# Mamba413/bess

Hardware: AMD Instinct MI355X
Metric: candidate subsets solved/sec (n=50k,p=10k,k<=200 LM) (higher is better)
Workload: dtype f64; 1 GPU; configs[1]: LM sequential path, Gaussian X n=50000 p=10000, s.list=1..200, GIC, warm start, max_iter=20, is_normal; score_pass=covariance updates (cached Gram columns), collective=none, ranks_with_work=1

## Files before the change

bess_amd/capi.py:

```python
import ctypes
import os
import sys

import numpy as np

_HERE = os.path.dirname(os.path.abspath(__file__))
LIB_PATH = os.environ.get("BESSX_LIB_PATH") or os.path.join(_HERE, "libbessx.so")

_D = ctypes.POINTER(ctypes.c_double)
_I = ctypes.POINTER(ctypes.c_int)
_i = ctypes.c_int
_d = ctypes.c_double
_ll = ctypes.c_longlong
_vp = ctypes.c_void_p

SYMBOLS = [
    "bessx_last_error", "bessx_device_info", "bessx_pywrap_bess", "bessx_bessCpp", "bessx_session_create",
    "bessx_session_destroy", "bessx_session_set_cv", "bessx_session_get_cv_folds", "bessx_session_sequential_path", "bessx_session_gs_path",
    "bessx_session_pgs_path", "bessx_session_get_screening", "bessx_session_get_screening_groups", "bessx_session_get_screening_scores", "bessx_session_score_mode", "bessx_session_counter",
    "bessx_session_trace_enable", "bessx_session_trace_size", "bessx_session_trace_copy_int",
    "bessx_session_trace_copy_double", "bessx_session_get_normalization", "bessx_session_score_pass_stats",
    "bessx_session_enable_kernel_timing", "bessx_session_submodel_steps", "bessx_session_fit", "bessx_session_fit_width", "bessx_session_reset_caches",
    "bessx_session_sequential_path_chain", "bessx_session_cv_eval", "bessx_session_debug_block_stream",
    "bessx_session_set_fill_hook", "bessx_session_set_kpath_chains",
# ... 537 lines not shown
    y, weight, state, lambda_seq = _f64(y).reshape(-1), _f64(weight), _f64(state), _f64(lambda_seq)
    sequence, g_index, always_select = _i32(sequence), _i32(g_index), _i32(always_select)
    cap = sequence.size * lambda_seq.size if path_type == 1 else 2 * (s_max - s_min + 1) + 128
    beta = np.zeros(p)
    beta_all = np.zeros((p, cap), order="F")
    coef0_all, loss_all, ic_all = np.zeros(cap), np.zeros(cap), np.zeros(cap)
    scr = np.zeros(max(screening_size, 1), dtype=np.int32)
    r = RResult()
    r.beta, r.all_capacity = _dp(beta), cap
    r.beta_all, r.coef0_all, r.train_loss_all, r.ic_all, r.screening_A = (_dp(beta_all), _dp(coef0_all), _dp(loss_all),
                                                                         _dp(ic_all), _ip(scr))
    _check(lib().bessx_bessCpp(_dp(x), n, p, _dp(y), data_type, _dp(weight), int(is_normal), algorithm_type, model_type,
                               max_iter, exchange_num, path_type, int(is_warm_start), ic_type, int(is_cv), K, _dp(state),
                               state.size, _ip(sequence), sequence.size, _dp(lambda_seq), lambda_seq.size, s_min, s_max,
                               K_max, epsilon, lambda_min, lambda_max, nlambda, int(is_screening), screening_size,
                               powell_path, _ip(g_index), g_index.size, _ip(always_select), always_select.size, tao,
                               ctypes.byref(r)))
    k = min(r.n_all, cap)
    out = {"beta": beta, "coef0": r.coef0, "train_loss": r.train_loss, "ic": r.ic, "lambda": r.lambda_,
           "beta_all": np.array(beta_all[:, :k]), "coef0_all": coef0_all[:k], "train_loss_all": loss_all[:k],
           "ic_all": ic_all[:k]}
    if path_type == 1:
        ns, nl = sequence.size, lambda_seq.size
        out["beta_all"] = [np.array(beta_all[:, j * ns:(j + 1) * ns]) for j in range(nl)]
        out["coef0_all"] = [coef0_all[j * ns:(j + 1) * ns] for j in range(nl)]
        out["train_loss_all"] = [loss_all[j * ns:(j + 1) * ns] for j in range(nl)]
        out["ic_all"] = ic_all[:ns * nl].reshape(nl, ns).T
    if is_screening:
        out["screening_A"] = scr[:screening_size].copy()
    return out


class Session:

    def __init__(self, x, y, weight=None, data_type=1, is_normal=True, model_type=1, algorithm_type=1, max_iter=20,
                 is_warm_start=True, always_select=(), x_col_major=False, device=-1, g_index=None,
                 is_screening=False, screening_size=0, score_mode=0, max_sparsity=0, stream=0, row_order=None):
        din = None
        if is_device_array(x):
            din, self.n, self.p, _keep = _device_input(x, y, weight, row_order, stream)
            x = y = w = None
        else:
            x = np.asfortranarray(x, dtype=np.float64) if x_col_major else _f64(x)
            self.n, self.p = x.shape
            y = _f64(y).reshape(-1)
            if y.size != self.n:
                raise ValueError("X.shape(0) should be equal to y.size")
            w = None if weight is None else _f64(weight)
        al = _i32(always_select)
        gi = None if g_index is None else _i32(g_index)
        self._gsize_max = 1
        if gi is not None and gi.size:
            self._gsize_max = int(np.max(np.diff(np.append(gi, self.p))))
        pb = Problem(self.n, self.p, _dp(x), int(x_col_major), _dp(y), _dp(w), data_type, int(is_normal), model_type,
                     algorithm_type, max_iter, int(is_warm_start), _ip(al), al.size, device, _ip(gi),
                     0 if gi is None else gi.size, int(is_screening), int(screening_size), int(score_mode),
                     int(max_sparsity))
        h = _vp()
        if din is not None:
            _check_device_route(lib().bessx_session_create_device(ctypes.byref(h), ctypes.byref(pb), ctypes.byref(din)))
        else:
            _check(lib().bessx_session_create(ctypes.byref(h), ctypes.byref(pb)))
        self._h = h
        self.K = 0
        self.is_warm_start = bool(is_warm_start)
        self.p_kept = lib().bessx_session_get_screening(h, None, 0)

    def score_mode(self):
        return int(lib().bessx_session_score_mode(self._h))

    def counters(self):
        names = {0: "chained_fits", 1: "cg_fallbacks", 2: "passes_over_X", 3: "chained_queued", 7: "cv_side_by_side_rounds",
                 8: "cv_union_fills", 9: "tie_rescues", 10: "cache_restarts", 11: "cv_contexts_dropped",
                 12: "cv_fold_contexts", 13: "shared_wide_fills", 14: "kpath_chunked_paths", 15: "kpath_stitch_refits",
                 16: "kpath_chunk_fills", 17: "kpath_chains_last_path",
                 18: "kpath_stitch_giveups", 19: "group_XTX_ns",
                 22: "kpath_coarse_us",
                 23: "kpath_chunks_us", 24: "kpath_stitch_us", 25: "panel_launches_one_group",
                 26: "panel_ns_one_group", 27: "panel_launches_two_groups", 28: "panel_ns_two_groups",
                 29: "shared_pass_launches", 30: "shared_pass_chain_slots", 31: "shared_pass_partial_batches",
                 32: "own_queue_streams_created_by_the_process", 33: "multi_responses_batched",
                 34: "multi_responses_host", 35: "multi_union_fills", 36: "x_bytes_uploaded_from_host",
                 37: "x_bytes_ingested_on_device", 38: "live_device_bytes_of_the_process",
                 39: "live_pinned_bytes_of_the_process", 40: "allocation_requests_of_the_process"}
        return {n: int(lib().bessx_session_counter(self._h, i)) for i, n in names.items()}

    def screening(self):
        a = np.zeros(self.p_kept, dtype=np.int32)
        lib().bessx_session_get_screening(self._h, _ip(a), a.size)
        return a

    def screening_groups(self):
        n = lib().bessx_session_get_screening_groups(self._h, None, 0)
        a = np.zeros(max(n, 1), dtype=np.int32)
        lib().bessx_session_get_screening_groups(self._h, _ip(a), n)
        return a[:n]

    def screening_scores(self):
        n = lib().bessx_session_get_screening_scores(self._h, None, 0)
        a = np.zeros(max(n, 1))
        lib().bessx_session_get_screening_scores(self._h, _dp(a), n)
        return a[:n]

    def close(self):
        if getattr(self, "_h", None):
            lib().bessx_session_destroy(self._h)
            self._h = None

    def __del__(self):
        try:
            self.close()
        except Exception:
            pass

    def __enter__(self):
        return self

    def __exit__(self, *a):
        self.close()

    def set_cv(self, K, fold_id=None, seed=123):
        f = None if fold_id is None else _i32(fold_id)
        _check(lib().bessx_session_set_cv(self._h, K, _ip(f), seed))
        self.K = K

    def cv_folds(self):
        f = np.zeros(self.n, dtype=np.int32)
        _check(lib().bessx_session_get_cv_folds(self._h, _ip(f)))
        return f

    def trace_enable(self, on=True):
        _check(lib().bessx_session_trace_enable(self._h, int(on)))

    def enable_kernel_timing(self, on=True):
        _check(lib().bessx_session_enable_kernel_timing(self._h, int(on)))

    def score_pass_stats(self, reset=False):
        sec, nb, cnt = _d(0), _d(0), _ll(0)
        _check(lib().bessx_session_score_pass_stats(self._h, int(reset), ctypes.byref(sec), ctypes.byref(cnt),
                                                    ctypes.byref(nb)))
        return {"seconds": sec.value, "launches": cnt.value, "algorithmic_bytes": nb.value}

    def submodel_steps(self, reset=False):
        cnt = _ll(0)
        _check(lib().bessx_session_submodel_steps(self._h, int(reset), ctypes.byref(cnt)))
        return cnt.value

    def normalization(self):
        xm, xn, ym = np.zeros(self.p_kept), np.zeros(self.p_kept), _d(0)
        _check(lib().bessx_session_get_normalization(self._h, _dp(xm), _dp(xn), ctypes.byref(ym)))
        return xm, xn, ym.value

    def _result(self, res, capacity, max_T0):
        beta = np.zeros(self.p)
        arr = {
            "cand_T0": np.zeros(capacity, dtype=np.int32), "cand_lambda": np.zeros(capacity),
            "cand_iters": np.zeros(capacity, dtype=np.int32), "cand_train_loss": np.zeros(capacity),
            "cand_ic": np.zeros(capacity), "cand_coef0": np.zeros(capacity),
            "cand_support": np.full((capacity, max_T0), -1, dtype=np.int32), "cand_beta": np.zeros((capacity, max_T0)),
        }
        res.beta = _dp(beta)
        res.capacity = capacity
        res.max_T0 = max_T0
        for k, v in arr.items():
            setattr(res, k, _ip(v) if v.dtype == np.int32 else _dp(v))
        return beta, arr

# ... 2316 lines not shown
```

bess_amd/csrc/bessx_dev.h:

```cpp
#ifndef BESSX_DEV_H
#define BESSX_DEV_H

#include <hip/hip_runtime.h>

namespace bessx {

struct FitCtrl {
  int done;
  int l;
  int T0;
  int k_cur;
  int irls_done;
  int irls_steps;
  int info;
  int same_prev;
  double coef0;
  double ll0;
  int d_fresh;
  int irls_last;
  int fast_same;
  int ls_m;
  double ll1;
  int gram_full;
  int cov_nfill;
  int cov_stall;
  int cov_groups;
  int cov_miss;
  int cov_nmiss;
  int serial;
  int sse_valid;
  double sse_dot;
  double sse_nrm;
  unsigned long long snap_seq;
};
static_assert(sizeof(FitCtrl) <= 128, "the published control block is 128 bytes");

constexpr int GRAM_JC = 8;
struct GramTask {
  int I, J0, nJ, pad_;
};

hipError_t launch_transpose_in(const double *src, int rows, int p, double *X, long ld, long r0, hipStream_t st);
hipError_t launch_ingest(const void *src, int f32, long long rs, long long cs, const int *order, long long n,
                         long long p, double *X, long long ld, unsigned *nan_flag, hipStream_t st);
enum { PREDICT_IDENTITY = 0, PREDICT_LOGISTIC = 1, PREDICT_POISSON = 2 };
hipError_t launch_predict(const void *src, int f32, long long rs, long long cs, long long n, const int *cols, int m,
                          const double *B, const double *c, int R, int link, double *out, long long ors, long long ocs,
                          double *out2, hipStream_t st);
struct EvalData {
  const void *y;
  int y_f32;
  long long yrs, ycs;
  const void *w;
  int w_f32;
  long long ws;
};
long long eval_workspace(int f32, long long rs, long long cs, long long n, int m, int R, int link, int weighted);
hipError_t launch_eval(const void *src, int f32, long long rs, long long cs, long long n, const int *cols, int m,
                       const double *B, const double *c, int R, int link, const EvalData &d, double *work, double *res,
                       hipStream_t st);
hipError_t launch_eval_finish(const double *part, long long nb, int RS, double *out, hipStream_t st);
long long cox_eval_workspace(long long n, int R);
hipError_t launch_cox_eval_eta(const void *src, int f32, long long rs, long long cs, long long n, const int *cols, int m,
                               const double *B, const double *zero, int R, const int *pos, double *eta, double *ex,
                               hipStream_t st);
bool cox_eval_eta_by_rows(long long rs, long long cs, int m);
hipError_t launch_cox_eval_eta_rows(const void *src, int f32, long long rs, long long cs, long long n, const int *cols,
                                    int m, const double *B, const double *zero, const int *pos, double *eta, double *ex,
                                    hipStream_t st);
hipError_t launch_cox_eval_scan_tot(const double *e, long long n, int R, double *scr, hipStream_t st);
hipError_t launch_cox_eval_suffix(double *ex, long long n, int R, double *scr, hipStream_t st);
hipError_t launch_cox_eval_loglik(const double *eta, double *ex, const double *wd, const int *first, long long n, int R,
                                  double *work, double *res, hipStream_t st);
hipError_t launch_cox_eval_pairs(const double *eta, const int *kg, const int *first, long long n, int R,
                                 unsigned long long *cnt, hipStream_t st);
long long cox_surv_workspace(long long n);
hipError_t launch_cox_baseline(const double *S, const double *wd, const int *first, long long n, const int *ends, int J,
                               double *h, double *scr, double *hout, hipStream_t st);
hipError_t launch_cox_surv_ex(const void *src, int f32, long long rs, long long cs, long long n, const int *cols, int m,
                              const double *B, const double *zero, double *ex, hipStream_t st);
hipError_t launch_cox_surv_curves(const double *ex, const double *hg, long long n, int T, int kind, double *out,
                                  long long ors, long long ocs, hipStream_t st);
constexpr int COX_BRIER_T_MAX = 1 << 20;
void cox_brier_split(long long n, long long *rows_per_slab, long long *slabs);
int cox_brier_row_groups(int T);
long long cox_brier_workspace(long long n, int T, int R);
hipError_t launch_cox_brier_ex(const void *src, int f32, long long rs, long long cs, long long n, const int *cols, int m,
                               const double *B, const double *zero, int R, double *ex, hipStream_t st);
hipError_t launch_cox_brier(const double *e, const double *time, const double *w, const double *wa, const double *hg,
                            const double *tg, const double *b, long long n, int T, int R, double W, double *part,
                            double *bs, int only, hipStream_t st);
constexpr int PAIRAUC_TILE = 1024, PAIRAUC_T_MAX = 1024;
long long pairauc_tiles_max(long long n, int T);
long long pairauc_workspace(long long n, int T, int R);
hipError_t launch_pairauc_eta(const void *src, int f32, long long rs, long long cs, long long n, const int *cols, int m,
                              const double *B, const double *zero, int R, const int *pos, double *eta, hipStream_t st);
hipError_t launch_pairauc(const double *eta, const double *cw, const double *lw, const int *kg, const int *first,
                          const int *tstart, const int *tseg, const int *tnext, long long n, int NT, int S, int R, int uno,
                          const int *last, const int *from, int Q, double *part, double *og, double *oe, int only,
                          hipStream_t st);
constexpr int INFO_M_MAX = 1024;
void info_split(long long n, int m, long long *rows_per_slab, int *slabs);
long long info_gram_workspace(long long n, int m);
long long info_workspace(int f32, long long rs, long long cs, long long n, int m, int link, int weighted);
hipError_t launch_info_gram(const void *src, int f32, long long rs, long long cs, long long n, const int *cols, int m,
                            const double *vw, const double *gw, double *part, double *info, long long ld, double *score,
                            hipStream_t st);
hipError_t launch_info(const void *src, int f32, long long rs, long long cs, long long n, const int *cols, int m,
                       const double *B, const double *c, int link, const EvalData &d, double *work, double *res,
                       double *info, long long ld, double *score, hipStream_t st);
bool info_eta_by_rows(long long rs, long long cs, int m);
hipError_t launch_info_vg(const void *src, int f32, long long rs, long long cs, long long n, const int *cols, int m,
                          const double *B, const double *c, int link, const EvalData &d, double *v, double *g,
                          hipStream_t st);
enum { SANDWICH_HC0 = 0, SANDWICH_HC1 = 1, SANDWICH_HC2 = 2, SANDWICH_HC3 = 3 };
int sandwich_run_rows();
int sandwich_sum_depth(long long rows);
int sandwich_sq_depth(long long G);
// ... 65 lines not shown
hipError_t launch_cox_addscore_cc(const double *wd, const double *S0, const int *first, const int *lastk, long long n,
                                  double *scr, double *Cc, hipStream_t st);
hipError_t launch_cox_addscore_quad(const void *src, int f32, long long rs, long long cs, long long n, const int *cand,
                                    int q, int block, const int *rowof, const double *e, const double *Cc, double *part,
                                    double *t, int only, hipStream_t st);
int groupscore_band(int dmax);
void groupscore_rows(long long n, long long *rows_per_slab, int *slabs);
int groupscore_cut(const int *d, int nt, int block, int *first);
long long groupscore_doubles(long long n, int m, int qmax, int band);
hipError_t launch_groupscore_gram(const void *src, int f32, long long rs, long long cs, long long n, const int *cand,
                                  int qb, int band, const double *vw, double *work, int only, hipStream_t st);
hipError_t launch_groupscore_sband(const double *Cb, int m, int qb, int band, const double *pk, double *Tb, double *bandS,
                                   double *a, hipStream_t st);
hipError_t launch_groupscore_extract(const double *bandT, int band, const int *lpos, const long long *offs, int g0, int ng,
                                     double *out, hipStream_t st);
void cox_groupscore_rows(long long n, long long *rows_per_slab, int *slabs, int *t_depth);
long long cox_groupscore_doubles(long long n, int qmax, int band);
hipError_t launch_cox_groupscore_cc(const double *wd, const double *S0, const int *first, const int *lastk, long long n,
                                    double *cc, hipStream_t st);
hipError_t launch_cox_groupscore_tband(const void *src, int f32, long long rs, long long cs, long long n, const int *cand,
                                       int qb, int band, const int *rowof, const double *e, const double *cc, double *work,
                                       int only, double **bandT, hipStream_t st);
hipError_t launch_y_prepare_multi(double *Y, int n, long ld, int R, const double *w, int data_type, int is_normal,
                                  int add_weight, double *y_mean, double *yy, hipStream_t st);
hipError_t launch_normalize(double *X, long ld, int n, int p, double *y, const double *w, int data_type,
                            int is_normal, int add_weight, double *x_mean, double *x_norm, double *y_mean,
                            hipStream_t st);
hipError_t launch_xtv(const double *X, long ld, int p, int U, const double *v, const double *v2, double *part,
                      double *part2, const FitCtrl *ctrl, int slot, hipStream_t st);
hipError_t launch_xtv_variant(int variant, const double *X, long ld, int p, const double *v, double *part,
                              hipStream_t st);
constexpr int XTV_MC_MAX = 8;
struct XtvMc {
  const double *v[XTV_MC_MAX], *v2[XTV_MC_MAX];
  double *part[XTV_MC_MAX], *part2[XTV_MC_MAX];
  const FitCtrl *ctrl[XTV_MC_MAX];
  int slot[XTV_MC_MAX];
  int nc;
  int *ran;
};
hipError_t launch_xtv_mc(const double *X, long ld, int p, int U, const XtvMc &a, bool two, hipStream_t st);
hipError_t launch_score(const double *part, const double *part2, int nrb, int p, const double *beta_dense,
                        const double *xtx, double n_t, double lambda, int glm, const unsigned char *always,
                        double *bd, const FitCtrl *ctrl, int slot, hipStream_t st);
struct PubArgs {
  const unsigned char *dev;
  unsigned char *host;
  int ctrl_bytes;
  size_t off_sse;
  int n_sse;
  size_t off_b, off_a;
  int kcopy;
  unsigned long long *seq_host;
  unsigned long long seq;
  const int *count_ptr;
  int on;
  unsigned char *snap;
  size_t snap_count_off;
};
struct TopkNeed {
  const double *bd;
  double *bd2;
  int p;
  int C;
  int *slot_of, *meta, *fcols;
  FitCtrl *ctrl;
  const int *A_cur;
  const double *bmm;
  int nbmm;
  const unsigned char *inA;
  int inc1;
  int bmm_fresh;
  PubArgs pub;
  PubArgs snap;
  int cont_on, cont_serial, cont_parent;
  int commit_on;
  int no_restart;
  int *cm_A_cur;
  double *cm_b_cur, *cm_beta_dense;
  int *cm_hist;
  double *cm_hist_beta, *cm_hist_coef0;
  int cm_hist_stride;
  unsigned char *cm_inA;
};
bool topk_can_fuse_need(int len);
struct TopkTie {
  int *flag;
  int *work;
};
hipError_t launch_topk(const double *score, int len, int k, int *out, int *cand, const FitCtrl *ctrl, int slot,
                       hipStream_t st, const int *run_flag = nullptr, const TopkNeed *need = nullptr,
                       const TopkTie *tie = nullptr);
bool topk_supported(int len, int k);
void topk_set_variant(int v);
void gram_set_variant(int v);
bool gram_lds_applies(int ntiles, int tile_base);
hipError_t gram_lds_prepare();
bool irls_gram_applies(int mt);
int irls_gram_slab_rows(int mt, long ld);
int irls_gram_chunks(int mt);
hipError_t launch_irls_gram(int fam, const double *X, const double *aux, long ld, int n, const int *cols,
                            const double *y, const double *w, const double *mask, int nslab, int mt, double *part,
                            int ntiles, const FitCtrl *ctrl, int slot, int t, int T0, const double *bcur,
                            double *llpart, hipStream_t st, int wfloor = 1, int rows_override = 0);
hipError_t launch_gram_reduce(const double *part, int nslab, int ntiles, double *Gt, const FitCtrl *ctrl, int slot,
                              int gate_mode, hipStream_t st);
hipError_t launch_gram(const double *X, const double *aux, long ld, const int *cols, const double *w,
                       int rows_per_slab, const GramTask *tasks, int ntask, int nslab, double *part, int ntiles,
                       double *Gt, const FitCtrl *ctrl, int slot, int gate_mode, hipStream_t st, int tile_base = 0);
hipError_t launch_gram_lm_cached(const double *X, const double *aux, long ld, int *cols, const double *w,
                                 const int *A_new, int T0, int mt, const GramTask *tasks_full, int ntask_full,
                                 int rps_full, int nslab_full, const GramTask *tasks_inc, int ntask_inc, int rps_inc,
                                 int nslab_inc, double *part, double *Gt, double *Rt, int *src, double *gbuf0,
                                 double *gbuf1, int *Ac, int *meta, FitCtrl *ctrl, int slot, hipStream_t st);
struct CholFuse {
  const double *G;
  const int *slot_of;
  int p;
  int T0;
  FitCtrl *ctrl;
  int *A_cur;
  double *b_cur, *beta_dense;
  int *hist;
  double *hist_beta, *hist_coef0;
  int hist_stride;
  unsigned char *inA;
  double yy;
  const double *d;
  const double *GS;
  int CS;
  const double *zero;
  PubArgs pub;
  double *fb_work;
  const int *dep;
};
constexpr size_t CHOL_FB_DOUBLES = 256 * 256 + 1024;
struct IrlsChk {
  int on;
  FitCtrl *ctrl;
  int t, fam;
  const double *llpart;
  int nblk, m;
  double *bcur, *bprev;
};
hipError_t launch_chol(const double *Gt, int m, int mt, double ridge, int ridge_skip0, const double *rhs,
                       const int *rhs_gather, double *sol, int *info, const FitCtrl *ctrl, int slot, int gate_mode,
                       hipStream_t st, const CholFuse *fuse = nullptr, const IrlsChk *chk = nullptr);
hipError_t launch_sym_fallback(const double *Gt, int m, int mt, double ridge, int ridge_skip0, const double *rhs,
                               const int *rhs_gather, double *sol, int *info, const FitCtrl *ctrl, int slot,
                               hipStream_t st, const CholFuse *fuse);
hipError_t launch_cg(int m, int mt, double ridge, const double *rhs, const int *A_new, double *sol, const FitCtrl *ctrl,
                     int slot, const CholFuse *fuse, int maxit, hipStream_t st, double tol = 1e-13, bool by_rows = true);
bool sel_cgr_applies(int len, int m);
hipError_t launch_sel_cgr(const double *score, int len, int k, int *A_new, const FitCtrl *ctrl, int slot,
                          const TopkNeed *need, double ridge, const double *rhs, double *sol, const CholFuse *fuse,
                          int maxit, hipStream_t st, double tol);
struct McState {
  int cand;
  int ncand;
  int need_d;
  int finished;
  int parked;
  int resume;
  int prev_fresh;
  int prev_T0;
  int solves;
// ... 116 lines not shown
bool screen_logit_group_supported(int gmax);
size_t screen_logit_group_state_doubles(int N);
hipError_t launch_screen_logit_group(const double *X, long ld, int n, int N, const int *gidx, const int *gsz,
                                     const double *y, const double *w, double *state, int *done,
                                     const unsigned char *always, double *score, hipStream_t st);
bool screen_cox_group_supported(int gmax);
hipError_t launch_screen_cox_group(const double *X, long ld, int n, int N, const int *gidx, const int *gsz,
                                   const double *st_, const double *w, const unsigned char *always, double *score,
                                   hipStream_t st);
hipError_t launch_cox_group_moments(const double *X, long ld, int n, int p, CoxBufs cb, const int *allcols, int mcols,
                                    int smax, int N, const int *gidx_h, const int *gsz_h, const int *gidx,
                                    const int *gsz, const int *goff, long mblk_len, double *mblk, double *mblk2,
                                    double *dcol, hipStream_t st);
hipError_t launch_group_score(int N, const int *gidx, const int *gsz, const int *goff, const double *mblk,
                              const double *dcol, const double *part, int nrb, int p, int lm, double n_t,
                              double lambda, const double *beta_dense, const unsigned char *always, double *bd,
                              hipStream_t st, int smax = 1, double *work = nullptr, double *zwork = nullptr,
                              const FitCtrl *ctrl = nullptr, int slot = 0, int eig_mode = 0, double *eig_v = nullptr,
                              double *eig_l = nullptr);
constexpr int GRP_EIG_MAX = 16;
hipError_t launch_group_expand(const int *G_sel, int T0, int gs, const int *gidx, int *cols, const FitCtrl *ctrl,
                               int slot, hipStream_t st);
hipError_t launch_commit_group(FitCtrl *ctrl, int slot, int T0, const int *G_new, int K, const int *cols,
                               const double *sol, int has_intercept, int wait_chain, int *A_cur, double *b_cur,
                               double *beta_dense, int *hist, double *hist_beta, double *hist_coef0, int hist_stride,
                               hipStream_t st);
hipError_t launch_screen_score_lm(const double *sxy, const double *sxx, int p, const unsigned char *always,
                                  double *score, hipStream_t st);
hipError_t launch_screen_logit(const double *X, long ld, int n, int p, const double *y, const double *w,
                               double *state, int *done, const unsigned char *always, double *score, hipStream_t st);
hipError_t launch_screen_cox(const double *X, long ld, int n, int p, const double *st_, const double *w,
                             const unsigned char *always, double *score, hipStream_t st);
hipError_t launch_gather_cols(const double *X, long ld, const int *A, int pnew, double *X2, hipStream_t st);
hipError_t launch_cov_need(const int *list, int len, const double *bd, double *bd2, int p, int *slot_of, int *meta,
                           int C, int *fcols, FitCtrl *ctrl, int slot, const int *A_cur, hipStream_t st,
                           int no_restart = 0);
hipError_t launch_cov_publish_slots(const int *fcols, const int *slot_w, int *slot_of, const FitCtrl *ctrl, hipStream_t st);
hipError_t launch_cov_fill_list(int *fcols, const int *extras, const double *bd2, int *slot_of, int *meta,
                                FitCtrl *ctrl, int parked, hipStream_t st, int spec_max, int spec, int spec_min = 0);
hipError_t launch_cov_resume(FitCtrl *ctrl, hipStream_t st);
struct CovRowSets {
  int nr;
  double *G[9], *GS[9];
  const double *xtx[9];
  int ex_lo[9], ex_hi[9];
};
hipError_t launch_cov_reduce_compact_sets(const double *part, int p, const int *fcols, const int *slot_of, int *meta,
                                          const CovRowSets &rs, int g0, int ngroups, int nslab, int CS,
                                          const FitCtrl *ctrl, int parked, hipStream_t st);
constexpr int CGB_MAX_K = 4096;
struct CgbState {
  double rr[2];
  double qq;
  int done_step;
  int steps;
};
struct CgbWork {
  double *x, *q, *r[2], *p[2], *ap[2], *part_pq[2], *part_qq;
  CgbState *st;
};
size_t cgb_work_doubles(int kcap);
hipError_t launch_cg_big(const double *G, int p, const int *slot_of, const int *meta, const int *A_new, int k,
                         double ridge, const double *xty, const double *beta_dense, double *work, int kcap, double *sol,
                         FitCtrl *ctrl, int slot, int nsteps, double tol, double yy, hipStream_t st);
struct CovUnion {
  int nf;
  const int *list[8];
  int len[8];
  int on_restart[8];
  int dn;
  const int *const *dlist;
  const int *dlen;
};
hipError_t launch_cov_fill_union(const CovUnion &u, int restart, const int *extras, const double *bd2, int spec_max,
                                 int spec_min, int *slot_of, int *meta, int p, int *fcols, FitCtrl *fill_ctrl,
                                 hipStream_t st, int C = 0);
int cov_streamed_tiles_per_wave();
hipError_t launch_cov_panel(const double *X, const double *aux, long ld, int p, const double *mask, const int *fcols,
                            int g0, int ngroups, int rows_per_slab, int nslab, double *part, const FitCtrl *ctrl,
                            int parked, hipStream_t st);
hipError_t cov_panel_prepare();
hipError_t launch_cov_reduce(const double *part, int p, const int *fcols, const int *slot_of, double *G, int g0,
                             int ngroups, int nslab, const FitCtrl *ctrl, int parked, hipStream_t st,
                             int ex_lo = 0, int ex_hi = 0);
hipError_t launch_rows_permute(const double *X, long ld, int p, const int *perm, long ldp, double *Xp, hipStream_t st);
hipError_t launch_cov_compact(const double *G, int p, const int *slot_of, const int *fcols, int g0, int ngroups,
                              double *GS, int CS, const FitCtrl *ctrl, int parked, hipStream_t st,
                              const double *xtx = nullptr, int *meta = nullptr);
hipError_t launch_cov_d(const double *G, int p, const int *slot_of, const double *xty, const int *A_cur,
                        const double *b_cur, double *d_out, const double *beta_dense, const double *xtx, double n_t,
                        double lambda, const unsigned char *always, double *bd, const unsigned char *inA, double *bmm,
                        const FitCtrl *ctrl, int slot, hipStream_t st);
hipError_t launch_cov_gram(const double *G, int p, const int *slot_of, const int *A_new, int T0, int mt, double *Gt,
                           int *meta, const FitCtrl *ctrl, int slot, hipStream_t st);
hipError_t launch_publish(const unsigned char *dev, unsigned char *host, int ctrl_bytes, size_t off_sse, int n_sse,
                          size_t off_b, size_t off_a, int kcopy, unsigned long long *seq_host, unsigned long long seq,
                          hipStream_t st, const int *count_ptr = nullptr);
hipError_t launch_vec_mul(const double *a, const double *b, long n, double *out, hipStream_t st);
hipError_t launch_part_sum(const double *part, int nrb, int p, double *out, hipStream_t st);
hipError_t launch_fill(double *a, long n, double v, hipStream_t st);
hipError_t launch_gram_cols(const int *A_new, int T0, int mp, int intercept, int rhs_col, int *cols, FitCtrl *ctrl,
                            int slot, const int *A_cur, int allow_skip, hipStream_t st);
hipError_t launch_copy(const double *src, double *dst, long n, hipStream_t st);

}
#endif
```

bess_amd/csrc/bessx_fit.cpp:

```cpp
#include "bessx_host.h"

namespace bessx {

static int score_pass(bessx_session *s, int kind, int rs, int slot, std::vector<std::pair<size_t, bool>> &k1_pairs) {
  if (rs == 0 && shared_pass_applies(s)) {
    if (s->timing) k1_pairs.push_back({(size_t)-1, false});
    if (kind == 2 && s->cox.one_pass)
      return shared_pass_submit(s, nullptr, nullptr, s->part_rs[rs], nullptr, &s->cox, s->ctrl, slot);
    if (kind != 2)
      return shared_pass_submit(s, s->r_rs[rs], kind == 1 ? s->h_rs[rs] : nullptr, s->part_rs[rs],
                                kind == 1 ? s->part2_rs[rs] : nullptr, nullptr, s->ctrl, slot);
  }
  hipEvent_t ea = nullptr, eb = nullptr;
  if (int rc = k1_begin(s, &ea, &eb)) return rc;
  hipError_t e;
  if (kind == 2)
    e = launch_cox_score_pass(s->X, s->ld, s->p, s->U, s->nrb, s->cox, s->part_rs[rs], s->part2_rs[rs], s->ctrl, slot, s->st);
  else
    e = launch_xtv(s->X, s->ld, s->p, s->U, s->r_rs[rs], kind == 1 ? s->h_rs[rs] : nullptr, s->part_rs[rs],
                   kind == 1 ? s->part2_rs[rs] : nullptr, s->ctrl, slot, s->st);
  if (s->timing && e == hipSuccess) {
    e = hipEventRecord(eb, s->st);
    k1_pairs.push_back({s->ev_used - 2, false});
  }
// ... 31 lines not shown
    return 0;
  }
  if (e == hipSuccess && mt > 16) {
    e = launch_gram(s->X, s->aux, s->ld, s->gcols, s->mask[rs], rps, tasks_full, ntask, nslab, s->gpart, ntiles, s->Gt,
                    s->ctrl, slot, 0, s->st, 0);
    if (e == hipSuccess)
      e = launch_chol_big(s->Gt, T0, mt, lambda, 0, s->xty[rs], s->A_new, s->sol, &s->ctrl->info, s->rdiag, s->zbig,
                          s->ctrl, slot, 0, s->st);
  } else if (e == hipSuccess) {
    int rps_i, nslab_i;
    const int ntask_i = s->gtask_inc_cnt[mt];
    gram_geometry(s, ntask_i * 3, &rps_i, &nslab_i);
    bessx_session::GramCache &gc = s->gcache[rs];
    e = launch_gram_lm_cached(s->X, s->aux, s->ld, s->gcols, s->mask[rs], s->A_new, T0, mt,
                              tasks_full, ntask, rps, nslab, s->gtasks + s->gtask_inc_off[mt],
                              ntask_i, rps_i, nslab_i, s->gpart, s->Gt, s->Rt, s->gsrc, gc.g0, gc.g1, gc.A, gc.meta,
                              s->ctrl, slot, s->st);
    const CholFuse fbz = chol_fallback_only(s);
    if (e == hipSuccess)
      e = launch_chol(s->Gt, T0, mt, lambda, 0, s->xty[rs], s->A_new, s->sol, &s->ctrl->info, s->ctrl, slot, 0, s->st,
                      &fbz);
    if (e == hipSuccess)
      e = launch_sym_fallback(s->Gt, T0, mt, lambda, 0, s->xty[rs], s->A_new, s->sol, &s->ctrl->info, s->ctrl, slot, s->st,
                              &fbz);
  }
  if (e == hipSuccess)
    e = launch_commit(s->ctrl, slot, T0, s->A_new, s->sol, 0, 0, s->A_cur, s->b_cur, s->beta_dense, s->hist,
                      s->hist_beta, s->hist_coef0, s->hist_stride, s->st, s->inA);
  if (e == hipSuccess)
    e = launch_resid_lm(s->X, s->ld, s->n, s->y, s->mask[rs], s->ctrl, slot, s->A_cur, s->b_cur, s->r_rs[rs],
                        s->sse, s->st);
  if (e != hipSuccess) return fail(BESSX_ERR_HIP, std::string("enqueue_lm_slot: ") + hipGetErrorString(e));
  return 0;
}


int enqueue_cov_fill(bessx_session *s, int rs, int ngroups, int parked, const FitCtrl *gate,
                            int gfirst, bool compact, const int *slot_map) {
  bessx_session::CovCache &cv = s->cov[rs];
  const FitCtrl *gc = gate ? gate : s->ctrl;
  const int *smap = slot_map ? slot_map : cv.slot_of;
  for (int g0 = gfirst; g0 < gfirst + ngroups; g0 += COV_SLOT_GROUPS) {
    const int ng = std::min(COV_SLOT_GROUPS, gfirst + ngroups - g0);
    hipEvent_t ea = nullptr, eb = nullptr;
    if (int rc = k1_begin(s, &ea, &eb)) return rc;
    hipError_t e = hipSuccess;
    if (s->cv_shared) {
      const int nsl_all = s->K * s->cvp_nsl;
      e = launch_cov_panel(s->Xp, s->zp, s->ldp, s->p, nullptr, s->cov_fcols, g0, ng, s->cvp_rps, nsl_all, s->cvp_part,
                           gc, parked, s->st);
      if (s->timing && e == hipSuccess) {
        e = hipEventRecord(eb, s->st);
        s->cov_timed.push_back({s->ev_used - 2, g0});
      }
      if (s->K + 1 <= 9 && e == hipSuccess) {
        CovRowSets rsets = {};
        rsets.nr = s->K + 1;
        for (int r = 0; r <= s->K; r++) {
          rsets.G[r] = s->cov[r].G;
          rsets.GS[r] = s->cov[r].GS;
          rsets.xtx[r] = s->xtx[r];
          rsets.ex_lo[r] = r == 0 ? 0 : (r - 1) * s->cvp_nsl;
          rsets.ex_hi[r] = r == 0 ? 0 : r * s->cvp_nsl;
        }
        e = launch_cov_reduce_compact_sets(s->cvp_part, s->p, s->cov_fcols, s->cov[0].slot_of, s->cov[0].meta, rsets, g0, ng,
                                           nsl_all, s->cov_cs, gc, parked, s->st);
      }
      for (int r = 0; r <= s->K && e == hipSuccess && s->K + 1 > 9; r++) {
        bessx_session::CovCache &cr = s->cov[r];
        const int lo = r == 0 ? 0 : (r - 1) * s->cvp_nsl, hi = r == 0 ? 0 : r * s->cvp_nsl;
        e = launch_cov_reduce(s->cvp_part, s->p, s->cov_fcols, cr.slot_of, cr.G, g0, ng, nsl_all, gc, parked, s->st,
                              lo, hi);
        if (e == hipSuccess)
          e = launch_cov_compact(cr.G, s->p, cr.slot_of, s->cov_fcols, g0, ng, cr.GS, s->cov_cs, gc, parked, s->st,
                                 s->xtx[r], cr.meta);
      }
      if (e != hipSuccess) return fail(BESSX_ERR_HIP, std::string("cov panel (shared): ") + hipGetErrorString(e));
      continue;
    }
    e = launch_cov_panel(s->X, s->aux, s->ld, s->p, s->mask[rs], s->cov_fcols, g0, ng, s->cov_rps,
                         s->cov_nslab, s->cov_part, gc, parked, s->st);
    if (s->timing && e == hipSuccess) {
      e = hipEventRecord(eb, s->st);
      s->cov_timed.push_back({s->ev_used - 2, g0});
    }
    if (e == hipSuccess)
      e = launch_cov_reduce(s->cov_part, s->p, s->cov_fcols, smap, cv.G, g0, ng, s->cov_nslab, gc, parked,
                            s->st);
    if (e == hipSuccess && compact)
      e = launch_cov_compact(cv.G, s->p, smap, s->cov_fcols, g0, ng, cv.GS, s->cov_cs, gc, parked, s->st, s->xtx[rs],
                             cv.meta);
    if (e != hipSuccess) return fail(BESSX_ERR_HIP, std::string("cov panel: ") + hipGetErrorString(e));
  }
  return 0;
}

int cov_C_dev(const bessx_session *s) { return s->cov_C - (s->cov_spec - COV_R); }

struct SlotFuse {
  const PubArgs *pub = nullptr;
  bool pub_fused = false;
  bool pub_snapshot = false;
  const PubArgs *attach = nullptr;
  bool attached = false;
  int cont_serial = 0, cont_parent = 0;
  bool cont = false, cont_fused = false;
};

CholFuse cov_fuse_args(bessx_session *s, int rs, int T0, bool force_chol, SlotFuse *sf) {
  bessx_session::CovCache &cv = s->cov[rs];
  CholFuse fz = {cv.G,          cv.slot_of, s->p,         T0,           s->ctrl,        s->A_cur, s->b_cur,
                 s->beta_dense, s->hist,    s->hist_beta, s->hist_coef0, s->hist_stride, s->inA,   s->yy_h[rs],
                 s->part_rs[rs], cv.GS, s->cov_cs,
                 cv.zero, PubArgs{}, s->fb_work, cv.meta + 4};
  if (sf && sf->pub && s->fuse && s->cov_cg && !force_chol && rs == 0) {
    fz.pub = *sf->pub;
    if (sf->pub_snapshot) fz.pub.on = 2;
    sf->pub_fused = true;
  }
  return fz;
}

int cgb_reserve(bessx_session *s) {
  bessx_session *owner = s->parent ? s->parent : s;
  if (!owner->cgb_work) {
    const int kcap = std::min(owner->cap, CGB_MAX_K);
    if (owner->own.alloc(&owner->cgb_work, cgb_work_doubles(kcap)) != hipSuccess) {
      (void)hipGetLastError();
      return 1;
    }
    owner->cgb_cap = kcap;
  }
  s->cgb_work = owner->cgb_work;
  s->cgb_cap = owner->cgb_cap;
  return 0;
}

int enqueue_cov_tail(bessx_session *s, int slot, int T0, double lambda, int rs, bool force_chol,
                            SlotFuse *sf) {
  const int mt = (T0 + 1 + 15) / 16;
  bessx_session::CovCache &cv = s->cov[rs];
  hipError_t e = hipSuccess;
  bool used_cgb = false;
  if (mt > 16 && s->cov_cg && !force_chol && T0 <= CGB_MAX_K && cgb_reserve(s) == 0) {
    e = launch_cg_big(cv.G, s->p, cv.slot_of, cv.meta, s->A_new, T0, lambda, s->xty[rs], s->beta_dense, s->cgb_work,
                      s->cgb_cap, s->sol, s->ctrl, slot, s->cgb_guess, s->cg_tol, s->yy_h[rs], s->st);
    used_cgb = e == hipSuccess;
    if (e == hipSuccess)
      e = launch_commit(s->ctrl, slot, T0, s->A_new, s->sol, 0, 0, s->A_cur, s->b_cur, s->beta_dense, s->hist,
                        s->hist_beta, s->hist_coef0, s->hist_stride, s->st, s->inA);
  } else if (mt > 16) {
    e = launch_cov_gram(cv.G, s->p, cv.slot_of, s->A_new, T0, mt, s->Gt, cv.meta, s->ctrl, slot, s->st);
    if (e == hipSuccess)
      e = launch_chol_big(s->Gt, T0, mt, lambda, 0, s->xty[rs], s->A_new, s->sol, &s->ctrl->info, s->rdiag, s->zbig,
                          s->ctrl, slot, 0, s->st);
    if (e == hipSuccess)
      e = launch_commit(s->ctrl, slot, T0, s->A_new, s->sol, 0, 0, s->A_cur, s->b_cur, s->beta_dense, s->hist,
                        s->hist_beta, s->hist_coef0, s->hist_stride, s->st, s->inA);
  } else {
    CholFuse fz = cov_fuse_args(s, rs, T0, force_chol, sf);
    if (s->cov_cg && !force_chol)
      e = launch_cg(T0, (T0 + 15) / 16, lambda, s->xty[rs], s->A_new, s->sol, s->ctrl, slot, &fz, 64, s->st, s->cg_tol,
                    s->cg_by_rows);
    else {
      e = launch_chol(s->Gt, T0, mt, lambda, 0, s->xty[rs], s->A_new, s->sol, &s->ctrl->info, s->ctrl, slot, 0, s->st,
                      &fz);
      if (e == hipSuccess)
        e = launch_sym_fallback(s->Gt, T0, mt, lambda, 0, s->xty[rs], s->A_new, s->sol, &s->ctrl->info, s->ctrl, slot,
                                s->st, &fz);
    }
  }
  if (e == hipSuccess && (rs != 0 || (mt > 16 && !used_cgb) || !s->cov_cg))
    e = launch_resid_lm(s->X, s->ld, s->n, s->y, s->mask[rs], s->ctrl, slot, s->A_cur, s->b_cur, s->r_rs[rs],
                        s->sse, s->st, 1);
  if (e != hipSuccess) return fail(BESSX_ERR_HIP, std::string("enqueue_cov_tail: ") + hipGetErrorString(e));
  return 0;
}

bool cov_speculates(const bessx_session *s) { return topk_supported(s->p, s->cov_spec) && s->p >= 2 * s->cov_spec; }

int enqueue_lm_slot_cov(bessx_session *s, int slot, int T0, double lambda, int rs, bool skip_d,
                               bool scores_ok, bool grow1, SlotFuse *sf) {
  bessx_session::CovCache &cv = s->cov[rs];
  hipError_t e = hipSuccess;
  if (skip_d && scores_ok) {
  } else if (!skip_d)
  {
    e = launch_cov_d(cv.G, s->p, cv.slot_of, s->xty[rs], s->A_cur, s->b_cur, s->part_rs[rs], s->beta_dense, s->xtx[rs],
                     (double)s->n_train[rs], lambda, s->always, s->bd, s->inA, s->cov_bmm, s->ctrl, slot, s->st);
    s->bmm_owner = rs;
  }
  else {
    e = launch_score(s->part_rs[rs], nullptr, 1, s->p, s->beta_dense, s->xtx[rs], (double)s->n_train[rs], lambda, 0,
                     s->always, s->bd, s->ctrl, slot, s->st);
    s->bmm_owner = -1;
  }
  if (e == hipSuccess && topk_can_fuse_need(s->p)) {
    TopkNeed nd = {cov_speculates(s) ? s->bd : nullptr, s->bd2, s->p, cov_C_dev(s), cv.slot_of, cv.meta, s->cov_fcols,
                   s->ctrl, s->A_cur, s->cov_bmm, (s->p + 31) / 32, s->inA, (slot == 1 && grow1) ? 1 : 0,
                   (slot == 1 && grow1 && s->bmm_owner == rs) ? 1 : 0};
    nd.cm_A_cur = s->A_cur;
    nd.cm_b_cur = s->b_cur;
    nd.cm_beta_dense = s->beta_dense;
    nd.cm_hist = s->hist;
    nd.cm_hist_beta = s->hist_beta;
    nd.cm_hist_coef0 = s->hist_coef0;
    nd.cm_hist_stride = s->hist_stride;
    nd.cm_inA = s->inA;
    nd.commit_on = (s->fuse && (T0 + 1 + 15) / 16 <= 16) ? 1 : 0;
    nd.no_restart = s->cov_no_restart ? 1 : 0;
    if (sf && sf->cont && s->fuse && slot == 1 && skip_d && scores_ok) {
      nd.cont_on = 1;
      nd.cont_serial = sf->cont_serial;
      nd.cont_parent = sf->cont_parent;
      sf->cont_fused = true;
      if (sf->attach) {
        nd.pub = *sf->attach;
        sf->attached = true;
      }
    }
    if (sf && sf->pub && sf->pub_snapshot && s->fuse && nd.commit_on && s->cov_cg && rs == 0) {
      nd.snap = *sf->pub;
      nd.snap.on = 2;
    }
    if (s->fuse_sel && s->fuse && s->cov_cg && s->cg_by_rows && sel_cgr_applies(s->p, T0)) {
      CholFuse fz = cov_fuse_args(s, rs, T0, false, sf);
      e = launch_sel_cgr(s->bd, s->p, T0, s->A_new, s->ctrl, slot, &nd, lambda, s->xty[rs], s->sol, &fz, 64, s->st,
                         s->cg_tol);
      if (e == hipSuccess && rs != 0)
        e = launch_resid_lm(s->X, s->ld, s->n, s->y, s->mask[rs], s->ctrl, slot, s->A_cur, s->b_cur, s->r_rs[rs],
                            s->sse, s->st, 1);
      if (e != hipSuccess) return fail(BESSX_ERR_HIP, std::string("enqueue_lm_slot_cov (fused): ") + hipGetErrorString(e));
      return 0;
    }
    e = launch_topk(s->bd, s->p, T0, s->A_new, s->cand, s->ctrl, slot, s->st, nullptr, &nd);
  } else if (e == hipSuccess) {
    e = launch_topk(s->bd, s->p, T0, s->A_new, s->cand, s->ctrl, slot, s->st, nullptr, nullptr, &s->tie);
    if (e == hipSuccess)
      e = launch_cov_need(s->A_new, T0, cov_speculates(s) ? s->bd : nullptr, s->bd2, s->p, cv.slot_of, cv.meta, cov_C_dev(s),
                          s->cov_fcols, s->ctrl, slot, s->A_cur, s->st, s->cov_no_restart ? 1 : 0);
  }
  if (e != hipSuccess) return fail(BESSX_ERR_HIP, std::string("enqueue_lm_slot_cov: ") + hipGetErrorString(e));
  return enqueue_cov_tail(s, slot, T0, lambda, rs, false, sf);
}

int cov_unpark(bessx_session *s, const FitCtrl *hc, int T0, double lambda, int rs, int *next_slot) {
  bessx_session::CovCache &cv = s->cov[rs];
  const int stalled = -1 - hc->l + 1, nm = hc->cov_nmiss;
  if (hc->cov_stall == 2) {
    s->cov_cg_fallbacks++;
    if ((T0 + 1 + 15) / 16 > 16) s->cgb_guess = 64;
    HIPX(launch_cov_resume(s->ctrl, s->st));
    if (int rc = enqueue_cov_tail(s, stalled, T0, lambda, rs, true)) return rc;
    *next_slot = stalled + 1;
    return 0;
  }
  if (hc->cov_stall == 3) {
    s->cov_tie_rescues++;
    HIPX(launch_cov_resume(s->ctrl, s->st));
    hipError_t e = launch_topk(s->bd, s->p, T0, s->A_new, s->cand, s->ctrl, stalled, s->st, nullptr, nullptr, &s->tie);
    if (e == hipSuccess)
      e = launch_cov_need(s->A_new, T0, cov_speculates(s) ? s->bd : nullptr, s->bd2, s->p, cv.slot_of, cv.meta,
                          cov_C_dev(s), s->cov_fcols, s->ctrl, stalled, s->A_cur, s->st, s->cov_no_restart ? 1 : 0);
    if (e != hipSuccess) return fail(BESSX_ERR_HIP, std::string("cov_unpark (tie): ") + hipGetErrorString(e));
    if (int rc = enqueue_cov_tail(s, stalled, T0, lambda, rs)) return rc;
    *next_slot = stalled + 1;
    return 0;
  }
  const bool spec = cov_speculates(s);
  hipError_t e = hipSuccess;
  struct FillGuard {
    bessx_session *c = nullptr;
    bool filled = false;
    ~FillGuard() {
      if (c) kchains_fill_end(c, filled);
    }
  } guard;
  const bool staged = s->kch_owner && kchains_staged(s) && cv.slot_w != nullptr;
  int *smap = staged ? cv.slot_w : cv.slot_of;
  if (s->kch_owner) {
    kchains_log(s, "parked: asks for the cache", T0, nm);
    const int waited = kchains_fill_begin(s);
    if (waited < 0) return fail(BESSX_ERR_HIP, "chunk chains: the fill rendezvous was abandoned");
    guard.c = s;
    kchains_log(s, waited ? "has the cache: looks again" : "has the cache: fills", T0, nm);
    if (waited > 0) {
      HIPX(launch_cov_resume(s->ctrl, s->st));
      e = launch_cov_need(s->A_new, T0, spec ? s->bd : nullptr, s->bd2, s->p, cv.slot_of, cv.meta, cov_C_dev(s),
                          s->cov_fcols, s->ctrl, stalled, s->A_cur, s->st, 1);
      if (e != hipSuccess) return fail(BESSX_ERR_HIP, std::string("cov_unpark (chunk chain): ") + hipGetErrorString(e));
      if (int rc = enqueue_cov_tail(s, stalled, T0, lambda, rs)) return rc;
      *next_slot = stalled + 1;
      return 0;
    }
  }
  if (s->fill_hook && rs == 0 && !s->parent && spec) {
    const int p = s->p;
    std::vector<int> miss((size_t)nm), slot_h((size_t)p);
    std::vector<double> sc((size_t)p);
    HIPX(hipMemcpyAsync(miss.data(), s->cov_fcols, (size_t)nm * sizeof(int), hipMemcpyDeviceToHost, s->st));
    HIPX(hipMemcpyAsync(sc.data(), s->bd2, (size_t)p * sizeof(double), hipMemcpyDeviceToHost, s->st));
    HIPX(hipMemcpyAsync(slot_h.data(), cv.slot_of, (size_t)p * sizeof(int), hipMemcpyDeviceToHost, s->st));
    HIPX(hipStreamSynchronize(s->st));
    std::vector<int> order;
    order.reserve((size_t)p);
    for (int j = 0; j < p; j++)
      if (slot_h[j] < 0 && sc[j] >= 0.0) order.push_back(j);
    int total = std::max(s->fill_hook_width, (nm + COV_R - 1) / COV_R * COV_R);
    if (nm + (int)order.size() < total) total = (nm + (int)order.size()) / COV_R * COV_R;
    if (total >= nm && total >= COV_R && total <= s->capA) {
      const int extra = total - nm;
      std::partial_sort(order.begin(), order.begin() + extra, order.end(), [&](int a, int b) {
        return sc[a] > sc[b] || (sc[a] == sc[b] && a < b);
      });
      std::vector<int> list(miss);
      list.insert(list.end(), order.begin(), order.begin() + extra);
      if (int rc = prefill_begin(s, list.data(), total, 2)) return rc;
      if (s->fill_hook(s->fill_hook_user, total / COV_R) != 0)
        return fail(BESSX_ERR_ARG, "the fill hook reported a failure");
      if (s->prefill_cols != 0) return fail(BESSX_ERR_ARG, "the fill hook returned without bessx_session_cov_prefill_end");
      s->shared_wide_fills++;
      HIPX(launch_cov_resume(s->ctrl, s->st));
      if (int rc = enqueue_cov_tail(s, stalled, T0, lambda, rs)) return rc;
      *next_slot = stalled + 1;
      return 0;
    }
  }
  const bool wide = spec && s->cov_C >= (s->p + 31) / 32 * 32 + COV_R && topk_supported(s->p, 2 * COV_R) && s->p >= 4 * COV_R;
  const int pool = wide ? 2 * COV_R : s->cov_spec;
  if (spec) e = launch_topk(s->bd2, s->p, pool, s->cov_extras, s->cand, nullptr, 0, s->st);
  if (e == hipSuccess)
    e = launch_cov_fill_list(s->cov_fcols, s->cov_extras, s->bd2, smap, cv.meta, s->ctrl, 1, s->st, s->cov_spec,
                             spec ? (wide ? 2 : 1) : 0, s->cov_spec_min);
  if (e != hipSuccess) return fail(BESSX_ERR_HIP, std::string("cov_unpark: ") + hipGetErrorString(e));
  const int room = spec ? std::min(((nm + s->cov_spec_min + s->cov_spec - 1) / s->cov_spec) * s->cov_spec - nm, pool) : 0;
  const int ngroups = (nm + room + COV_R - 1) / COV_R;
  if (test_hook("panel_log")) std::fprintf(stderr, "[bessx] fill: level %d, %d missing, list of up to %d -> %d group(s)%s\n", T0, nm, nm + room, ngroups, s->kch_owner ? " (chunk chain)" : "");
  hipStream_t own_st = s->st;
  hipStream_t fill_st = staged ? s->kch_owner->kch_fill_st : nullptr;
  if (fill_st && !s->kch_ev && s->own.event(&s->kch_ev, hipEventDisableTiming) != hipSuccess) {
    (void)hipGetLastError();
    fill_st = nullptr;
  }
  if (fill_st) {
    HIPX(hipEventRecord(s->kch_ev, own_st));
    HIPX(hipStreamWaitEvent(fill_st, s->kch_ev, 0));
    s->st = fill_st;
  }
  int frc = enqueue_cov_fill(s, rs, ngroups, 1, nullptr, 0, true, smap);
  hipError_t fe = hipSuccess;
  if (frc == 0 && staged) fe = launch_cov_publish_slots(s->cov_fcols, cv.slot_w, cv.slot_of, s->ctrl, s->st);
  s->st = own_st;
  if (frc) return frc;
  HIPX(fe);
  if (s->kch_owner) {
    HIPX(hipStreamSynchronize(fill_st ? fill_st : s->st));
    s->kch_owner->kch_chunk_fills++;
    guard.filled = true;
    kchains_log(s, "fill done", ngroups, nm);
  }
  HIPX(launch_cov_resume(s->ctrl, s->st));
  if (int rc = enqueue_cov_tail(s, stalled, T0, lambda, rs)) return rc;
  *next_slot = stalled + 1;
  return 0;
}

int glm_geometry(bessx_session *s, int T0, int *mt, int *mp, int *ntask, int *ntiles, int *rps, int *nslab) {
  *mt = (T0 + 2 + 15) / 16;
  *mp = *mt * 16;
  const GramTask *tk = nullptr;
  if (int rc = gram_tasks_for(s, *mt, &tk, ntask)) return rc;
  *ntiles = *mt * (*mt + 1) / 2;
  gram_geometry(s, *ntask, rps, nslab, *ntiles);
  if ((size_t)*nslab * *ntiles * 256 > s->gpart_elems) return fail(BESSX_ERR_ARG, "gram workspace too small");
  return 0;
}

int enqueue_glm_head(bessx_session *s, int slot, int T0, double lambda, int rs, bool skip_k1,
                            std::vector<std::pair<size_t, bool>> &k1_pairs) {
  const int fam = s->model_type;
  int mt, mp, ntask, ntiles, rps, nslab;
  if (int rc = glm_geometry(s, T0, &mt, &mp, &ntask, &ntiles, &rps, &nslab)) return rc;
  hipError_t e = hipSuccess;
  if (!skip_k1) {
    if (int rc = score_pass(s, 1, rs, slot, k1_pairs)) return rc;
  } else if (s->timing) {
    k1_pairs.push_back({(size_t)-1, false});
  }
  if (e == hipSuccess)
    e = launch_score(s->part_rs[rs], s->part2_rs[rs], s->nrb, s->p, s->beta_dense, nullptr, (double)s->n_train[rs],
                     lambda, 1, s->always, s->bd, s->ctrl, slot, s->st);
  if (e == hipSuccess) e = launch_topk(s->bd, s->p, T0, s->A_new, s->cand, s->ctrl, slot, s->st, nullptr, nullptr, &s->tie);
  if (e == hipSuccess)
    e = launch_gram_cols(s->A_new, T0, mp, 1, 1, s->gcols, s->ctrl, slot, s->A_cur, fam == 2 ? 1 : 0, s->st);
  if (e == hipSuccess) e = launch_glm_irls_begin(s->ctrl, slot, fam, T0 + 1, s->bcur, s->bprev, s->st);
  if (e != hipSuccess) return fail(BESSX_ERR_HIP, std::string("enqueue_glm_head: ") + hipGetErrorString(e));
  return 0;
}

int enqueue_glm_irls_step(bessx_session *s, int slot, int t, int T0, double lambda, int rs) {
  const int fam = s->model_type;
  int mt, mp, ntask, ntiles, rps, nslab;
  if (int rc = glm_geometry(s, T0, &mt, &mp, &ntask, &ntiles, &rps, &nslab)) return rc;
  double *z = s->aux + 2 * s->ld;
  if (s->irls_fuse && irls_gram_applies(mt)) {
    const int rows = irls_gram_slab_rows(mt, s->ld);
    const int ns = (int)((s->ld + rows - 1) / rows);
    if ((size_t)ns * ntiles * 256 <= s->gpart_elems && (size_t)ns <= s->llpart_cap) {
      hipError_t e = launch_irls_gram(fam, s->X, s->aux, s->ld, s->n, s->gcols, s->y, s->w, s->mask[rs], ns, mt,
                                      s->gpart, ntiles, s->ctrl, slot, t, T0, s->bcur, s->llpart, s->st, s->irls_wfloor);
      if (e == hipSuccess) e = launch_gram_reduce(s->gpart, ns, ntiles, s->Gt, s->ctrl, slot, 1, s->st);
      const IrlsChk ck = {1, s->ctrl, t, fam, s->llpart, ns, T0 + 1, s->bcur, s->bprev};
      const CholFuse fbz = chol_fallback_only(s);
      if (e == hipSuccess)
        e = launch_chol(s->Gt, T0 + 1, mt, 2.0 * lambda, 1, nullptr, nullptr, s->bcur, &s->ctrl->info, s->ctrl, slot, 1,
                        s->st, &fbz, &ck);
      if (e == hipSuccess && s->glm_fallback)
        e = launch_sym_fallback(s->Gt, T0 + 1, mt, 2.0 * lambda, 1, nullptr, nullptr, s->bcur, &s->ctrl->info, s->ctrl, slot,
                                s->st, &fbz);
      if (e != hipSuccess) return fail(BESSX_ERR_HIP, std::string("enqueue_glm_irls_step: ") + hipGetErrorString(e));
      return 0;
    }
  }
  hipError_t e = launch_glm_irls_prep(fam, s->X, s->ld, s->n, s->y, s->w, s->mask[rs], s->ctrl, slot, t, s->A_new, T0,
                                      s->bcur, s->Wv, z, s->llpart, s->st, s->irls_wfloor);
  if (e == hipSuccess)
    e = launch_glm_irls_check(s->ctrl, slot, t, fam, s->llpart, s->n_sse_blk, T0 + 1, s->bcur, s->bprev, s->st);
  const GramTask *tk = nullptr;
  int ntk = 0;
  if (int rc = gram_tasks_for(s, mt, &tk, &ntk)) return rc;
  if (e == hipSuccess)
    e = launch_gram(s->X, s->aux, s->ld, s->gcols, s->Wv, rps, tk, ntask, nslab, s->gpart, ntiles, s->Gt, s->ctrl,
// ... 578 lines not shown
    s->glm_fallback = true;
    HIPX(hipStreamSynchronize(s->st));
    HIPX(hipMemsetAsync(&s->ctrl->info, 0, sizeof(int), s->st));
    s->cache[rs].valid = s->cache[rs].model_only = false;
    s->dev_state_rs = -1;
    return algorithm_fit_grouped(s);
  }
  if (hc->info) return fail(BESSX_ERR_NUMERIC, "non-finite value in the k x k solve (singular Gram matrix?)");
  const int K = hc->k_cur;
  const double *sse_h = reinterpret_cast<const double *>(s->res_h + ((unsigned char *)s->sse - s->resblk));
  const double *b_h = reinterpret_cast<const double *>(s->res_h + ((unsigned char *)s->b_cur - s->resblk));
  const int *a_h = reinterpret_cast<const int *>(s->res_h + ((unsigned char *)s->A_cur - s->resblk));
  s->beta.idx.assign(a_h, a_h + K);
  s->beta.val.assign(b_h, b_h + K);
  s->coef0 = hc->coef0;
  s->l = hc->done ? hc->l : s->max_iter + 1;
  double tr = 0.0, te = 0.0;
  for (int b = 0; b < s->n_sse_blk; b++) {
    tr += sse_h[2 * b];
    te += sse_h[2 * b + 1];
  }
  s->sse_train = tr;
  s->sse_test = te;
  s->n_fits += 1;
  s->n_iters += hc->l;
  if (gcov && hc->done) {
    cc.valid = true;
    cc.cov_layout = true;
    cc.lambda = lambda;
    cc.T0 = T0;
    cc.beta = s->beta;
    cc.coef0 = s->coef0;
    s->dev_state_rs = rs;
  }
  if (s->trace.on) {
    const int L = hc->l;
    std::vector<double> hb((size_t)(L + 1) * s->hist_stride), hc0(L + 1);
    HIPX(hipMemcpy(hb.data(), s->hist_beta, hb.size() * sizeof(double), hipMemcpyDeviceToHost));
    HIPX(hipMemcpy(hc0.data(), s->hist_coef0, hc0.size() * sizeof(double), hipMemcpyDeviceToHost));
    for (int it = 1; it <= L; it++) {
      const std::vector<int> &cc = cols_hist[it - 1];
      s->trace.meta.push_back(it);
      s->trace.meta.push_back(T0);
      s->trace.meta.push_back(s->n_train[rs]);
      s->trace.meta.push_back((int)s->trace.a_flat.size());
      for (size_t i = 0; i < cc.size(); i++) {
        s->trace.a_flat.push_back(cc[i]);
        s->trace.beta_flat.push_back(hb[(size_t)it * s->hist_stride + i]);
      }
      s->trace.coef0_calls.push_back(hc0[it]);
    }
  }
  return 0;
}

int enqueue_chained(bessx_session *s, const bessx_session::Hint &hint, int rs, int parent, int buf, int batch,
                           double parent_lambda, int parent_T0) {
  const int Tn = hint.T0;
  if (!(hint.on && s->chain && s->publish && s->warm_start && !s->trace.on && rs == 0 && s->cov_mode && Tn >= 1 &&
        Tn <= s->cap && Tn + COV_R + s->cov_spec <= s->cov_C && topk_supported(s->p, Tn)))
    return 0;
  bessx_session::Ahead &ah = s->ahead;
  s->chain_queued++;
  ah.armed = true;
  ah.T0 = Tn;
  ah.lambda = hint.lambda;
  ah.rs = rs;
  ah.serial = ++s->fit_serial;
  ah.buf = buf;
  const bool cont_fusable = s->fuse && hint.lambda == parent_lambda && topk_can_fuse_need(s->p);
  PubArgs parent_pub = {};
  const bool have_parent_pub = s->pend_on && cont_fusable && s->defer_pub;
  if (have_parent_pub) {
    parent_pub = s->pend;
    s->pend_on = false;
  } else if (int rc = publish_flush(s)) {
    return rc;
  }
  if (!cont_fusable) HIPX(launch_fit_continue(s->ctrl, Tn, s->hist, s->st, ah.serial, 1, parent));
  const PubArgs pa = publish_args(s, Tn, buf, &ah.seq);
  bool published = false, snapshotted = false;
  for (int b = 0, sl = 1; b < batch && sl <= s->max_iter; b++, sl++) {
    SlotFuse sf;
    const bool last = b + 1 == batch || sl == s->max_iter;
    if (last) {
      sf.pub = &pa;
      sf.pub_snapshot = s->defer_pub;
    }
    if (sl == 1 && cont_fusable) {
      sf.cont = true;
      sf.cont_serial = ah.serial;
      sf.cont_parent = parent;
      if (have_parent_pub) sf.attach = &parent_pub;
    }
    if (int rc = enqueue_lm_slot_cov(s, sl, Tn, hint.lambda, rs, sl == 1, hint.lambda == parent_lambda,
                                     hint.lambda == parent_lambda && Tn == parent_T0 + 1, &sf))
      return rc;
    if (sl == 1 && cont_fusable && !sf.cont_fused) return fail(BESSX_ERR_HIP, "internal: chained fit was not opened");
    if (sl == 1 && have_parent_pub && !sf.attached) return fail(BESSX_ERR_HIP, "internal: deferred publication lost");
    published = published || sf.pub_fused;
    snapshotted = snapshotted || (sf.pub_fused && sf.pub_snapshot);
  }
  if (snapshotted) {
    s->pend = publish_from_snapshot(pa);
    s->pend_on = true;
    return 0;
  }
  return published ? 0 : publish_launch(s, pa);
}


int algorithm_fit(bessx_session *s) {
  if (s->grouped) return algorithm_fit_grouped(s);
  const int T0 = s->sparsity_level, rs = s->cur_rows;
  const double lambda = s->lambda_level;
  if (rs != 0 && !s->fold_ctx.empty()) fold_contexts_invalidate(s);
  if (T0 < 1 || T0 > s->cap)
    return fail(BESSX_ERR_ARG, "sparsity level " + std::to_string(T0) + " outside [1, " + std::to_string(s->cap) +
                                   "]: a session holds work space for min(p, max(2046, bessx_problem.max_sparsity))"
                                   " active columns, max_sparsity <= " + std::to_string(T0_HARD));
  if (s->model_type == 4)
    if (int rc = cox_reserve(s, T0)) return rc;
  if (!topk_supported(s->p, T0)) return fail(BESSX_ERR_UNSUPPORTED, "top-k selection: p too large for this sparsity level");
  const bool glm = s->model_type != 1;
  const bool cox = s->model_type == 4;
  const int k_init = (int)s->beta_init.idx.size();
  if (k_init > s->cap) return fail(BESSX_ERR_ARG, "initial support too large");
  bessx_session::RsCache &cc = s->cache[rs];
  const bool cov = s->cov_mode && !glm && T0 + COV_R + s->cov_spec <= s->cov_C && k_init + COV_R + s->cov_spec <= s->cov_C;
  bool use_cache = cc.valid && cc.coef0 == s->coef0_init && cc.beta.idx == s->beta_init.idx &&
                   cc.beta.val == s->beta_init.val && (!cox || s->cox_state_rs == rs) && (glm || cc.cov_layout == cov);
  if (cox) s->cox_state_rs = rs;
  bool model_kept = cov && !use_cache && cc.model_only && cc.cov_layout && s->dev_state_rs == rs &&
                          cc.coef0 == s->coef0_init && cc.beta.idx == s->beta_init.idx && cc.beta.val == s->beta_init.val &&
                          !s->trace.on && test_hook("model_kept") == nullptr;
  cc.valid = cc.model_only = false;
  const bessx_session::Hint hint = s->hint;
  s->hint.on = false;
  bool ahead_hit = false;
  int my_buf = 0, ahead_serial = 0;
  if (s->ahead.armed) {
    s->ahead.armed = false;
    const bessx_session::Ahead mine = s->ahead;
    if (cov && use_cache && s->dev_state_rs == rs && mine.T0 == T0 && mine.lambda == lambda && mine.rs == rs &&
        !s->trace.on) {
      if (int rc = enqueue_chained(s, hint, rs, mine.serial, mine.buf ^ 1, 2, lambda, T0)) return rc;
      if (!s->ahead.armed)
        if (int rc = publish_flush(s)) return rc;
      if (int rc = publish_wait(s, mine.buf, mine.seq)) return rc;
      ahead_hit = reinterpret_cast<const FitCtrl *>(s->res_h)->serial == mine.serial;
      if (!ahead_hit) {
        s->ahead.armed = false;
        s->pend_on = false;
      }
      (ahead_hit ? s->chain_hits : s->chain_dead)++;
      my_buf = mine.buf;
      ahead_serial = mine.serial;
    } else {
      HIPX(hipStreamSynchronize(s->st));
      s->pend_on = false;
      s->dev_state_rs = -1;
      use_cache = false;
      model_kept = false;
      s->chain_mismatch++;
    }
  }
// ... 269 lines not shown
```

bess_amd/csrc/bessx_host.h:

```cpp
#ifndef BESSX_HOST_H
#define BESSX_HOST_H
#include <hip/hip_runtime.h>

#include <algorithm>
#include <atomic>
#include <chrono>
#include <cfloat>
#include <cmath>
#include <cstdio>
#include <condition_variable>
#include <cstring>
#include <functional>
#include <mutex>
#include <numeric>
#include <random>
#include <string>
#include <thread>
#include <vector>

#include "../../include/bessx.h"
#include "bessx_dev.h"
#include "bessx_sync.h"

namespace bessx {
// ... 210 lines not shown
  double *Wv = nullptr, *llpart = nullptr, *bcur = nullptr, *bprev = nullptr;
  int irls_guess = 8;
  bool grouped = false;
  int N = 0, gmax = 1;
  int g_uniform = 0;
  std::vector<int> gidx_h, gsz_h, goff_h;
  int *gidx = nullptr, *gsz = nullptr, *goff = nullptr, *gcols_new = nullptr;
  double *mblk = nullptr, *dcol = nullptr;
  double *mblk2 = nullptr;
  double *mwork = nullptr, *zwork = nullptr;
  int *allcols = nullptr;
  std::vector<double *> gxtx_rs;
  std::vector<double *> geig_v_rs, geig_l_rs;
  std::vector<double> geig_lambda;
  std::vector<char> geig_valid;
  bool geig_on = true;
  int cox_state_rs = -1;
  int dev_state_rs = -1;
  CoxBufs cox = {};
  int *idcols = nullptr;
  struct RsCache {
    bool valid = false;
    bool model_only = false;
    bool cov_layout = false;
    double lambda = 0.0;
    int T0 = 0;
    SparseVec beta;
    double coef0 = 0.0;
  };
  std::vector<RsCache> cache;
  std::vector<int> n_train;
  std::vector<double> yy_h;
  int K = 0;
  double *part2 = nullptr, *bd = nullptr, *beta_dense = nullptr, *sol = nullptr;
  double *tmpv = nullptr;
  int *A_new = nullptr, *cand = nullptr, *hist = nullptr, *gcols = nullptr, *info = nullptr;
  double *fb_work = nullptr;
  int *tie_buf = nullptr;
  TopkTie tie = {nullptr, nullptr};
  double *hist_beta = nullptr, *hist_coef0 = nullptr;
  int cap = 0;
  int capA = 0;
  int hist_stride = 0;
  double *rdiag = nullptr, *zbig = nullptr;
  std::vector<std::pair<int, GramTask *>> big_tasks;
  std::vector<int> big_task_cnt;
  size_t cox_M_cols = 0;
  GramTask *gtasks = nullptr;
  std::vector<int> gtask_off, gtask_cnt;
  std::vector<int> gtask_inc_off, gtask_inc_cnt;
  struct GramCache {
    double *g0 = nullptr, *g1 = nullptr;
    int *A = nullptr, *meta = nullptr;
  };
  std::vector<GramCache> gcache;
  struct CovCache {
    double *G = nullptr;
    int *slot_of = nullptr, *meta = nullptr;
    int *slot_w = nullptr;
    double *GS = nullptr;
    double *zero = nullptr;
    bool shares_map = false;
  };
  std::vector<CovCache> cov;
  long long dbg_waits = 0, dbg_waits_ready = 0;
  double dbg_enq_s = 0.0;
  bool cov_mode = false;
  int cov_cs = 512;
  double cg_tol = 1e-13;
  int cov_spec = 32;
  int cov_spec_min = 8;
  bool fuse_sel = true;
  bool cg_by_rows = true;
  bool irls_fuse = true;
  bool glm_fallback = false;
  int irls_wfloor = 1;
  size_t llpart_cap = 0;
  long long n_submodel_steps = 0;
  bool defer_pub = true;
  bool fuse = true;
  bool cov_cg = true;
  long long cov_cg_fallbacks = 0;
  long long cov_tie_rescues = 0;
  int cov_C = 0;
  int cov_rps = 0, cov_nslab = 0;
  bool cv_shared = false;
  double *Xp = nullptr, *zp = nullptr, *cvp_part = nullptr;
  long ldp = 0;
  int cvp_rps = 0, cvp_nsl = 0;
  bessx_session *parent = nullptr;
  std::vector<bessx_session *> fold_ctx;
  bool cv_side_by_side = true;
  bool cov_no_restart = false;
  FitCtrl *fill_ctrl = nullptr;
  FitCtrl *fill_ctrl_h = nullptr;
  hipEvent_t ev_fill = nullptr, ev_ctx = nullptr;
  long long cv_union_fills = 0, cv_rounds = 0;
  long long cv_ctx_dropped = 0;
  int fill_groups_seen = 0;
  FoldPool *fold_pool = nullptr;
  double wait_deadline_s = 30.0;
  double sbs_t[6] = {0, 0, 0, 0, 0, 0};
  double *cov_part = nullptr, *bd2 = nullptr;
  unsigned char *inA = nullptr;
  double *cov_bmm = nullptr;
  int bmm_owner = -1;
  int *cov_fcols = nullptr, *cov_extras = nullptr;
  long long cov_panel_groups = 0;
  bessx::KChains *kch = nullptr;
  bessx_session *kch_owner = nullptr;
  int kpath_chains = 0;
  int kch_index = -1;
  unsigned long long kch_gen_seen = 0;
  bool light_confirm = true;
  bool kch_fill_tried = false;
  bool kch_sp_member = false;
  long long sp_launches = 0, sp_chain_slots = 0, sp_partial = 0;
  int *kch_slot_w = nullptr;
  hipStream_t kch_fill_st = nullptr;
  hipEvent_t kch_ev = nullptr;
  int resp_R = 0;
  double *resp_y = nullptr, *resp_xty = nullptr, *resp_part = nullptr, *own_xty = nullptr;
  std::vector<double> resp_mean, resp_yy, resp_null;
  double *own_y = nullptr;
  double own_yy = 0.0, own_mean = 0.0, own_null = 0.0;
  long long multi_batched = 0, multi_host = 0, multi_fills = 0;
  long long x_host_bytes = 0, x_dev_bytes = 0;
  bool fcols_wide = false;
  long long kch_paths = 0, kch_refits = 0, kch_chunk_fills = 0;
  int kch_last_chains = 0;
  bool kch_auto_off = false;
  int cov_panel_blocks = 0;
  bool own_hw_queue = false;
  long long group_xtx_ns = 0;
  hipEvent_t xtx_ev[2] = {nullptr, nullptr};
  bool xtx_ev_pending = false;
  bool path_group_xtx = true;
  long long kch_giveups = 0;
  double kch_t[3] = {0, 0, 0};
  bessx_fill_hook fill_hook = nullptr;
  void *fill_hook_user = nullptr;
  int fill_hook_width = 0;
  long long shared_wide_fills = 0;
  int prefill_cols = 0;
  int prefill_base = 0;
  double *cgb_work = nullptr;
  int cgb_cap = 0, cgb_guess = 40;
  std::vector<std::pair<size_t, int>> cov_timed;
  double *Rt = nullptr;
  int *gsrc = nullptr;
  double *gpart = nullptr, *Gt = nullptr;
  size_t gpart_elems = 0;
  int *init_idx_d = nullptr;
  double *init_val_d = nullptr;
  unsigned char *resblk = nullptr;
  size_t res_bytes = 0;
  FitCtrl *ctrl = nullptr;
  double *sse = nullptr, *b_cur = nullptr;
  int *A_cur = nullptr;
  int n_sse_blk = 0;
  unsigned char *res_h = nullptr;
  bool publish = true;
  unsigned long long *pub_flag = nullptr, pub_seq = 0;
  unsigned char *res_buf[2] = {nullptr, nullptr};
  unsigned char *snap[2] = {nullptr, nullptr};
  bool pend_on = false;
// ... 205 lines not shown
```

bess_amd/csrc/bessx_k_cov.hip:

```cpp
#include "bessx_kdev.hpp"

namespace bessx {

constexpr int COV_NJ = 4;

#ifdef BESSX_PANEL_CLOCK
#define PCLK_BEGIN()                                                  \
  const unsigned long long pclk_t0_ = __builtin_amdgcn_s_memtime();   \
  const unsigned long long pclk_r0_ = __builtin_amdgcn_s_memrealtime()
#define PCLK_END(tag)                                                                                           \
  do {                                                                                                          \
    asm volatile("s_waitcnt vmcnt(0) lgkmcnt(0)" ::: "memory");                                                 \
    if (blockIdx.x == 7 && threadIdx.x == 0) {                                                                  \
      const unsigned long long dt_ = __builtin_amdgcn_s_memtime() - pclk_t0_;                                   \
      const unsigned long long dr_ = __builtin_amdgcn_s_memrealtime() - pclk_r0_;                               \
      printf("PCLK %s cycles %llu ticks100MHz %llu MHz %.0f\n", tag, dt_, dr_, dr_ ? 100.0 * (double)dt_ / (double)dr_ : 0.0); \
    }                                                                                                           \
  } while (0)
#else
#define PCLK_BEGIN()
#define PCLK_END(tag)
#endif

__device__ __forceinline__ bool cov_gate(const FitCtrl *ctrl, int slot) {
  if (ctrl->done) return false;
  if (slot == 0) return ctrl->l == 0;
  return ctrl->l == slot - 1 && !ctrl->same_prev;
}


__global__ void __launch_bounds__(256) k_cov_need(const int *__restrict__ list, int len,
                                                  const double *__restrict__ bd, double *__restrict__ bd2, int p,
                                                  int *__restrict__ slot_of, int *__restrict__ meta, int C,
                                                  int *__restrict__ fcols, FitCtrl *__restrict__ ctrl, int slot,
                                                  const int *__restrict__ A_cur, int no_restart) {
  KT(12);
  if (ctrl->done || (slot == 0 ? ctrl->l != 0 : ctrl->l != slot - 1)) return;
  cov_need_body<256>(list, len, bd, bd2, p, slot_of, meta, C, fcols, ctrl, slot, A_cur, false, no_restart != 0);
}

__global__ void __launch_bounds__(256) k_cov_fill_list(int *__restrict__ fcols, const int *__restrict__ extras,
                                                       const double *__restrict__ bd2, int *__restrict__ slot_of,
                                                       int *__restrict__ meta, FitCtrl *__restrict__ ctrl,
                                                       int parked, int spec_max, int spec, int spec_min) {
  KT(10);
  if (parked ? !ctrl->cov_stall : (ctrl->done || ctrl->l != 0)) return;
  const int nm = ctrl->cov_nmiss;
  const int tid = threadIdx.x;
  if (nm == 0) {
    if (tid == 0) ctrl->cov_nfill = 0;
    return;
  }
  const int count = meta[0];
  const int pool = spec == 2 ? 2 * COV_R : spec_max;
  const int room = spec ? min(((nm + spec_min + spec_max - 1) / spec_max) * spec_max - nm, pool) : 0;
  __shared__ int s_ne;
  if (tid < 64) {
    const int col = (spec && tid < pool) ? extras[tid] : -1;
    const double sc = col >= 0 ? bd2[col] : -1.0;
    const bool valid = col >= 0 && sc >= 0.0 && slot_of[col] < 0;
    const unsigned long long bal = __ballot(valid);
    int rank = 0;
    if (pool > spec_max) {
      for (int u = 0; u < 64; u++) {
        const double su = __shfl(sc, u);
        const int cu = __shfl(col, u);
        const bool vu = (bal >> u) & 1ull;
        if (vu && (su > sc || (su == sc && cu < col))) rank++;
      }
    } else {
      rank = __popcll(bal & ((1ull << tid) - 1ull));
    }
    if (valid && rank < room) fcols[nm + rank] = col;
    if (tid == 0) s_ne = min((int)__popcll(bal), room);
  }
  __syncthreads();
  const int tot = nm + s_ne, padded = (tot + COV_R - 1) / COV_R * COV_R;
  for (int i = tot + tid; i < padded; i += 256) fcols[i] = -1;
  for (int i = tid; i < tot; i += 256) slot_of[fcols[i]] = count + i;
  if (tid == 0) {
    meta[0] = count + tot;
    ctrl->cov_nfill = padded;
    ctrl->cov_groups += padded / COV_R;
  }
}

__global__ void __launch_bounds__(256) k_cov_publish_slots(const int *__restrict__ fcols, const int *__restrict__ slot_w,
                                                           int *__restrict__ slot_of, const FitCtrl *__restrict__ ctrl) {
  if (!ctrl->cov_stall) return;
  const int nf = ctrl->cov_nfill;
  for (int i = threadIdx.x; i < nf; i += 256) {
    const int col = fcols[i];
    if (col >= 0) slot_of[col] = slot_w[col];
  }
}

__global__ void k_cov_resume(FitCtrl *__restrict__ ctrl) {
  KT(11);
  if (ctrl->cov_stall) {
    ctrl->cov_stall = 0;
    ctrl->l = -1 - ctrl->l;
  }
}

__global__ void __launch_bounds__(256) k_cov_fill_union(const CovUnion u, int restart, const int *__restrict__ extras,
                                                        const double *__restrict__ bd2, int spec_max, int spec_min,
                                                        int *__restrict__ slot_of, int *__restrict__ meta, int p,
                                                        int *__restrict__ fcols, FitCtrl *__restrict__ fill_ctrl, int C) {
  __shared__ int wsum[4];
  __shared__ int s_ne;
  const int tid = threadIdx.x, lane = tid & 63, wave = tid >> 6;
  const int nsets = u.nf + u.dn;
  if (restart == 2) {
    int ub = 0;
    for (int f = 0; f < nsets; f++) {
      if (f < u.nf && u.on_restart[f]) continue;
      const int *__restrict__ list = f < u.nf ? u.list[f] : u.dlist[f - u.nf];
      const int len = f < u.nf ? u.len[f] : u.dlen[f - u.nf];
      for (int base = 0; base < len; base += 256) {
        const int i = base + tid;
        const int col = i < len ? list[i] : -1;
        ub += __syncthreads_count(col >= 0 && slot_of[col] < 0);
      }
    }
    restart = (meta[0] + ub + COV_R > C) ? 1 : 0;
    __syncthreads();
  }
  if (restart) {
    for (int j = tid; j < p; j += 256) slot_of[j] = -1;
    __syncthreads();
  }
  const int count = restart ? 0 : meta[0];
  int nm = 0;
  for (int f = 0; f < nsets; f++) {
    if (f < u.nf && u.on_restart[f] && !restart) continue;
    const int *__restrict__ list = f < u.nf ? u.list[f] : u.dlist[f - u.nf];
    const int len = f < u.nf ? u.len[f] : u.dlen[f - u.nf];
    for (int base = 0; base < len; base += 256) {
      const int i = base + tid;
      const int col = i < len ? list[i] : -1;
      const int miss = (col >= 0 && slot_of[col] < 0) ? 1 : 0;
      const unsigned long long bal = __ballot(miss);
      const int rank = __popcll(bal & ((1ull << lane) - 1ull));
      if (lane == 0) wsum[wave] = __popcll(bal);
      __syncthreads();
      int off = 0, tot = 0;
#pragma unroll
      for (int w = 0; w < 4; w++) {
        off += (w < wave) ? wsum[w] : 0;
        tot += wsum[w];
      }
      if (miss) {
        fcols[nm + off + rank] = col;
        slot_of[col] = count + nm + off + rank;
      }
      nm += tot;
      __syncthreads();
    }
  }
  const int room = (extras != nullptr && nm > 0) ? min(((nm + spec_min + spec_max - 1) / spec_max) * spec_max - nm, spec_max) : 0;
  if (tid == 0) s_ne = 0;
  __syncthreads();
  if (tid < 64 && room > 0) {
    const int col = tid < spec_max ? extras[tid] : -1;
    const bool valid = col >= 0 && bd2[col] >= 0.0 && slot_of[col] < 0;
    const unsigned long long bal = __ballot(valid);
    const int rank = __popcll(bal & ((1ull << tid) - 1ull));
// ... 112 lines not shown
      __builtin_amdgcn_sched_barrier(0);                                                                        \
    }                                                                                                           \
  } while (0)
#define DP_CHUNK(cur, nxt, st, ms, rload)                                                                       \
  do {                                                                                                          \
    read_ops((cur) + 16, ob);                                                                                   \
    __builtin_amdgcn_sched_barrier(0);                                                                          \
    DP_STEP(oa, 0, nxt, st, ms, rload);                                                                         \
    __syncthreads();                                                                                            \
    read_ops(nxt, oa);                                                                                          \
    __builtin_amdgcn_sched_barrier(0);                                                                          \
    DP_STEP(ob, 1, nxt, st, ms, rload);                                                                         \
  } while (0)
  double *buf0 = smem, *buf1 = smem + BUF;
  const long r_last = r_begin + (long)(nchunk - 1) * DP_RB;
#pragma unroll
  for (int i = 0; i < NL; i++) DP_LOAD1(stA, mA, r_begin, i);
#pragma unroll
  for (int i = 0; i < NL; i++) DP_STORE1(buf0, stA, mA, i);
  {
    const long r1 = min(r_begin + DP_RB, r_last), r2 = min(r_begin + 2 * DP_RB, r_last);
#pragma unroll
    for (int i = 0; i < NL; i++) DP_LOAD1(stB, mB, r1, i);
#pragma unroll
    for (int i = 0; i < NL; i++) DP_LOAD1(stA, mA, r2, i);
  }
  __syncthreads();
  Ops oa, ob;
  read_ops(buf0, oa);
  for (int k = 0; k < nchunk; k += 2) {
    {
      const long rl = min(r_begin + (long)(k + 3) * DP_RB, r_last);
      DP_CHUNK(buf0, buf1, stB, mB, rl);
    }
    if (k + 1 >= nchunk) break;
    {
      const long rl = min(r_begin + (long)(k + 4) * DP_RB, r_last);
      DP_CHUNK(buf1, buf0, stA, mA, rl);
    }
  }
#undef DP_STEP
#undef DP_CHUNK
#undef DP_MFMA
#undef DP_LOAD1
#undef DP_STORE1
  const size_t tiles_per_slab = (size_t)njg * COV_NJ * 2;
#pragma unroll
  for (int a = 0; a < NA; a++) {
    const int jg = 2 * jb + ((ta + a) >> 2);
    if (jg < njg) {
#pragma unroll
      for (int t = 0; t < NB; t++) {
        double *out = part + (((size_t)((tb + t) >> 1) * nslab + slab) * tiles_per_slab + (size_t)(jg * COV_NJ + ((ta + a) & 3)) * 2 + ((tb + t) & 1)) * 256;
        *reinterpret_cast<d4 *>(out + lane * 4) = acc[a * NB + t];
      }
    }
  }
}

template <bool MASKED>
__global__ void __launch_bounds__(512, 1) k_cov_panel_dp(const double *__restrict__ X, const double *__restrict__ aux,
                                                         long ld, int p, const double *__restrict__ mask,
                                                         const int *__restrict__ fcols, int g0, int ngroups,
                                                         int rows_per_slab, int nslab, int njg,
                                                         double *__restrict__ part, const FitCtrl *__restrict__ ctrl,
                                                         int big) {
  KT(5);
  if (big ? !ctrl->cov_stall : (ctrl->done || ctrl->l != 0)) return;
  const int nfill = ctrl->cov_nfill;
  if (g0 * COV_R >= nfill) return;
  extern __shared__ double smem[];
  PCLK_BEGIN();
  if (ngroups >= 2 && (g0 + 1) * COV_R < nfill)
    cov_dp_body<MASKED, 4>(X, aux, ld, p, mask, fcols, g0, rows_per_slab, nslab, njg, part, smem);
  else
    cov_dp_body<MASKED, 2>(X, aux, ld, p, mask, fcols, g0, rows_per_slab, nslab, njg, part, smem);
  PCLK_END("dp");
}

__device__ __forceinline__ void cov_reduce_body(const double *__restrict__ part, int g0, int ngroups, int nslab,
                                                int njg, int p, const int *__restrict__ fcols,
                                                const int *__restrict__ slot_of, double *__restrict__ G,
                                                const FitCtrl *__restrict__ ctrl, int big,
                                                int ex_lo, int ex_hi) {
  if (big ? !ctrl->cov_stall : (ctrl->done || ctrl->l != 0)) return;
  const int gl = blockIdx.y;
  if (gl >= ngroups || (g0 + gl) * COV_R >= ctrl->cov_nfill) return;
  const size_t tiles_per_slab = (size_t)njg * COV_NJ * 2;
  const int tile = blockIdx.x, e = threadIdx.x;
  double s = 0.0;
  for (int sl = 0; sl < nslab; sl++)
    if (sl < ex_lo || sl >= ex_hi) s += part[(((size_t)gl * nslab + sl) * tiles_per_slab + tile) * 256 + e];
  const int jt = tile >> 1, ni = tile & 1, lane = e >> 2, reg = e & 3;
  const int j = jt * 16 + (lane >> 4) + 4 * reg;
  const int ci = (g0 + gl) * COV_R + ni * 16 + (lane & 15);
  const int col = fcols[ci];
  if (j < p && col >= 0) G[(size_t)slot_of[col] * p + j] = s;
}

__global__ void __launch_bounds__(256) k_cov_reduce(const double *__restrict__ part, int g0, int ngroups, int nslab,
                                                    int njg, int p, const int *__restrict__ fcols,
                                                    const int *__restrict__ slot_of, double *__restrict__ G,
                                                    const FitCtrl *__restrict__ ctrl, int slot, int big,
                                                    int ex_lo, int ex_hi) {
  KT(6);
  cov_reduce_body(part, g0, ngroups, nslab, njg, p, fcols, slot_of, G, ctrl, big, ex_lo, ex_hi);
}

__global__ void __launch_bounds__(256) k_cov_reduce_sets(const double *__restrict__ part, int g0, int ngroups, int nslab,
                                                         int njg, int p, const int *__restrict__ fcols,
                                                         const int *__restrict__ slot_of, const CovRowSets rs,
                                                         const FitCtrl *__restrict__ ctrl, int big) {
  KT(6);
  const int r = blockIdx.z;
  cov_reduce_body(part, g0, ngroups, nslab, njg, p, fcols, slot_of, rs.G[r], ctrl, big, rs.ex_lo[r], rs.ex_hi[r]);
}

__device__ __forceinline__ void cov_compact_body(const double *__restrict__ G, int p,
                                                 const int *__restrict__ slot_of,
                                                 const int *__restrict__ fcols, int g0, double *__restrict__ GS,
                                                 int CS, const FitCtrl *__restrict__ ctrl, int big,
                                                 const double *__restrict__ xtx, int *__restrict__ meta) {
  if (big ? !ctrl->cov_stall : (ctrl->done || ctrl->l != 0)) return;
  const int gl = blockIdx.y;
  if ((g0 + gl) * COV_R >= ctrl->cov_nfill) return;
  const int j = blockIdx.x * 256 + threadIdx.x;
  const int t = j < p ? slot_of[j] : -1;
  if (t < 0) return;
  const double dj = xtx != nullptr ? xtx[j] : 0.0;
  for (int c = 0; c < COV_R; c++) {
    const int col = fcols[(g0 + gl) * COV_R + c];
    if (col < 0) continue;
    const int sc = slot_of[col];
    if (sc < 0) continue;
    const double v = G[(size_t)sc * p + j];
    if (xtx != nullptr && j != col && v * v >= (1.0 - 2e-11) * dj * xtx[col] && dj > 0.0) meta[4] = 1;
    if (sc < CS && t < CS) {
      GS[(size_t)sc * CS + t] = v;
      GS[(size_t)t * CS + sc] = v;
    }
  }
}

__global__ void __launch_bounds__(256) k_cov_compact(const double *__restrict__ G, int p,
                                                     const int *__restrict__ slot_of,
                                                     const int *__restrict__ fcols, int g0, double *__restrict__ GS,
                                                     int CS, const FitCtrl *__restrict__ ctrl, int big,
                                                     const double *__restrict__ xtx, int *__restrict__ meta) {
  KT(7);
  cov_compact_body(G, p, slot_of, fcols, g0, GS, CS, ctrl, big, xtx, meta);
}

__global__ void __launch_bounds__(256) k_cov_compact_sets(const CovRowSets rs, int p, const int *__restrict__ slot_of,
                                                          const int *__restrict__ fcols, int g0, int CS,
                                                          const FitCtrl *__restrict__ ctrl, int big,
                                                          int *__restrict__ meta) {
  KT(7);
  const int r = blockIdx.z;
  cov_compact_body(rs.G[r], p, slot_of, fcols, g0, rs.GS[r], CS, ctrl, big, rs.xtx[r], meta);
}


__device__ __forceinline__ void cov_d_body(const double *__restrict__ G, int p, const int *__restrict__ slot_of,
                                           const double *__restrict__ xty, const int *__restrict__ A_cur,
                                           const double *__restrict__ b_cur, double *__restrict__ d_out,
                                           const double *__restrict__ beta_dense, const double *__restrict__ xtx,
                                           double n_t, double lambda, const unsigned char *__restrict__ always,
                                           double *__restrict__ bd, const unsigned char *__restrict__ inA,
                                           double *__restrict__ bmm, const FitCtrl *__restrict__ ctrl, int slot,
                                           int jb ) {
  const int jj = threadIdx.x & 31, g = threadIdx.x >> 5;
  const int j = jb * 32 + jj;
  const bool epi = g == 0 && j < p;
  const double e_xty = epi ? xty[j] : 0.0, e_b = epi ? beta_dense[j] : 0.0, e_xtx = epi ? xtx[j] : 1.0;
  const unsigned char e_in = epi ? inA[j] : (unsigned char)0;
  const unsigned char e_al = (epi && always != nullptr) ? always[j] : (unsigned char)0;
  if (slot >= 0 && (ctrl->done || ctrl->l != slot - 1)) return;
  constexpr int CHUNK = 512;
  __shared__ int s_sl[CHUNK];
  __shared__ double s_b[CHUNK];
  __shared__ double sm[8][32];
  const int kc = ctrl->k_cur;
  double acc0 = 0.0, acc1 = 0.0;
  for (int base = 0; base < kc; base += CHUNK) {
    const int cnt = min(CHUNK, kc - base);
    for (int i = threadIdx.x; i < cnt; i += 256) {
      const int sl = slot_of[A_cur[base + i]];
      if (sl < 0) const_cast<FitCtrl *>(ctrl)->cov_miss = 1;
      s_sl[i] = sl;
// ... 95 lines not shown
  const int a = I * 16 + (lane >> 4) + 4 * r, b = J * 16 + (lane & 15);
  double v = 0.0;
  if (a < T0 && b < T0) {
    const int sl = slot_of[A_new[b]];
    if (sl >= 0)
      v = G[(size_t)sl * p + A_new[a]];
    else
      const_cast<FitCtrl *>(ctrl)->cov_miss = 1;
  }
  Gt[(size_t)t * 256 + lane * 4 + r] = v;
}


hipError_t launch_cov_need(const int *list, int len, const double *bd, double *bd2, int p, int *slot_of, int *meta,
                           int C, int *fcols, FitCtrl *ctrl, int slot, const int *A_cur, hipStream_t st,
                           int no_restart) {
  hipLaunchKernelGGL(k_cov_need, dim3(1), dim3(256), 0, st, list, len, bd, bd2, p, slot_of, meta, C, fcols, ctrl, slot,
                     A_cur, no_restart);
  LAUNCH_CHECK();
  return hipSuccess;
}

hipError_t launch_cov_publish_slots(const int *fcols, const int *slot_w, int *slot_of, const FitCtrl *ctrl, hipStream_t st) {
  hipLaunchKernelGGL(k_cov_publish_slots, dim3(1), dim3(256), 0, st, fcols, slot_w, slot_of, ctrl);
  LAUNCH_CHECK();
  return hipSuccess;
}

hipError_t launch_cov_fill_list(int *fcols, const int *extras, const double *bd2, int *slot_of, int *meta,
                                FitCtrl *ctrl, int parked, hipStream_t st, int spec_max, int spec, int spec_min) {
  if (spec_min <= 0) spec_min = spec_max / 2;
  hipLaunchKernelGGL(k_cov_fill_list, dim3(1), dim3(256), 0, st, fcols, extras, bd2, slot_of, meta, ctrl, parked,
                     spec_max, spec, spec_min);
  LAUNCH_CHECK();
  return hipSuccess;
}

hipError_t launch_cov_resume(FitCtrl *ctrl, hipStream_t st) {
  hipLaunchKernelGGL(k_cov_resume, dim3(1), dim3(1), 0, st, ctrl);
  LAUNCH_CHECK();
  return hipSuccess;
}

hipError_t launch_cov_fill_union(const CovUnion &u, int restart, const int *extras, const double *bd2, int spec_max,
                                 int spec_min, int *slot_of, int *meta, int p, int *fcols, FitCtrl *fill_ctrl,
                                 hipStream_t st, int C) {
  if (u.nf < 1 || u.nf > 8 || u.dn < 0 || (u.dn > 0 && (!u.dlist || !u.dlen)) || spec_max > 64 || spec_min < 0 || spec_min > spec_max) return hipErrorInvalidValue;
  hipLaunchKernelGGL(k_cov_fill_union, dim3(1), dim3(256), 0, st, u, restart, extras, bd2, spec_max, spec_min, slot_of, meta, p,
                     fcols, fill_ctrl, C);
  LAUNCH_CHECK();
  return hipSuccess;
}

int cov_streamed_tiles_per_wave() { return COV_NJ; }

hipError_t launch_cov_panel(const double *X, const double *aux, long ld, int p, const double *mask, const int *fcols,
                            int g0, int ngroups, int rows_per_slab, int nslab, double *part, const FitCtrl *ctrl,
                            int parked, hipStream_t st) {
  if (ngroups < 1 || ngroups > 2) return hipErrorInvalidValue;
  const int pt = (p + 15) / 16, njg = (pt + COV_NJ - 1) / COV_NJ;
  const size_t ldsd = (size_t)2 * (DP_SC + 64) * DP_LD * sizeof(double);
  const long nbd = (long)nslab * ((njg + 1) / 2);
  if (mask)
    hipLaunchKernelGGL(k_cov_panel_dp<true>, dim3((unsigned)nbd), dim3(512), ldsd, st, X, aux, ld, p, mask, fcols, g0,
                       ngroups, rows_per_slab, nslab, njg, part, ctrl, parked);
  else
    hipLaunchKernelGGL(k_cov_panel_dp<false>, dim3((unsigned)nbd), dim3(512), ldsd, st, X, aux, ld, p, mask, fcols, g0,
                       ngroups, rows_per_slab, nslab, njg, part, ctrl, parked);
  LAUNCH_CHECK();
  return hipSuccess;
}

hipError_t cov_panel_prepare() {
  const int ldsd = (int)((size_t)2 * (DP_SC + 64) * DP_LD * sizeof(double));
  hipError_t e = hipFuncSetAttribute(reinterpret_cast<const void *>(&k_cov_panel_dp<true>),
                                     hipFuncAttributeMaxDynamicSharedMemorySize, ldsd);
  if (e != hipSuccess) return e;
  return hipFuncSetAttribute(reinterpret_cast<const void *>(&k_cov_panel_dp<false>),
                             hipFuncAttributeMaxDynamicSharedMemorySize, ldsd);
}

hipError_t launch_cov_reduce(const double *part, int p, const int *fcols, const int *slot_of, double *G, int g0,
                             int ngroups, int nslab, const FitCtrl *ctrl, int parked, hipStream_t st, int ex_lo,
                             int ex_hi) {
  const int pt = (p + 15) / 16, njg = (pt + COV_NJ - 1) / COV_NJ;
  hipLaunchKernelGGL(k_cov_reduce, dim3(njg * COV_NJ * 2, ngroups), dim3(256), 0, st, part, g0, ngroups, nslab, njg, p,
                     fcols, slot_of, G, ctrl, 0, parked, ex_lo, ex_hi);
  LAUNCH_CHECK();
  return hipSuccess;
}

hipError_t launch_cov_reduce_compact_sets(const double *part, int p, const int *fcols, const int *slot_of, int *meta,
                                          const CovRowSets &rs, int g0, int ngroups, int nslab, int CS,
                                          const FitCtrl *ctrl, int parked, hipStream_t st) {
  if (rs.nr < 1 || rs.nr > 9) return hipErrorInvalidValue;
  const int pt = (p + 15) / 16, njg = (pt + COV_NJ - 1) / COV_NJ;
  hipLaunchKernelGGL(k_cov_reduce_sets, dim3(njg * COV_NJ * 2, ngroups, rs.nr), dim3(256), 0, st, part, g0, ngroups,
                     nslab, njg, p, fcols, slot_of, rs, ctrl, parked);
  LAUNCH_CHECK();
  hipLaunchKernelGGL(k_cov_compact_sets, dim3((p + 255) / 256, ngroups, rs.nr), dim3(256), 0, st, rs, p, slot_of, fcols,
                     g0, CS, ctrl, parked, meta);
  LAUNCH_CHECK();
  return hipSuccess;
}

__global__ void __launch_bounds__(256) k_rows_permute(const double *__restrict__ X, long ld, const int *__restrict__ perm,
                                                      long ldp, double *__restrict__ Xp) {
  const long r = (long)blockIdx.x * 256 + threadIdx.x;
  if (r >= ldp) return;
  const int o = perm[r];
  Xp[(size_t)blockIdx.y * ldp + r] = o >= 0 ? X[(size_t)blockIdx.y * ld + o] : 0.0;
}
hipError_t launch_rows_permute(const double *X, long ld, int p, const int *perm, long ldp, double *Xp, hipStream_t st) {
  for (int j0 = 0; j0 < p; j0 += 32768) {
    const int nj = std::min(32768, p - j0);
    hipLaunchKernelGGL(k_rows_permute, dim3((unsigned)((ldp + 255) / 256), nj), dim3(256), 0, st, X + (size_t)j0 * ld, ld,
                       perm, ldp, Xp + (size_t)j0 * ldp);
    LAUNCH_CHECK();
  }
  return hipSuccess;
}

hipError_t launch_cov_compact(const double *G, int p, const int *slot_of, const int *fcols, int g0, int ngroups,
                              double *GS, int CS, const FitCtrl *ctrl, int parked, hipStream_t st, const double *xtx,
                              int *meta) {
  hipLaunchKernelGGL(k_cov_compact, dim3((p + 255) / 256, ngroups), dim3(256), 0, st, G, p, slot_of, fcols, g0, GS, CS,
                     ctrl, parked, xtx, meta);
  LAUNCH_CHECK();
  return hipSuccess;
}


hipError_t launch_cov_d(const double *G, int p, const int *slot_of, const double *xty, const int *A_cur,
                        const double *b_cur, double *d_out, const double *beta_dense, const double *xtx, double n_t,
                        double lambda, const unsigned char *always, double *bd, const unsigned char *inA, double *bmm,
                        const FitCtrl *ctrl, int slot, hipStream_t st) {
  hipLaunchKernelGGL(k_cov_d, dim3((p + 31) / 32), dim3(256), 0, st, G, p, slot_of, xty, A_cur, b_cur, d_out,
                     beta_dense, xtx, n_t, lambda, always, bd, inA, bmm, ctrl, slot);
  LAUNCH_CHECK();
  return hipSuccess;
}

hipError_t launch_mc_cov_d(const McChain *chains, int nchains, int p, hipStream_t st) {
  hipLaunchKernelGGL(k_mc_cov_d, dim3((p + 31) / 32, nchains), dim3(256), 0, st, chains);
  LAUNCH_CHECK();
  return hipSuccess;
}

hipError_t launch_cov_gram(const double *G, int p, const int *slot_of, const int *A_new, int T0, int mt, double *Gt,
                           int *meta, const FitCtrl *ctrl, int slot, hipStream_t st) {
  hipLaunchKernelGGL(k_cov_gram, dim3(mt * (mt + 1) / 2), dim3(256), 0, st, G, p, slot_of, A_new, T0, Gt, meta, ctrl,
                     slot);
  LAUNCH_CHECK();
  return hipSuccess;
}


}
```

bess_amd/csrc/bessx_k_solve.hip:

```cpp
#include "bessx_kdev.hpp"

namespace bessx {


__device__ __forceinline__ unsigned long long score_key(double v) {
  unsigned long long b = (unsigned long long)__double_as_longlong(v);
  return (b >> 63) ? 0ull : b;
}



template <int NT>
__device__ __forceinline__ bool repeated_set_body(const TopkNeed &nd, int k, int *__restrict__ out, int slot) {
  constexpr int NWV = NT / 64;
#ifdef BESSX_KTRACE
  unsigned long long tph_ = wall_clock64();
#endif
  PH(16);
  __shared__ double rmn[NWV], rmx[NWV];
  double mn = DBL_MAX, mx = -1.0;
  for (int b = threadIdx.x; b < nd.nbmm; b += NT) {
    mn = fmin(mn, nd.bmm[2 * b]);
    mx = fmax(mx, nd.bmm[2 * b + 1]);
  }
  wave_min_max(mn, mx);
  PH(17);
  if ((threadIdx.x & 63) == 0) {
    rmn[threadIdx.x >> 6] = mn;
    rmx[threadIdx.x >> 6] = mx;
  }
  __syncthreads();
  mn = rmn[0];
  mx = rmx[0];
#pragma unroll
  for (int w = 1; w < NWV; w++) {
    mn = fmin(mn, rmn[w]);
    mx = fmax(mx, rmx[w]);
  }
  const bool same = nd.ctrl->l >= 1 && nd.ctrl->k_cur == k && mn > mx;
  __syncthreads();
  if (threadIdx.x == 0) {
    nd.ctrl->fast_same = 0;
    if (same) nd.ctrl->same_prev = 1;
  }
  PH(18);
  if (!same) return false;
  if (nd.commit_on) {
    __shared__ int same_any_sh;
    __syncthreads();
    commit_body(nd.ctrl, slot, k, out, nullptr, 0, 0, nd.cm_A_cur, nd.cm_b_cur, nd.cm_beta_dense, nd.cm_hist,
                nd.cm_hist_beta, nd.cm_hist_coef0, nd.cm_hist_stride, &same_any_sh, nd.cm_inA);
    PH(19);
    if (nd.snap.on == 2) {
      if (threadIdx.x == 0) nd.ctrl->snap_seq = nd.snap.seq;
      __syncthreads();
      snapshot_body(nd.snap);
    }
    PH(20);
#ifdef BESSX_KTRACE
    if (threadIdx.x == 0) atomicAdd(&g_phase[28], 1ull);
#endif
  }
  return true;
}

template <int EB, int NT>
__device__ __forceinline__ void topk_body(const double *__restrict__ score, const int *__restrict__ idx_in,
                                          int len_total, int chunk, int k, int *__restrict__ out,
                                          int *__restrict__ out_count, const FitCtrl *ctrl, int slot,
                                          const int *__restrict__ run_flag, const TopkNeed &nd) {
  constexpr int NWV = NT / 64;
  if (nd.cont_on) {
    FitCtrl *c = nd.ctrl;
    const bool go = c->serial == nd.cont_parent && c->done && c->d_fresh && c->l >= 0 && !c->cov_stall && !c->info;
    if (!go) return;
    for (int i = threadIdx.x; i < k; i += NT) nd.cm_hist[i] = 0;
    __syncthreads();
    if (threadIdx.x == 0) {
      c->done = 0;
      c->l = 0;
      c->T0 = k;
      c->irls_done = 0;
      c->irls_steps = 0;
      c->info = 0;
      c->same_prev = 0;
      c->d_fresh = 0;
      c->cov_nfill = 0;
      c->cov_stall = 0;
      c->cov_groups = 0;
      c->cov_miss = 0;
      c->cov_nmiss = 0;
      c->sse_valid = 0;
      c->fast_same = 0;
      c->serial = nd.cont_serial;
    }
    __syncthreads();
  } else if (ctrl != nullptr && (ctrl->done || ctrl->l != slot - 1)) {
    return;
  }
  if (run_flag != nullptr && *run_flag == 0) return;
  __shared__ int wcnt[2][NWV];
  if (nd.slot_of != nullptr && nd.inc1 && nd.ctrl->l == 0 && nd.ctrl->k_cur + 1 == k &&
      (gridDim.x == 1 || nd.pub.on)) {
    __shared__ unsigned long long bk[NWV];
    __shared__ int bi[NWV];
    PH_BEGIN();
    const bool one_round = k - 1 <= NT;
    const int a_mine = (one_round && (int)threadIdx.x < k - 1) ? nd.A_cur[threadIdx.x] : -1;
    const int sl_mine = a_mine >= 0 ? nd.slot_of[a_mine] : 0;
    const int cnt_cache = one_round ? nd.meta[0] : 0;
    unsigned long long best = 0ull;
    int besti = 0x7fffffff;
    bool have = false;
    int dupl = 0;
    auto feed = [&](unsigned long long key, int i) {
      if (!have || key > best) {
        best = key;
        besti = i;
        have = true;
        dupl = 0;
      } else if (key == best) {
        dupl = 1;
        if (i < besti) besti = i;
      }
    };
    if (nd.bmm != nullptr && nd.bmm_fresh) {
      for (int b = threadIdx.x; b < nd.nbmm; b += NT) {
        const double v = nd.bmm[2 * b + 1];
        if (v >= 0.0) feed(score_key(v), (int)nd.bmm[2 * nd.nbmm + b]);
      }
    } else {
      double sc[EB];
      unsigned char ia[EB];
#pragma unroll
      for (int e = 0; e < EB; e++) {
        const int i = threadIdx.x + e * NT;
        const bool in = i < len_total;
        sc[e] = in ? score[i] : 0.0;
        ia[e] = in ? nd.inA[i] : (unsigned char)1;
      }
#pragma unroll
      for (int e = 0; e < EB; e++) {
        const int i = threadIdx.x + e * NT;
        if (!ia[e]) feed(score_key(sc[e]), i);
      }
    }
    PH(0);
    const unsigned long long mybest = best;
    const int mybesti = besti;
    wave_argmax(best, besti);
    if ((threadIdx.x & 63) == 0) {
      bk[threadIdx.x >> 6] = best;
      bi[threadIdx.x >> 6] = besti;
    }
    __syncthreads();
    best = bk[0];
    besti = bi[0];
#pragma unroll
    for (int w = 1; w < NWV; w++)
      if (bk[w] > best || (bk[w] == best && bi[w] < besti)) {
        best = bk[w];
        besti = bi[w];
      }
    {
      int dup = (have && mybest == best && (mybesti != besti || dupl)) ? 1 : 0;
      if (!dup && threadIdx.x < 32) {
        const int j = (besti & ~31) + (int)threadIdx.x;
        if (j < len_total && j != besti && !nd.inA[j] && score_key(score[j]) == best) dup = 1;
      }
      if (__syncthreads_or(dup)) goto full_search;
    }
    PH(1);
    const int *A_old = nd.A_cur;
    int lo = 0;
    if (one_round) {
      const int sl_new = nd.slot_of[besti];
      int smaller = 0;
      if (a_mine >= 0) {
        out[threadIdx.x + (a_mine > besti ? 1 : 0)] = a_mine;
        smaller = a_mine < besti ? 1 : 0;
      }
      lo = __syncthreads_count(smaller);
      const int miss = ((a_mine >= 0 && sl_mine < 0) || sl_new < 0) ? 1 : 0;
      const bool any_miss = __syncthreads_or(miss) != 0;
      if (threadIdx.x == 0) {
        out[lo] = besti;
        nd.ctrl->fast_same = 0;
      }
      PH(2);
      if (!any_miss && !(cnt_cache + k + COV_R > nd.C) && slot > 0) {
        if (threadIdx.x == 0) {
          nd.ctrl->same_prev = 0;
          nd.ctrl->cov_nmiss = 0;
        }
        __syncthreads();
        PH(3);
        PH_COUNT();
        return;
      }
      __syncthreads();
      cov_need_body<NT>(out, k, nd.bd, nd.bd2, nd.p, nd.slot_of, nd.meta, nd.C, nd.fcols, nd.ctrl, slot, nd.A_cur, true,
                      nd.no_restart != 0);
      PH(3);
      PH_COUNT();
      return;
    }
    for (int base = 0; base < k - 1; base += NT) {
      const int i = base + threadIdx.x;
      int smaller = 0;
      if (i < k - 1) {
        const int a = A_old[i];
        out[i + (a > besti ? 1 : 0)] = a;
        smaller = a < besti ? 1 : 0;
      }
      lo += __syncthreads_count(smaller);
    }
    if (threadIdx.x == 0) {
      out[lo] = besti;
      nd.ctrl->fast_same = 0;
    }
    __syncthreads();
    PH(2);
    cov_need_body<NT>(out, k, nd.bd, nd.bd2, nd.p, nd.slot_of, nd.meta, nd.C, nd.fcols, nd.ctrl, slot, nd.A_cur, true,
                      nd.no_restart != 0);
    PH(3);
    PH_COUNT();
    return;
  }
full_search:
  if (nd.slot_of != nullptr && nd.ctrl->fast_same) {
    if (repeated_set_body<NT>(nd, k, out, slot)) return;
  }
  __shared__ int wsum[NWV];
  __shared__ int wsum2[NWV];
  const int tid = threadIdx.x, lane = tid & 63, wave = tid >> 6;
  const int base = blockIdx.x * chunk;
  const int len = min(chunk, len_total - base);
  const int kk = min(k, len);
  const int E = (len + NT - 1) / NT;
  const int e0 = tid * E;
  unsigned long long key[EB];
#pragma unroll
  for (int e = 0; e < EB; e++) {
    int i = e0 + e;
    bool ok = e < E && i < len;
    int src = ok ? (idx_in ? idx_in[base + i] : base + i) : 0;
    key[e] = ok ? score_key(score[src]) : 0ull;
  }
  unsigned long long T = 0ull;
  int par = 0;
  for (int bit = 62; bit >= 0; bit--) {
    const unsigned long long cand = T | (1ull << bit);
    int c = 0;
#pragma unroll
    for (int e = 0; e < EB; e++) c += __popcll(__ballot(key[e] >= cand));
    if (lane == 0) wcnt[par][wave] = c;
    __syncthreads();
    int tot = 0;
#pragma unroll
    for (int w = 0; w < NWV; w++) tot += wcnt[par][w];
    if (tot >= kk) T = cand;
    par ^= 1;
    if (tot == kk) break;
  }
  int ngt = 0, neq = 0;
#pragma unroll
  for (int e = 0; e < EB; e++) {
    bool ok = e < E && (e0 + e) < len;
    ngt += (ok && key[e] > T) ? 1 : 0;
    neq += (ok && key[e] == T) ? 1 : 0;
  }
  auto block_excl_scan = [&](int v, int *ws, int &total) -> int {
    int inc = v;
#pragma unroll
    for (int o = 1; o < 64; o <<= 1) {
      int t = __shfl_up(inc, o);
      if (lane >= o) inc += t;
    }
    if (lane == 63) ws[wave] = inc;
    __syncthreads();
    int off = 0, tot = 0;
#pragma unroll
    for (int w = 0; w < NWV; w++) {
      int sv = ws[w];
      off += (w < wave) ? sv : 0;
      tot += sv;
    }
    total = tot;
    __syncthreads();
    return off + inc - v;
  };
  int tot_eq, tot_gt;
  (void)block_excl_scan(ngt, wsum, tot_gt);
  const int need_eq = kk - tot_gt;
  int eq_before = block_excl_scan(neq, wsum2, tot_eq);
  if (nd.slot_of != nullptr && tot_eq > need_eq && kk < len) {
    if (tid == 0) {
      nd.ctrl->cov_stall = 3;
      nd.ctrl->l = -1 - nd.ctrl->l;
      nd.ctrl->fast_same = 0;
    }
    return;
  }
  int take_eq = min(max(need_eq - eq_before, 0), neq);
  int nsel = ngt + take_eq, tot_sel;
  int pos = block_excl_scan(nsel, wsum, tot_sel);
  int *o = out + (size_t)blockIdx.x * k;
  int eq_seen = 0;
#pragma unroll
  for (int e = 0; e < EB; e++) {
    bool ok = e < E && (e0 + e) < len;
    bool sel = ok && key[e] > T;
    if (ok && key[e] == T) {
      sel = eq_seen < take_eq;
      eq_seen++;
    }
    if (sel) {
      o[pos] = idx_in ? idx_in[base + e0 + e] : base + e0 + e;
      pos++;
    }
  }
  if (tid == 0 && out_count != nullptr && tot_eq > need_eq && kk < len) out_count[0] = 1;
  if (nd.slot_of != nullptr) {
    __syncthreads();
    cov_need_body<NT>(out, k, nd.bd, nd.bd2, nd.p, nd.slot_of, nd.meta, nd.C, nd.fcols, nd.ctrl, slot, nd.A_cur, false,
                      nd.no_restart != 0);
  }
}

template <int EB>
__global__ void __launch_bounds__(1024) k_topk(const double *__restrict__ score, const int *__restrict__ idx_in,
                                               int len_total, int chunk, int k, int *__restrict__ out,
                                               int *__restrict__ out_count, const FitCtrl *ctrl, int slot,
                                               const int *__restrict__ run_flag, const TopkNeed nd) {
  KT(1);
  if (nd.pub.on && blockIdx.x == 1) {
    publish_body(nd.pub);
    return;
  }
  topk_body<EB, 1024>(score, idx_in, len_total, chunk, k, out, out_count, ctrl, slot, run_flag, nd);
}

__global__ void __launch_bounds__(1024) k_topk_ties(const double *__restrict__ score, int len, int k,
                                                    int *__restrict__ out, int *__restrict__ flag,
                                                    int *__restrict__ work, const FitCtrl *ctrl, int slot,
                                                    const int *__restrict__ run_flag) {
  if (ctrl != nullptr && (ctrl->done || ctrl->l != slot - 1)) return;
  if (run_flag != nullptr && *run_flag == 0) return;
  if (flag[0] == 0) return;
  constexpr int NT = 1024, NWV = NT / 64;
  __shared__ int wsum[NWV];
  __shared__ int sh_first, sh_last;
  __shared__ double sh_piv;
  const int tid = threadIdx.x, lane = tid & 63, wave = tid >> 6;
  int *idx = work, *Lp = work + len, *Rp = work + 2 * (size_t)len;
  for (int i = tid; i < len; i += NT) idx[i] = i;
  if (tid == 0) {
    sh_first = 0;
    sh_last = len;
  }
  __syncthreads();
  auto block_rank = [&](bool f, int &total) -> int {
    const unsigned long long m = __ballot(f);
    const int before = (int)__builtin_amdgcn_mbcnt_hi((unsigned)(m >> 32), __builtin_amdgcn_mbcnt_lo((unsigned)m, 0u));
    if (lane == 0) wsum[wave] = __popcll(m);
    __syncthreads();
    int off = 0, tot = 0;
#pragma unroll
    for (int w = 0; w < NWV; w++) {
      off += w < wave ? wsum[w] : 0;
      tot += wsum[w];
    }
    total = tot;
    __syncthreads();
    return off + before;
  };
  int depth = 0;
  while ((len >> (depth + 1)) > 0) depth++;
  depth *= 2;
  const int nth = k;
  while (true) {
    const int first = sh_first, last = sh_last;
    if (last - first <= 3) break;
    if (depth == 0) {
      if (tid == 0) {
        int *f = idx + first;
        const long hl = (long)nth + 1 - first;
        auto adjust = [&](long hole, int value) {
          const long top = hole;
          long child = hole;
          while (child < (hl - 1) / 2) {
            child = 2 * (child + 1);
            if (score[f[child]] > score[f[child - 1]]) child--;
            f[hole] = f[child];
            hole = child;
          }
          if ((hl & 1) == 0 && child == (hl - 2) / 2) {
            child = 2 * (child + 1);
            f[hole] = f[child - 1];
            hole = child - 1;
          }
          long parent = (hole - 1) / 2;
          while (hole > top && score[f[parent]] > score[value]) {
            f[hole] = f[parent];
            hole = parent;
            parent = (hole - 1) / 2;
          }
          f[hole] = value;
        };
        if (hl >= 2)
          for (long parent = (hl - 2) / 2;; parent--) {
            adjust(parent, f[parent]);
            if (parent == 0) break;
          }
        for (int i = nth + 1; i < last; i++)
          if (score[idx[i]] > score[f[0]]) {
            const int value = idx[i];
            idx[i] = f[0];
            adjust(0, value);
          }
        const int t = idx[first];
        idx[first] = idx[nth];
        idx[nth] = t;
// ... 1025 lines not shown
  if (wave == 0) {
    double t1 = 0.0, t2 = 0.0, t3 = 0.0, gd = 0.0;
#pragma unroll
    for (int r = 0; r < RPT; r++) {
      const int row = lane + 64 * r;
      const double x = xs[row], qr = qs[row] + r_t[r];
      t1 = fma(x, qr, t1);
      t2 = fma(x, x, t2);
      t3 = fma(fabs(x), fabs(qr), t3);
      gd = fmax(gd, gds[row]);
    }
    const double a1 = wsum(t1), a2 = wsum(t2), a3 = wsum(t3);
#pragma unroll
    for (int o = 32; o >= 1; o >>= 1) gd = fmax(gd, __shfl_xor(gd, o));
    if (tid == 0) {
      const double tr = fz.yy - a1 - ridge * a2;
      fz.ctrl->sse_dot = a1;
      fz.ctrl->sse_nrm = a2;
      fz.ctrl->sse_valid =
          (tr > 1e-6 * fz.yy && 4e-16 * (a3 + (ridge + gd) * a2 + fz.yy) <= 1e-10 * tr) ? 1 : 0;
    }
  }
  __syncthreads();
  CGP(5);
  commit_body(fz.ctrl, slot, m, A_new, sol, 0, 0, fz.A_cur, fz.b_cur, fz.beta_dense, fz.hist, fz.hist_beta,
              fz.hist_coef0, fz.hist_stride, &same_any_sh, fz.inA);
  CGP(6);
}

template <int RPT, int NCW>
__global__ void __launch_bounds__(512) k_cgr(int m, int nc, double ridge, const double *__restrict__ rhs,
                                             const int *__restrict__ A_new, double *__restrict__ sol,
                                             const FitCtrl *__restrict__ ctrl, int slot, const CholFuse fz, int maxit,
                                             const double tol) {
  KT(2);
  cgr_body<RPT, NCW>(m, nc, ridge, rhs, A_new, sol, ctrl, slot, fz, maxit, tol);
  if (fz.pub.on) {
    __syncthreads();
    if (fz.pub.on == 2) {
      if (fz.ctrl->snap_seq != fz.pub.seq) snapshot_body(fz.pub);
    } else {
      publish_body(fz.pub);
    }
  }
}

template <int EB, int RPT, int NCW>
__global__ void __launch_bounds__(512) k_sel_cgr(const double *__restrict__ score, int len, int k, int *out,
                                                 const FitCtrl *ctrl, int slot, const TopkNeed nd, int nc, double ridge,
                                                 const double *__restrict__ rhs, double *sol, const CholFuse fz,
                                                 int maxit, const double tol) {
  KT(14);
  if (nd.pub.on && blockIdx.x == 1) {
    publish_body(nd.pub);
    return;
  }
#ifdef BESSX_KTRACE
  const unsigned long long kt0_ = wall_clock64();
#endif
  {
    if (!nd.cont_on && nd.commit_on && nd.slot_of != nullptr && !ctrl->done && ctrl->l == slot - 1 && ctrl->l >= 1 &&
        nd.ctrl->fast_same) {
      if (repeated_set_body<512>(nd, k, out, slot)) {
        if (fz.pub.on) {
          __syncthreads();
          if (fz.pub.on == 2) {
            if (fz.ctrl->snap_seq != fz.pub.seq) snapshot_body(fz.pub);
          } else {
            publish_body(fz.pub);
          }
        }
#ifdef BESSX_KTRACE
        asm volatile("s_waitcnt vmcnt(0) lgkmcnt(0)" ::: "memory");
        if (threadIdx.x == 0) {
          atomicAdd(&g_phase[8], wall_clock64() - kt0_);
          atomicAdd(&g_phase[14], 1ull);
        }
        KT(15);
#endif
        return;
      }
    }
  }
  topk_body<EB, 512>(score, nullptr, len, len, k, out, nullptr, ctrl, slot, nullptr, nd);
  __syncthreads();
#ifdef BESSX_KTRACE
  const unsigned long long kt1_ = wall_clock64();
  unsigned long long kt2_ = kt1_;
#endif
  cgr_body<RPT, NCW>(k, nc, ridge, rhs, out, sol, ctrl, slot, fz, maxit, tol);
#ifdef BESSX_KTRACE
  asm volatile("s_waitcnt vmcnt(0) lgkmcnt(0)" ::: "memory");
  kt2_ = wall_clock64();
#endif
  if (fz.pub.on) {
    __syncthreads();
    if (fz.pub.on == 2) {
      if (fz.ctrl->snap_seq != fz.pub.seq) snapshot_body(fz.pub);
    } else {
      publish_body(fz.pub);
    }
  }
#ifdef BESSX_KTRACE
  {
    asm volatile("s_waitcnt vmcnt(0) lgkmcnt(0)" ::: "memory");
    if (threadIdx.x == 0) {
      const unsigned long long kt3_ = wall_clock64();
      const int cls = ctrl->same_prev ? 0 : 1;
      atomicAdd(&g_phase[8 + 3 * cls], kt1_ - kt0_);
      atomicAdd(&g_phase[9 + 3 * cls], kt2_ - kt1_);
      atomicAdd(&g_phase[10 + 3 * cls], kt3_ - kt2_);
      atomicAdd(&g_phase[14 + cls], 1ull);
    }
  }
  KT(15);
#endif
}

template <int EB>
__device__ __noinline__ void mc_topk_call(const double *score, int p, int k, int *out, const FitCtrl *ctrl, int slot,
                                          const TopkNeed *nd) {
  topk_body<EB, 512>(score, nullptr, p, p, k, out, nullptr, ctrl, slot, nullptr, *nd);
}
template <int RPT, int NCW>
__device__ __noinline__ void mc_cgr_call(int m, int nc, double ridge, const double *rhs, const int *A_new, double *sol,
                                         const FitCtrl *ctrl, int slot, const CholFuse *fz, int maxit, double tol) {
  cgr_body<RPT, NCW>(m, nc, ridge, rhs, A_new, sol, ctrl, slot, *fz, maxit, tol);
}

template <int EB>
__global__ void __launch_bounds__(512) k_mc_sel_cgr(const McChain *__restrict__ chains) {
  const McChain &ch = chains[blockIdx.y];
  McState *st = ch.state;
  const int tid = threadIdx.x;
  if (st->finished || st->parked) return;
  const TopkNeed &nd = ch.nd;
  const CholFuse &fz = ch.fz;
  FitCtrl *ctrl = nd.ctrl;
  {
    const int nd_ = st->need_d;
    __syncthreads();
    if (nd_ && ctrl->done == 0 && tid == 0) st->need_d = 0;
    __syncthreads();
    if (nd_ && ctrl->done) {
    }
  }
  for (int pass = 0; pass < 4; pass++) {
    __syncthreads();
    const int resume = st->resume;
    if (!resume) {
      if (ctrl->done) {
        const int cand = st->cand, T0 = ctrl->T0, W = ch.width;
        for (int i = tid; i < W; i += 512) {
          ch.rec_A[(size_t)cand * W + i] = i < T0 ? fz.A_cur[i] : -1;
          ch.rec_b[(size_t)cand * W + i] = i < T0 ? fz.b_cur[i] : 0.0;
        }
        const int fresh = (ctrl->d_fresh && !ctrl->info && !ctrl->cov_miss) ? 1 : 0;
        const int bad = (ctrl->info || ctrl->cov_miss) ? 1 : 0;
        __syncthreads();
        if (tid == 0) {
          ch.rec_i[cand * MC_REC_I + 0] = T0;
          ch.rec_i[cand * MC_REC_I + 1] = ctrl->l;
          ch.rec_i[cand * MC_REC_I + 2] = ctrl->sse_valid;
          ch.rec_i[cand * MC_REC_I + 3] = 1;
          ch.rec_d[cand * MC_REC_D + 0] = ctrl->coef0;
          ch.rec_d[cand * MC_REC_D + 1] = ctrl->sse_dot;
          ch.rec_d[cand * MC_REC_D + 2] = ctrl->sse_nrm;
        }
        if (bad) {
          if (tid == 0) {
            ch.rec_i[cand * MC_REC_I + 3] = 0;
            st->finished = 2;
            st->why = 2;
          }
          return;
        }
        if (cand + 1 >= st->ncand) {
          if (tid == 0) {
            st->cand = cand + 1;
            st->finished = 1;
          }
          return;
        }
        const int Tn = ch.seq[cand + 1];
        for (int i = tid; i < Tn; i += 512) nd.cm_hist[i] = 0;
        __syncthreads();
        if (tid == 0) {
          st->cand = cand + 1;
          st->prev_fresh = fresh;
          st->prev_T0 = T0;
          ctrl->done = 0;
          ctrl->l = 0;
          ctrl->T0 = Tn;
          ctrl->irls_done = 0;
          ctrl->irls_steps = 0;
          ctrl->info = 0;
          ctrl->same_prev = 0;
          ctrl->d_fresh = 0;
          ctrl->cov_nfill = 0;
          ctrl->cov_stall = 0;
          ctrl->cov_groups = 0;
          ctrl->cov_miss = 0;
          ctrl->cov_nmiss = 0;
          ctrl->sse_valid = 0;
          ctrl->fast_same = 0;
// ... 531 lines not shown
```

bess_amd/csrc/bessx_kchunks.cpp:

```cpp
#include "bessx_host.h"
#include "bessx_kplan.h"
#include <optional>

namespace bessx {

struct SharedPass {
  PassRendezvous rdv;
  bool on = false;
  int kind = 0;
  int cap = XTV_MC_MAX;
  hipStream_t st = nullptr;
  std::mutex launch_mu;
  hipEvent_t ev_in[XTV_MC_MAX] = {};
  static constexpr int RING = 8;
  hipEvent_t ev_out[RING] = {};
  XtvMc xq = {};
  CoxMc cq = {};
  std::atomic<int> rc{0};
  void fail_with(hipError_t e) {
    int none = 0;
    if (e != hipSuccess) rc.compare_exchange_strong(none, (int)e);
  }
  bool timing = false;
  std::vector<hipEvent_t> tev;
// ... 703 lines not shown
        HIPX(hipMemcpyAsync(k->mc_ulen, stage_len, (size_t)u.dn * sizeof(int), hipMemcpyHostToDevice, st));
        u.dlist = k->mc_ulist;
        u.dlen = k->mc_ulen;
      }
      if (spec_src)
        HIPX(launch_topk(spec_src->bd2, p, s->cov_spec, spec_src->cov_extras, spec_src->cand, nullptr, 0, st));
      HIPX(launch_cov_fill_union(u, 0, spec_src ? spec_src->cov_extras : nullptr, spec_src ? spec_src->bd2 : nullptr,
                                 s->cov_spec, s->cov_spec / 2, s->cov[0].slot_of, s->cov[0].meta, p, s->cov_fcols,
                                 s->fill_ctrl, st));
      HIPX(hipMemcpyAsync(s->fill_ctrl_h, s->fill_ctrl, sizeof(FitCtrl), hipMemcpyDeviceToHost, st));
      HIPX(hipStreamSynchronize(st));
      s->cov_panel_groups += s->fill_ctrl_h->cov_groups - s->fill_groups_seen;
      s->fill_groups_seen = s->fill_ctrl_h->cov_groups;
      const int ngroups = s->fill_ctrl_h->cov_nfill / COV_R;
      if (ngroups > (ub + s->cov_spec + 2 * COV_R - 1) / COV_R)
        return fail(BESSX_ERR_NUMERIC, "internal error: union fill list longer than its bound (merged chains)");
      if (int rc = enqueue_cov_fill(s, 0, ngroups, 1, s->fill_ctrl)) return rc;
      if (s->timing) {
        HIPX(hipStreamSynchronize(st));
        if (int rc = cov_collect(s, s->fill_ctrl_h->cov_nfill)) return rc;
      }
      for (size_t i = 0; i < parked.size(); i++) stage_resume[i] = parked[i];
      HIPX(hipMemcpyAsync(k->mc_rlist, stage_resume, parked.size() * sizeof(int), hipMemcpyHostToDevice, st));
      HIPX(launch_mc_resume_list(k->mc_chains, k->mc_rlist, (int)parked.size(), st));
      if (fills) (*fills)++;
    }
    if (all) break;
  }
  rec.i.assign((size_t)nrec * MC_REC_I, 0);
  rec.A.assign((size_t)nrec * width, 0);
  rec.d.assign((size_t)nrec * MC_REC_D, 0.0);
  rec.b.assign((size_t)nrec * width, 0.0);
  HIPX(hipMemcpyAsync(rec.i.data(), k->mc_rec_i, rec.i.size() * sizeof(int), hipMemcpyDeviceToHost, st));
  HIPX(hipMemcpyAsync(rec.d.data(), k->mc_rec_d, rec.d.size() * sizeof(double), hipMemcpyDeviceToHost, st));
  HIPX(hipMemcpyAsync(rec.A.data(), k->mc_rec_A, rec.A.size() * sizeof(int), hipMemcpyDeviceToHost, st));
  HIPX(hipMemcpyAsync(rec.b.data(), k->mc_rec_b, rec.b.size() * sizeof(double), hipMemcpyDeviceToHost, st));
  HIPX(hipStreamSynchronize(st));
  for (const McJob &j : jobs) {
    for (auto &cc : j.c->cache) cc.valid = cc.model_only = false;
    j.c->dev_state_rs = -1;
  }
  return 0;
}

int mc_contexts(bessx_session *s, int n) {
  if (hipSetDevice(s->device) != hipSuccess) return fail(BESSX_ERR_HIP, "merged chains: device");
  if (!s->kch) s->kch = new KChains();
  KChains *k = s->kch;
  while ((int)k->mc_ctx.size() < n) {
    bessx_session *c = nullptr;
    if (int rc = chain_ctx_create(s, &c, false)) {
      (void)hipGetLastError();
      return rc;
    }
    c->kch_index = -1;
    k->mc_ctx.push_back(c);
  }
  return 0;
}

bessx_session *mc_context(bessx_session *s, int i) { return s->kch->mc_ctx[(size_t)i]; }

namespace {

using Clock = std::chrono::steady_clock;
double secs(Clock::time_point a, Clock::time_point b) { return std::chrono::duration<double>(b - a).count(); }

struct StartModel {
  SparseVec b;
  double c0 = 0.0;
};

struct ChunkPath {
  bessx_session *s;
  KChains *k;
  const int *seq;
  int ns;
  double lambda;
  int ic_type, C, width;
  bool lm_cov;
  std::vector<int> bounds;
  CoarsePlan coarse;
  bool staged = false;
  std::vector<StartModel> start;
  std::vector<ChunkRun> run;
  bool early_on = false;
  std::vector<ChunkRun> early_st;
  std::vector<char> early_ok;
  long long refits = 0, iters_path = 0;
  int give_up_from = -1;
  Clock::time_point t_begin, t_coarse, t_chunks;

  void plan() {
    const char *esh = test_hook("kchunks_shared_pass");
    double wdiv = (!esh || std::atoi(esh) != 0) ? 1e9 : 160.0;
    if (const char *ew = test_hook("kchunks_len_div")) wdiv = std::max(1.0, std::atof(ew));
    bounds = chunk_bounds(s->model_type == 1, seq, ns, C, wdiv);
    constexpr int COARSE_MAX = 3;
    int M = lm_cov ? std::min(C - 1, COARSE_MAX) : 0;
    if (const char *ev = test_hook("kchunks_coarse")) M = std::max(0, std::min(M, std::atoi(ev)));
    coarse = coarse_plan(C, M);
  }

  void fill_stream() {
    if (lm_cov) {
      const char *ev = test_hook("kchunks_staged");
      staged = !ev || std::atoi(ev) != 0;
    }
    if (staged && !s->kch_slot_w && k->own.alloc(&s->kch_slot_w, (size_t)s->p) != hipSuccess) {
      (void)hipGetLastError();
      staged = false;
    }
    if (!staged || s->kch_fill_st || s->kch_fill_tried) return;
    s->kch_fill_tried = true;
    hipDeviceProp_t prop;
    const int cus = hipGetDeviceProperties(&prop, s->device) == hipSuccess ? prop.multiProcessorCount : 0;
    const int blocks = s->cov_panel_blocks;
    const int rounds = (cus > 0 && blocks > 0) ? (blocks + cus - 1) / cus : 0;
    const int idle = rounds > 0 ? cus - (blocks + rounds - 1) / rounds : 0;
    int leave = idle >= 4 ? std::min(16, idle) : 0, stride = 1;
    if (const char *er = test_hook("kchunks_reserve")) {
      leave = std::max(0, std::atoi(er));
      if (const char *c2 = std::strchr(er, ':')) stride = std::max(1, std::atoi(c2 + 1));
    }
    if (leave > 0 && !ctx_stream_create(s->device, &s->kch_fill_st, leave, stride)) s->kch_fill_st = nullptr;
  }

  int coarse_chain(bessx_path_chain *link) {
    t_begin = Clock::now();
    const char *el = test_hook("kchunks_log");
    k->log_on = el && std::atoi(el) != 0;
    k->log_t0 = t_begin;
    k->log.clear();
    run = std::vector<ChunkRun>((size_t)C);
    start.assign((size_t)C, StartModel());
    if (link) {
      for (int i = 0; i < link->init_len; i++) {
        if (link->init_idx[i] < 0 || link->init_idx[i] >= s->p) return fail(BESSX_ERR_ARG, "chain: init index out of range");
        start[0].b.idx.push_back(link->init_idx[i]);
        start[0].b.val.push_back(link->init_val[i]);
      }
      start[0].c0 = link->init_coef0;
      link->stopped_at = -1;
    }
    s->hint.on = false;
    StartModel at = start[0];
    for (size_t m = 0; m < coarse.coarse_at.size(); m++) {
      if (int rc = run_fit(s, seq[bounds[(size_t)coarse.coarse_at[m]] - 1], lambda, at.b, at.c0)) return rc;
      at = {s->beta, s->coef0};
      for (int r = 0; r < C; r++)
        if (coarse.start_of[(size_t)r] == (int)m + 1) start[(size_t)r] = at;
    }
    if (int rc = settle_device_chain(s)) return rc;
    HIPX(hipStreamSynchronize(s->st));
    t_coarse = Clock::now();
    return 0;
  }

  int writer_map_in_step() {
    if (!staged) return 0;
    HIPX(hipMemcpyAsync(s->kch_slot_w, s->cov[0].slot_of, (size_t)s->p * sizeof(int), hipMemcpyDeviceToDevice, s->st));
    HIPX(hipStreamSynchronize(s->st));
    return 0;
  }

  void walk(bessx_session *c, ChunkRun &t, int count, bool keep_model = false) {
    t.rc = (keep_model || hipSetDevice(s->device) == hipSuccess) ? context_begin(c, keep_model) : fail(BESSX_ERR_HIP, "hipSetDevice");
    c->timing = s->timing;
    if (t.rc == 0) t.rc = sequential_path(c, seq + t.lo, count, &lambda, 1, ic_type, 0, &t.res, &t.chain);
    if (t.rc == 0 && hipStreamSynchronize(c->st) != hipSuccess) t.rc = fail(BESSX_ERR_HIP, "chunk chain: stream");
    if (t.rc) t.err = g_err;
    t.last_len = t.chain.last_len;
    t.last_coef0 = t.chain.last_coef0;
  }

  int budget_of(int r) const { return std::max(8, (run[r].hi - run[r].lo) / 6); }

  void early_stitch(int r) {
    bessx_session *c = k->ctx[(size_t)r - 1];
    ChunkRun &q = run[(size_t)r], &t = early_st[(size_t)r];
    const int want = std::min(q.hi - q.lo, budget_of(r));
    const auto t0 = Clock::now();
    sp_leave(c);
    while (k->progress[r].load(std::memory_order_acquire) < want && k->ended[r].load(std::memory_order_acquire) == 0) {
      kchains_safe_point(c);
      std::this_thread::sleep_for(std::chrono::microseconds(20));
      if (secs(t0, Clock::now()) > s->wait_deadline_s) return;
    }
    if (k->ended[r].load(std::memory_order_acquire) == 2) return;
    const int rows = k->progress[r].load(std::memory_order_acquire);
    if (rows < want) return;
    t.shape(q.lo, q.hi, width);
    t.link_behind(run[(size_t)r - 1], &q, rows);
    kchains_log(c, "early stitch of the next chunk", q.lo, rows);
    sp_join(c);
    walk(c, t, want, true);
    if (t.rc == 0) early_ok[(size_t)r] = 1;
    else (void)hipGetLastError();
    kchains_log(c, "early stitch done", t.res.n_candidates, t.chain.stopped_at);
  }

  void chunk_job(int r) {
    if (r >= C) return;
    bessx_session *c = k->ctx[r];
    ChunkRun &q = run[r];
    const StartModel &m = start[(size_t)r];
    q.link(m.b.idx.data(), m.b.val.data(), (int)m.b.idx.size(), m.c0);
    kchains_log(c, "chunk starts", q.lo, q.hi);
    walk(c, q, q.hi - q.lo);
    kchains_log(c, "chunk ends", q.lo, q.hi);
    if (r < 10) k->ended[r].store(q.rc ? 2 : 1, std::memory_order_release);
    if (early_on && q.rc == 0 && r + 1 < C) early_stitch(r + 1);
    sp_leave(c);
    kchains_leave(k, q.rc != 0);
  }

  int chunk_round(std::optional<SharedPassScope> &scope) {
    if (int rc = writer_map_in_step()) return rc;
    if (lm_cov)
      for (bessx_session *c : k->ctx) c->cov[0].slot_w = staged ? s->kch_slot_w : nullptr;
    for (int r = 0; r < C; r++) run[r].shape(bounds[r], bounds[r + 1], width);
    kchains_round(k, C, staged);
    scope.emplace(s, k, C, lm_cov);
    early_on = C <= 9;
    if (const char *ee = test_hook("kchunks_early_stitch")) early_on = early_on && std::atoi(ee) != 0;
    early_st = std::vector<ChunkRun>((size_t)C);
    early_ok.assign((size_t)C, 0);
    for (int r = 0; r < 10; r++) {
      k->progress[r].store(0, std::memory_order_relaxed);
      k->ended[r].store(0, std::memory_order_relaxed);
    }
    if (!k->pool.run([this](int r) { chunk_job(r); }, s->wait_deadline_s))
      return fail(BESSX_ERR_HIP, "chunk chains: a host thread did not come back");
    for (int r = 0; r < C; r++)
      if (run[r].rc) return fail(run[r].rc, "chunk chain: " + run[r].err);
    t_chunks = Clock::now();
    return 0;
  }

  void stitch_job(int r, ChunkRun &t) {
    bessx_session *c = k->ctx[r];
    const ChunkRun &q = run[r];
    t.shape(q.lo, q.hi, width);
// ... 201 lines not shown
```

bess_amd/csrc/bessx_kdev.hpp:

```cpp
#ifndef BESSX_KDEV_HPP
#define BESSX_KDEV_HPP
#include <hip/hip_runtime.h>

#include <algorithm>
#include <cfloat>
#include <climits>
#include <cstdint>
#include <cstdlib>
#include <string>

#include "bessx_dev.h"

namespace bessx {
#ifdef BESSX_KTRACE
__device__ unsigned long long g_ktrace[1 << 16];
__device__ unsigned int g_ktrace_n;
#define KT(id)                                                                   \
  do {                                                                           \
    if (blockIdx.x == 0 && blockIdx.y == 0 && threadIdx.x == 0) {                \
      const unsigned n_ = atomicAdd(&g_ktrace_n, 1u);                            \
      if (n_ < (1u << 16)) g_ktrace[n_] = (wall_clock64() << 8) | (unsigned)(id); \
    }                                                                            \
  } while (0)
#else
// ... 374 lines not shown
                                                double *__restrict__ bcur, double *__restrict__ bprev) {
  __shared__ double sm[NT / 64];
  __shared__ int fin;
  double s = 0.0;
  for (int b = threadIdx.x; b < nblk; b += NT) s += llpart[b];
  s = wave_sum(s);
  if ((threadIdx.x & 63) == 0) sm[threadIdx.x >> 6] = s;
  __syncthreads();
  if (threadIdx.x == 0) {
    s = 0.0;
    for (int q = 0; q < NT / 64; q++) s += sm[q];
    int done = 0;
    if (fam == 2) {
      if (t == 0) {
        ctrl->ll0 = s;
      } else {
        if (fabs(ctrl->ll0 - s) / (0.1 + fabs(s)) < 1e-6) done = 1;
        if (!done) ctrl->ll0 = s;
      }
      fin = done ? 2 : ((t == 30) ? 1 : 0);
    } else {
      if (t == 0) {
        ctrl->ll0 = 1e5;
      } else {
        if (fabs(ctrl->ll0 - s) / fabs(0.1 + ctrl->ll0) < 1e-6) done = 1;
        if (!done) ctrl->ll0 = s;
      }
      fin = (done || t == 50) ? 1 : 0;
    }
  }
  __syncthreads();
  const int f = fin;
  if (f != 2)
    for (int i = threadIdx.x; i < m; i += NT) bprev[i] = bcur[i];
  __syncthreads();
  if (threadIdx.x == 0) {
    ctrl->irls_steps = t + 1;
    if (f != 0) ctrl->irls_done = 1;
  }
  return f != 0;
}

__device__ __forceinline__ double clampv(double v, double c) { return v > c ? c : (v < -c ? -c : v); }

__device__ __forceinline__ d2 lin_pred2(const double *__restrict__ X, long ld, long i, const int *__restrict__ A,
                                        const double *__restrict__ b, int k) {
  d2 acc0 = d2{0.0, 0.0}, acc1 = d2{0.0, 0.0}, acc2 = d2{0.0, 0.0}, acc3 = d2{0.0, 0.0};
  int a = 0;
  for (; a + 4 <= k; a += 4) {
    const d2 x0 = *reinterpret_cast<const d2 *>(X + (size_t)A[a] * ld + i);
    const d2 x1 = *reinterpret_cast<const d2 *>(X + (size_t)A[a + 1] * ld + i);
    const d2 x2 = *reinterpret_cast<const d2 *>(X + (size_t)A[a + 2] * ld + i);
    const d2 x3 = *reinterpret_cast<const d2 *>(X + (size_t)A[a + 3] * ld + i);
    acc0 += x0 * b[a];
    acc1 += x1 * b[a + 1];
    acc2 += x2 * b[a + 2];
    acc3 += x3 * b[a + 3];
  }
  for (; a < k; a++) acc0 += *reinterpret_cast<const d2 *>(X + (size_t)A[a] * ld + i) * b[a];
  return (acc0 + acc1) + (acc2 + acc3);
}

__device__ __forceinline__ void block_pair_sum_128(double a, double b, double *out2) {
  __shared__ double smp[2][2];
  a = wave_sum(a);
  b = wave_sum(b);
  if ((threadIdx.x & 63) == 0) {
    smp[threadIdx.x >> 6][0] = a;
    smp[threadIdx.x >> 6][1] = b;
  }
  __syncthreads();
  if (threadIdx.x == 0) {
    out2[0] = smp[0][0] + smp[1][0];
    out2[1] = smp[0][1] + smp[1][1];
  }
}

__device__ __forceinline__ const double *gram_col(const double *__restrict__ X, const double *__restrict__ aux,
                                                  long ld, int idx) {
  return idx >= 0 ? X + (size_t)idx * ld : aux + (size_t)(-idx - 1) * ld;
}

template <int NT>
__device__ void cov_need_body(const int *__restrict__ list, int len, const double *__restrict__ bd,
                              double *__restrict__ bd2, int p, int *__restrict__ slot_of, int *__restrict__ meta, int C,
                              int *__restrict__ fcols, FitCtrl *__restrict__ ctrl, int slot,
                              const int *__restrict__ A_cur, bool known_diff = false, bool no_restart = false) {
  __shared__ int wsum[NT / 64];
  const int tid = threadIdx.x, lane = tid & 63, wave = tid >> 6;
  if (slot > 0 && known_diff) {
    if (tid == 0) ctrl->same_prev = 0;
  } else if (slot > 0) {
    int diff = 1;
    if (ctrl->l >= 1 && ctrl->k_cur == len) {
      diff = 0;
      for (int i = tid; i < len; i += NT) diff |= (list[i] != A_cur[i]);
    }
    diff = __syncthreads_or(diff);
    if (tid == 0) ctrl->same_prev = diff ? 0 : 1;
    if (!diff) return;
  }
  int count = meta[0];
  bool restart = count + len + COV_R > C;
  if (restart) {
    int missing = 0;
    for (int base = 0; base < len; base += NT) {
      const int i = base + tid;
      const int col = i < len ? list[i] : -1;
      missing += __syncthreads_count(col >= 0 && slot_of[col] < 0);
    }
    restart = count + missing + COV_R > C;
  }
  if (restart && no_restart && slot > 0) {
    if (tid == 0) {
      ctrl->cov_nmiss = 0;
      ctrl->cov_stall = 4;
      ctrl->l = -1 - ctrl->l;
    }
    return;
  }
  if (restart) {
    for (int j = tid; j < p; j += NT) slot_of[j] = -1;
    count = 0;
    __syncthreads();
  }
  int nm = 0;
  if (!restart && len <= NT) {
    const int col = tid < len ? list[tid] : -1;
    const int miss = (col >= 0 && slot_of[col] < 0) ? 1 : 0;
    if (!__syncthreads_or(miss)) {
      if (tid == 0) ctrl->cov_nmiss = 0;
      return;
    }
  }
  for (int base = 0; base < len; base += NT) {
    const int i = base + tid;
    const int col = i < len ? list[i] : -1;
    const int miss = (col >= 0 && slot_of[col] < 0) ? 1 : 0;
    int inc = miss;
#pragma unroll
    for (int o = 1; o < 64; o <<= 1) {
      int t = __shfl_up(inc, o);
      if (lane >= o) inc += t;
    }
    if (lane == 63) wsum[wave] = inc;
    __syncthreads();
    int off = 0, tot = 0;
#pragma unroll
    for (int w = 0; w < NT / 64; w++) {
      off += (w < wave) ? wsum[w] : 0;
      tot += wsum[w];
    }
    if (miss) fcols[nm + off + inc - 1] = col;
    nm += tot;
    __syncthreads();
  }
  const bool spec = nm > 0 && bd != nullptr;
  if (tid == 0) {
    if (restart) {
      meta[0] = 0;
      meta[3] += 1;
      meta[4] = 0;
    }
    ctrl->cov_nmiss = nm;
    if (nm > 0 && slot > 0) {
      ctrl->cov_stall = 1;
      ctrl->l = -1 - ctrl->l;
    }
  }
  if (spec) {
    for (int j = tid; j < p; j += NT) bd2[j] = slot_of[j] >= 0 ? -1.0 : bd[j];
    __syncthreads();
    for (int i = tid; i < nm; i += NT) bd2[fcols[i]] = -1.0;
  }
}

#define LAUNCH_CHECK()                         \
  do {                                         \
    hipError_t e__ = hipGetLastError();        \
    if (e__ != hipSuccess) return e__;         \
  } while (0)

}
#endif
```

bess_amd/csrc/bessx_session.cpp:

```cpp
#include "bessx_host.h"

namespace bessx {

thread_local std::string g_err;
thread_local int g_marginal_fit_variant = 0;



void ctx_free(bessx_session *c) {
  if (!c) return;
  if (c->st) (void)hipStreamSynchronize(c->st);
  c->own.release();
  if (c->st) ctx_stream_destroy(c->st);
  delete c;
}

void drop_fold_contexts(bessx_session *s) {
  if (s->fold_pool) {
    s->fold_pool->stop();
    if (!s->fold_pool->broken) delete s->fold_pool;
    s->fold_pool = nullptr;
  }
  for (bessx_session *c : s->fold_ctx) ctx_free(c);
  s->fold_ctx.clear();
  s->cv_own.release_one(s->fill_ctrl);
  s->cv_own.release_one(s->fill_ctrl_h);
  s->cv_own.release_one(s->ev_fill);
  s->cv_own.release_one(s->ev_ctx);
  s->fill_ctrl = s->fill_ctrl_h = nullptr;
  s->ev_fill = s->ev_ctx = nullptr;
  s->fill_groups_seen = 0;
}

void session_free(bessx_session *s) {
  if (!s) return;
  if (std::getenv("BESSX_DEBUG") && !s->fold_ctx.empty())
    std::fprintf(stderr, "[bessx] fold chains side by side: %lld rounds, %lld union fills; ms in start %.2f, enqueue %.2f, "
                 "wait %.2f, fill %.2f, continue %.2f, results %.2f\n", s->cv_rounds, s->cv_union_fills, s->sbs_t[0] * 1e3,
                 s->sbs_t[1] * 1e3, s->sbs_t[2] * 1e3, s->sbs_t[3] * 1e3, s->sbs_t[4] * 1e3, s->sbs_t[5] * 1e3);
  drop_fold_contexts(s);
  if (std::getenv("BESSX_DEBUG") && s->kch_paths)
    std::fprintf(stderr, "[bessx] chunk chains: %lld paths, %lld stitch refits, %lld fills in the chunk phase; ms per path in "
                 "the coarse chain %.2f, the chunks %.2f, the stitch %.2f\n", s->kch_paths, s->kch_refits, s->kch_chunk_fills,
                 1e3 * s->kch_t[0] / s->kch_paths, 1e3 * s->kch_t[1] / s->kch_paths, 1e3 * s->kch_t[2] / s->kch_paths);
  kchains_free(s);
  if (std::getenv("BESSX_DEBUG"))
    std::fprintf(stderr, "[bessx] chained fits: queued %lld, used %lld, not started %lld, mismatched %lld; "
                 "CG solves handed to Cholesky: %lld; waits for a published block: %lld, of which the block was "
                 "already there %lld; queueing chained fits took %.3f ms\n",
                 s->chain_queued, s->chain_hits, s->chain_dead, s->chain_mismatch, s->cov_cg_fallbacks, s->dbg_waits,
                 s->dbg_waits_ready, s->dbg_enq_s * 1e3);
  (void)hipSetDevice(s->device);
  if (s->st) (void)hipStreamSynchronize(s->st);
  s->cv_own.release();
  s->own.release();
  if (s->st) ctx_stream_destroy(s->st);
  delete s;
}

size_t part_elems(const bessx_session *s) {
  return cox_score_part_doubles(s->nrb, s->p, s->model_type == 4 && s->cox.one_pass);
}

int k1_begin(bessx_session *s, hipEvent_t *a, hipEvent_t *b) {
  if (!s->timing) return 0;
  if (s->ev_used + 2 > s->ev_pool.size()) {
    for (int i = 0; i < 64; i++) {
      hipEvent_t e;
      HIPX(s->own.event(&e));
      s->ev_pool.push_back(e);
    }
  }
  *a = s->ev_pool[s->ev_used++];
  *b = s->ev_pool[s->ev_used++];
  HIPX(hipEventRecord(*a, s->st));
  return 0;
}

int k1_collect(bessx_session *s, const std::vector<std::pair<size_t, bool>> &pairs) {
  if (!s->timing) return 0;
  for (auto &pr : pairs) {
    if (!pr.second || pr.first == (size_t)-1) continue;
    float ms = 0.f;
    HIPX(hipEventElapsedTime(&ms, s->ev_pool[pr.first], s->ev_pool[pr.first + 1]));
    s->k1_seconds += (double)ms * 1e-3;
    s->k1_launches += 1;
    s->k1_bytes += 8.0 * (double)s->n * (double)s->p;
  }
  s->ev_used = 0;
  return 0;
}

int cov_collect(bessx_session *s, int nfill) {
  if (!s->timing) return 0;
  for (auto &pr : s->cov_timed) {
    const int real = std::min(2, std::max(0, nfill / 32 - pr.second));
    if (real == 0) continue;
    float ms = 0.f;
    HIPX(hipEventElapsedTime(&ms, s->ev_pool[pr.first], s->ev_pool[pr.first + 1]));
    s->k1_seconds += (double)ms * 1e-3;
    s->k1_launches += 1;
    s->k1_bytes += 8.0 * (double)s->n * (double)s->p;
    s->panel_w_seconds[real - 1] += (double)ms * 1e-3;
    s->panel_w_launches[real - 1] += 1;
    if (test_hook("panel_log")) std::fprintf(stderr, "[bessx] panel pass: %d group(s) %.3f ms%s\n", real, ms, s->kch_owner ? " (chunk chain)" : "");
  }
  s->cov_timed.clear();
  s->ev_used = 0;
  return 0;
}

int alloc_gram_cache(bessx_session *s) {
  Owner &own = rowset_owner(s, (int)s->gcache.size());
  bessx_session::GramCache c;
  hipError_t e = own.alloc(&c.g0, (size_t)256 * 256);
  if (e == hipSuccess) e = own.alloc(&c.g1, (size_t)256 * 256);
  if (e == hipSuccess) e = own.alloc(&c.A, 256);
  if (e == hipSuccess) e = own.zeros(&c.meta, 2);
  if (e != hipSuccess) return fail(BESSX_ERR_HIP, std::string("Gram cache: ") + hipGetErrorString(e));
  s->gcache.push_back(c);
  return 0;
}

int alloc_cov_cache(bessx_session *s, bool share_map) {
  Owner &own = rowset_owner(s, (int)s->cov.size());
  bessx_session::CovCache c;
  hipError_t e = own.alloc(&c.G, (size_t)s->p * s->cov_C);
  if (share_map && !s->cov.empty()) {
    c.slot_of = s->cov[0].slot_of;
    c.meta = s->cov[0].meta;
    c.shares_map = true;
  }
  if (e == hipSuccess && !c.shares_map) e = own.alloc(&c.slot_of, (size_t)s->p);
  if (e == hipSuccess && !c.shares_map) e = own.alloc(&c.meta, 8);
  if (e == hipSuccess) e = own.zeros(&c.GS, (size_t)COV_CS * COV_CS);
  if (e == hipSuccess && !c.shares_map) e = hipMemset(c.slot_of, 0xff, (size_t)s->p * sizeof(int));
  if (e == hipSuccess && !c.shares_map) e = hipMemset(c.meta, 0, 8 * sizeof(int));
  if (e == hipSuccess) e = own.zeros(&c.zero, 8);
  if (e != hipSuccess) return fail(BESSX_ERR_HIP, std::string("Gram column cache: ") + hipGetErrorString(e));
  s->cov.push_back(c);
  return 0;
}

struct OwnStream {
  hipStream_t st;
  int device, leave_out, stride;
  bool in_use;
};
static std::mutex g_own_mu;
static std::vector<OwnStream> g_own_streams;
static long long g_own_created = 0;
long long ctx_streams_created() {
  std::lock_guard<std::mutex> lk(g_own_mu);
  return g_own_created;
}
static constexpr size_t OWN_QUEUE_CAP = 24;

void ctx_stream_destroy(hipStream_t st) {
  if (!st) return;
  {
    std::lock_guard<std::mutex> lk(g_own_mu);
    for (auto &o : g_own_streams)
      if (o.st == st && o.in_use) {
        (void)hipStreamSynchronize(st);
        o.in_use = false;
        return;
      }
  }
  (void)hipStreamDestroy(st);
}

bool ctx_stream_create(int device, hipStream_t *st, int leave_out, int stride) {
  const char *hook = test_hook("ctx_streams");
  if (hook && std::string(hook) == "pool") return false;
  {
    size_t cap = OWN_QUEUE_CAP;
    if (const char *ec = test_hook("ctx_streams_cap")) cap = (size_t)std::max(0, std::atoi(ec));
    std::lock_guard<std::mutex> lk(g_own_mu);
    size_t busy = 0;
// ... 839 lines not shown
  }
  s->cache.assign(1, bessx_session::RsCache());
  if (s->grouped) {
    HIPT(s->own.alloc(&s->gidx, (size_t)s->N));
    HIPT(s->own.alloc(&s->gsz, (size_t)s->N));
    HIPT(s->own.alloc(&s->goff, (size_t)s->N + 1));
    HIPT(hipMemcpy(s->gidx, s->gidx_h.data(), (size_t)s->N * sizeof(int), hipMemcpyHostToDevice));
    HIPT(hipMemcpy(s->gsz, s->gsz_h.data(), (size_t)s->N * sizeof(int), hipMemcpyHostToDevice));
    HIPT(hipMemcpy(s->goff, s->goff_h.data(), ((size_t)s->N + 1) * sizeof(int), hipMemcpyHostToDevice));
    HIPT(s->own.alloc(&s->gcols_new, (size_t)s->capA));
    HIPT(s->own.alloc(&s->mblk, (size_t)s->goff_h[s->N]));
    HIPT(s->own.alloc(&s->dcol, (size_t)p));
    if (s->gmax > 16) {
      HIPT(s->own.alloc(&s->mwork, (size_t)s->goff_h[s->N]));
      HIPT(s->own.alloc(&s->zwork, (size_t)2 * p));
    }
    if (s->model_type == 4) {
      HIPT(s->own.alloc(&s->mblk2, (size_t)s->goff_h[s->N]));
      HIPT(s->own.alloc(&s->allcols, (size_t)p));
      HIPT(launch_iota(s->allcols, p, s->st));
    }
    HIPT(s->own.alloc(&q, (size_t)s->goff_h[s->N]));
    s->gxtx_rs.push_back(q);
  }
  TRY(alloc_gram_cache(s));
  {
    int mode = pb->score_mode;
    if (mode == 0)
      if (const char *ev = std::getenv("BESSX_SCORE_MODE")) mode = std::atoi(ev);
    if (mode < 0 || mode > 2) return bail(fail(BESSX_ERR_ARG, "score_mode must be 0 (auto), 1 (streaming) or 2 (covariance)"));
    const bool eligible = s->model_type == 1 && (!s->grouped || (s->g_uniform > 0 && s->gmax <= GRP_EIG_MAX));
    if (mode == 2 && !eligible)
      return bail(fail(BESSX_ERR_ARG, "covariance score mode exists for LM with singleton groups or groups of one width "
                                      "(at most 16 columns) only"));
    if (eligible && mode != 1) {
      s->cov_spec = COV_R;
      if (const char *ev = test_hook("cov_spec_min")) s->cov_spec_min = std::max(1, std::min(COV_R - 1, std::atoi(ev)));
      const long all = ((long)p + 31) / 32 * 32 + COV_R + s->cov_spec;
      const long budget = (((long)2 << 30) / ((long)p * 8)) / 32 * 32;
      long C = all <= budget ? all : std::min<long>(2560, budget);
      if (const char *ev = test_hook("cov_cap"))
        C = std::min<long>(C, std::max(0, std::atoi(ev)) / 32 * 32);
      if (s->grouped && C < all) C = 0;
      if (C >= 2 * COV_R + s->cov_spec) {
        s->cov_mode = true;
        s->cov_C = (int)C;
        const int pt = (p + 15) / 16, njg = (pt + cov_streamed_tiles_per_wave() - 1) / cov_streamed_tiles_per_wave();
        long ns = 1, rps = ld;
        long panel_blocks = 0;
        {
          const long conc = 256;
          double best = 1e300;
          const long ns_max = std::max<long>(1, std::min<long>(64, ld / 256));
          for (long t = 1; t <= ns_max; t++) {
            const long r = ((ld + t - 1) / t + 63) / 64 * 64, used = (ld + r - 1) / r;
            const long blocks = (long)((njg + 1) / 2) * used;
            const double cost = (double)((blocks + conc - 1) / conc) * (double)r * (blocks < conc ? 2.0 : 1.0);
            if (cost < best) {
              best = cost;
              ns = used;
              rps = r;
              panel_blocks = blocks;
            }
          }
        }
        s->cov_panel_blocks = (int)std::min<long>(panel_blocks, 1 << 30);
        s->cov_rps = (int)rps;
        s->cov_nslab = (int)ns;
        HIPT(s->own.alloc(&s->cov_part, (size_t)COV_SLOT_GROUPS * ns * njg * cov_streamed_tiles_per_wave() * 2 * 256));
        HIPT(s->own.alloc(&s->bd2, (size_t)p));
        HIPT(s->own.zeros(&s->inA, (size_t)p));
        HIPT(s->own.alloc(&s->cov_bmm, (size_t)3 * ((p + 31) / 32)));
        HIPT(s->own.alloc(&s->cov_fcols, (size_t)s->capA + 4 * COV_R));
        HIPT(s->own.alloc(&s->cov_extras, (size_t)2 * COV_R));
        TRY(alloc_cov_cache(s));
        HIPT(cov_panel_prepare());
        if (const char *ev = test_hook("cov_solver")) s->cov_cg = std::string(ev) != "chol";
        if (const char *ev = test_hook("fuse")) s->fuse = std::string(ev) != "0";
        if (const char *ev = test_hook("fuse_sel")) s->fuse_sel = std::string(ev) != "0";
        if (const char *ev = test_hook("defer_publish")) s->defer_pub = std::string(ev) != "0";
        if (!s->fuse) s->defer_pub = false;
        if (const char *ev = test_hook("cg_layout")) s->cg_by_rows = std::string(ev) != "tiles";
        if (const char *ev = test_hook("cov_cs")) s->cov_cs = std::min(COV_CS, std::max(1, std::atoi(ev)));
      } else if (mode == 2) {
        return bail(fail(BESSX_ERR_ARG, "covariance score mode: p too large for the Gram column cache"));
      }
    }
  }
  HIPT(s->own.alloc(&s->idcols, (size_t)capA + 16));
  if (s->model_type == 4) HIPT(cox_alloc(s));
  if (s->model_type == 1) {
    TRY(prepare_rowset(s, 0));
    if (const char *ev = test_hook("path_group_xtx")) s->path_group_xtx = std::string(ev) != "0";
  }
  HIPT(hipStreamSynchronize(s->st));
#undef TRY
#undef HIPT
  *out = s;
  return BESSX_OK;
}

static int fetch_device_vector(const char *what, const void *data, int dtype, long long stride, int n, int device,
                               hipStream_t caller, std::vector<double> &host) {
  int dev = -1;
  if (int rc = check_device_matrix(what, data, dtype, stride, 0, n, 1, &dev)) return rc;
  if (dev != device) return fail(BESSX_ERR_ARG, std::string(what) + ": memory of another device than the session's");
  const long long ld = ((long long)n + 127) / 128 * 128;
  Owner sc;
  double *d = nullptr;
  unsigned *flag = nullptr;
  HIPX(sc.alloc(&d, (size_t)ld));
  HIPX(sc.alloc(&flag, 1));
  hipStream_t st = nullptr;
  HIPX(hipStreamCreateWithFlags(&st, hipStreamNonBlocking));
  host.assign((size_t)n, 0.0);
  int rc = ingest_enqueue(data, dtype == BESSX_F32, stride, 0, nullptr, n, 1, d, ld, flag, caller, st);
  if (rc == 0) {
    hipError_t e = hipMemcpyAsync(host.data(), d, (size_t)n * sizeof(double), hipMemcpyDeviceToHost, st);
    if (e == hipSuccess) e = hipStreamSynchronize(st);
    if (e != hipSuccess) rc = fail(BESSX_ERR_HIP, std::string(what) + ": " + hipGetErrorString(e));
  }
  (void)hipStreamDestroy(st);
  return rc;
}

}

extern "C" {

int bessx_session_create_device(bessx_session **out, const bessx_problem *pb, const bessx_device_input *in) {
  if (!out || !pb || !in) return fail(BESSX_ERR_ARG, "null argument");
  if (pb->n < 1 || pb->p < 1) return fail(BESSX_ERR_ARG, "n and p must be positive");
  if (!in->y_host && !in->y_dev) return fail(BESSX_ERR_ARG, "device input: y_host or y_dev must be given");
  if (in->y_host && in->y_dev) return fail(BESSX_ERR_ARG, "device input: give y_host or y_dev, not both");
  if (in->weight_host && in->weight_dev) return fail(BESSX_ERR_ARG, "device input: give weight_host or weight_dev, not both");
  if (int rc = need_device()) return rc;
  const int n = pb->n;
  int xdev = -1;
  if (int rc = check_device_matrix("device input x", in->x, in->x_dtype, in->x_row_stride, in->x_col_stride, n, pb->p, &xdev))
    return rc;
  if (pb->device >= 0 && pb->device != xdev)
    return fail(BESSX_ERR_ARG, "device input x: memory of another device than bessx_problem.device");
  if (in->row_order) {
    std::vector<unsigned char> seen((size_t)n, 0);
    for (int i = 0; i < n; i++) {
      const int r = in->row_order[i];
      if (r < 0 || r >= n || seen[(size_t)r]) return fail(BESSX_ERR_ARG, "device input: row_order must be a permutation of 0..n-1");
      seen[(size_t)r] = 1;
    }
  }
  HIPX(hipSetDevice(xdev));
  hipStream_t caller = static_cast<hipStream_t>(in->stream);
  std::vector<double> yh, wh;
  if (in->y_dev)
    if (int rc = fetch_device_vector("device input y", in->y_dev, in->y_dtype, in->y_stride, n, xdev, caller, yh)) return rc;
  if (in->weight_dev)
    if (int rc = fetch_device_vector("device input weight", in->weight_dev, in->weight_dtype, in->weight_stride, n, xdev,
                                     caller, wh))
      return rc;
  bessx_problem q = *pb;
  q.x = nullptr;
  q.x_col_major = 0;
  q.y = in->y_dev ? yh.data() : in->y_host;
  q.weight = in->weight_dev ? wh.data() : in->weight_host;
  q.device = xdev;
  DevX dx;
// ... 429 lines not shown
  return BESSX_OK;
}

int bessx_session_submodel_steps(bessx_session *s, int reset, long long *steps) {
  if (!s) return fail(BESSX_ERR_ARG, "null session");
  if (steps) *steps = s->n_submodel_steps;
  if (reset) s->n_submodel_steps = 0;
  return BESSX_OK;
}

int bessx_session_score_pass_stats(bessx_session *s, int reset, double *seconds, long long *launches,
                                   double *algorithmic_bytes) {
  if (!s) return fail(BESSX_ERR_ARG, "null session");
  if (seconds) *seconds = s->k1_seconds;
  if (launches) *launches = s->k1_launches;
  if (algorithmic_bytes) *algorithmic_bytes = s->k1_bytes;
  if (reset) {
    s->k1_seconds = 0.0;
    s->k1_launches = 0;
    s->k1_bytes = 0.0;
    s->panel_w_seconds[0] = s->panel_w_seconds[1] = 0.0;
    s->panel_w_launches[0] = s->panel_w_launches[1] = 0;
  }
  return BESSX_OK;
}

int bessx_session_score_mode(const bessx_session *s) { return s && s->cov_mode ? 2 : 1; }

long long bessx_session_counter(const bessx_session *s, int which) {
  if (!s && which >= 38 && which <= 40) {
    return which == 38 ? Ledger::device_bytes.load() : (which == 39 ? Ledger::pinned_bytes.load() : Ledger::requests.load());
  }
  if (!s) return -1;
  switch (which) {
    case 0: return s->chain_hits;
    case 1: return s->cov_cg_fallbacks;
    case 2: return s->cov_panel_groups;
    case 3: return s->chain_queued;
    case 4: return 0;
    case 5:
    case 6: return 0;
    case 7: return s->cv_rounds;
    case 8: return s->cv_union_fills;
    case 9: return s->cov_tie_rescues;
    case 11: return s->cv_ctx_dropped;
    case 12: return (long long)s->fold_ctx.size();
    case 13: return s->shared_wide_fills;
    case 14: return s->kch_paths;
    case 15: return s->kch_refits;
    case 16: return s->kch_chunk_fills;
    case 17: return s->kch_last_chains;
    case 18: return s->kch_giveups;
    case 19: {
      if (s->xtx_ev_pending && s->xtx_ev[0] && s->xtx_ev[1]) {
        float ms = 0.f;
        bessx_session *w = const_cast<bessx_session *>(s);
        if (hipEventSynchronize(s->xtx_ev[1]) == hipSuccess && hipEventElapsedTime(&ms, s->xtx_ev[0], s->xtx_ev[1]) == hipSuccess)
          w->group_xtx_ns = (long long)(1e6 * (double)ms);
        w->xtx_ev_pending = false;
      }
      return s->group_xtx_ns;
    }
    case 20:
    case 21: return 0;
    case 22: return (long long)(1e6 * s->kch_t[0]);
    case 23: return (long long)(1e6 * s->kch_t[1]);
    case 24: return (long long)(1e6 * s->kch_t[2]);
    case 25: return s->panel_w_launches[0];
    case 26: return (long long)(1e9 * s->panel_w_seconds[0]);
    case 27: return s->panel_w_launches[1];
    case 28: return (long long)(1e9 * s->panel_w_seconds[1]);
    case 29: return s->sp_launches;
    case 30: return s->sp_chain_slots;
    case 31: return s->sp_partial;
    case 32: return ctx_streams_created();
    case 33: return s->multi_batched;
    case 34: return s->multi_host;
    case 35: return s->multi_fills;
    case 36: return s->x_host_bytes;
    case 37: return s->x_dev_bytes;
    case 38: return Ledger::device_bytes.load();
    case 39: return Ledger::pinned_bytes.load();
    case 40: return Ledger::requests.load();
    case 10: {
      if (s->cov.empty()) return 0;
      int m[8] = {0, 0, 0, 0, 0, 0, 0, 0};
      if (hipSetDevice(s->device) != hipSuccess || hipStreamSynchronize(s->st) != hipSuccess ||
          hipMemcpy(m, s->cov[0].meta, sizeof(m), hipMemcpyDeviceToHost) != hipSuccess)
        return -1;
      return m[3];
    }
    default: return -1;
  }
}

int bessx_session_get_screening(const bessx_session *s, int *columns, int cap) {
  if (!s) return 0;
  for (int j = 0; j < s->p && j < cap && columns; j++) columns[j] = caller_col(s, j);
  return s->p;
}

int bessx_session_get_screening_groups(const bessx_session *s, int *groups, int cap) {
  if (!s) return 0;
  const int cnt = (int)s->screen_groups.size();
  for (int g = 0; g < cnt && g < cap && groups; g++) groups[g] = s->screen_groups[g];
  return cnt;
}

int bessx_session_get_screening_scores(const bessx_session *s, double *scores, int cap) {
  if (!s) return 0;
  const int cnt = (int)s->screen_scores.size();
  for (int u = 0; u < cnt && u < cap && scores; u++) scores[u] = s->screen_scores[u];
  return cnt;
}

int bessx_session_reset_caches(bessx_session *s) {
  if (!s) return fail(BESSX_ERR_ARG, "null session");
  HIPX(hipSetDevice(s->device));
  for (auto &v : s->cv_init) v.clear();
  return reset_path_caches(s);
}

int bessx_session_fit_width(const bessx_session *s, int T0) {
  if (!s || T0 < 1 || T0 > s->N) return -1;
  if (!s->grouped) return T0;
  std::vector<int> sz(s->gsz_h);
  std::partial_sort(sz.begin(), sz.begin() + T0, sz.end(), std::greater<int>());
  long w = 0;
  for (int i = 0; i < T0; i++) w += sz[i];
  return (int)std::min<long>(w, s->p);
}


}
```

Measured before the change: 19070 candidates/s.

## Build covariance fill lists on device inside top-k and fuse compaction into reduce

When the top-k kernel finds missing Gram columns, it now runs a second top-k over bd2 and builds the fill list on device, marking the control block as listed. The host unpark path then skips its own top-k and fill-list launches and reads the group count from the control block. Compaction of the Gram submatrix is folded into the reduce kernel, and a redundant slot-map copy and sync in the k-chunk path is skipped. This cuts launches and host-device round trips per fill, at the cost of extra work inside the single-block top-k kernel and more complex state handling.

```diff
diff --git a/bess_amd/capi.py b/bess_amd/capi.py
--- a/bess_amd/capi.py
+++ b/bess_amd/capi.py
@@ -643,7 +643,8 @@
                  32: "own_queue_streams_created_by_the_process", 33: "multi_responses_batched",
                  34: "multi_responses_host", 35: "multi_union_fills", 36: "x_bytes_uploaded_from_host",
                  37: "x_bytes_ingested_on_device", 38: "live_device_bytes_of_the_process",
-                 39: "live_pinned_bytes_of_the_process", 40: "allocation_requests_of_the_process"}
+                 39: "live_pinned_bytes_of_the_process", 40: "allocation_requests_of_the_process",
+                 41: "fill_lists_built_on_device"}
         return {n: int(lib().bessx_session_counter(self._h, i)) for i, n in names.items()}
 
     def screening(self):
diff --git a/bess_amd/csrc/bessx_dev.h b/bess_amd/csrc/bessx_dev.h
--- a/bess_amd/csrc/bessx_dev.h
+++ b/bess_amd/csrc/bessx_dev.h
@@ -34,6 +34,7 @@
   unsigned long long snap_seq;
 };
 static_assert(sizeof(FitCtrl) <= 128, "the published control block is 128 bytes");
+constexpr int COV_STALL_LISTED = 5;
 
 constexpr int GRAM_JC = 8;
 struct GramTask {
@@ -265,6 +266,9 @@
   double *cm_hist_beta, *cm_hist_coef0;
   int cm_hist_stride;
   unsigned char *cm_inA;
+  int list_on;
+  int *extras;
+  int list_pool, list_spec_max, list_spec, list_spec_min;
 };
 bool topk_can_fuse_need(int len);
 struct TopkTie {
@@ -547,7 +551,8 @@
 hipError_t cov_panel_prepare();
 hipError_t launch_cov_reduce(const double *part, int p, const int *fcols, const int *slot_of, double *G, int g0,
                              int ngroups, int nslab, const FitCtrl *ctrl, int parked, hipStream_t st,
-                             int ex_lo = 0, int ex_hi = 0);
+                             int ex_lo = 0, int ex_hi = 0, double *GS = nullptr, int CS = 0, const double *xtx = nullptr,
+                             int *meta = nullptr);
 hipError_t launch_rows_permute(const double *X, long ld, int p, const int *perm, long ldp, double *Xp, hipStream_t st);
 hipError_t launch_cov_compact(const double *G, int p, const int *slot_of, const int *fcols, int g0, int ngroups,
                               double *GS, int CS, const FitCtrl *ctrl, int parked, hipStream_t st,
diff --git a/bess_amd/csrc/bessx_fit.cpp b/bess_amd/csrc/bessx_fit.cpp
--- a/bess_amd/csrc/bessx_fit.cpp
+++ b/bess_amd/csrc/bessx_fit.cpp
@@ -137,12 +137,14 @@
                          s->cov_nslab, s->cov_part, gc, parked, s->st);
     if (s->timing && e == hipSuccess) {
       e = hipEventRecord(eb, s->st);
-      s->cov_timed.push_back({s->ev_used - 2, g0});
-    }
+      const int known = s->cov_known_nfill >= 0 ? std::min(COV_SLOT_GROUPS, s->cov_known_nfill / COV_R - g0) : 0;
+      s->cov_timed.push_back({s->ev_used - 2, known > 0 ? -known : g0});
+    }
+    const bool in_reduce = compact && s->fill_dev;
     if (e == hipSuccess)
       e = launch_cov_reduce(s->cov_part, s->p, s->cov_fcols, smap, cv.G, g0, ng, s->cov_nslab, gc, parked,
-                            s->st);
-    if (e == hipSuccess && compact)
+                            s->st, 0, 0, in_reduce ? cv.GS : nullptr, s->cov_cs, s->xtx[rs], cv.meta);
+    if (e == hipSuccess && compact && !in_reduce)
       e = launch_cov_compact(cv.G, s->p, smap, s->cov_fcols, g0, ng, cv.GS, s->cov_cs, gc, parked, s->st, s->xtx[rs],
                              cv.meta);
     if (e != hipSuccess) return fail(BESSX_ERR_HIP, std::string("cov panel: ") + hipGetErrorString(e));
@@ -160,6 +162,7 @@
   bool attached = false;
   int cont_serial = 0, cont_parent = 0;
   bool cont = false, cont_fused = false;
+  bool ahead = false;
 };
 
 CholFuse cov_fuse_args(bessx_session *s, int rs, int T0, bool force_chol, SlotFuse *sf) {
@@ -234,6 +237,15 @@
 
 bool cov_speculates(const bessx_session *s) { return topk_supported(s->p, s->cov_spec) && s->p >= 2 * s->cov_spec; }
 
+bool cov_fill_wide(const bessx_session *s) {
+  return cov_speculates(s) && s->cov_C >= (s->p + 31) / 32 * 32 + COV_R && topk_supported(s->p, 2 * COV_R) && s->p >= 4 * COV_R;
+}
+
+bool cov_list_on_device(const bessx_session *s, int rs) {
+  return s->fill_dev && cov_fill_wide(s) && !s->kch_owner && !s->parent && !s->cv_shared && !s->cov_no_restart &&
+         !s->grouped && !(s->fill_hook && rs == 0);
+}
+
 int enqueue_lm_slot_cov(bessx_session *s, int slot, int T0, double lambda, int rs, bool skip_d,
                                bool scores_ok, bool grow1, SlotFuse *sf) {
   bessx_session::CovCache &cv = s->cov[rs];
@@ -264,6 +276,14 @@
     nd.cm_inA = s->inA;
     nd.commit_on = (s->fuse && (T0 + 1 + 15) / 16 <= 16) ? 1 : 0;
     nd.no_restart = s->cov_no_restart ? 1 : 0;
+    if (cov_list_on_device(s, rs) && !(sf && sf->ahead)) {
+      nd.list_on = 1;
+      nd.extras = s->cov_extras;
+      nd.list_pool = 2 * COV_R;
+      nd.list_spec_max = s->cov_spec;
+      nd.list_spec = 2;
+      nd.list_spec_min = s->cov_spec_min > 0 ? s->cov_spec_min : s->cov_spec / 2;
+    }
     if (sf && sf->cont && s->fuse && slot == 1 && skip_d && scores_ok) {
       nd.cont_on = 1;
       nd.cont_serial = sf->cont_serial;
@@ -381,15 +401,19 @@
       return 0;
     }
   }
-  const bool wide = spec && s->cov_C >= (s->p + 31) / 32 * 32 + COV_R && topk_supported(s->p, 2 * COV_R) && s->p >= 4 * COV_R;
+  const bool listed = hc->cov_stall == COV_STALL_LISTED;
+  if (listed && (s->kch_owner || hc->cov_nfill < COV_R || hc->cov_nfill % COV_R))
+    return fail(BESSX_ERR_NUMERIC, "internal error: a device-built fill list where the host hands the list out");
+  if (listed) s->cov_dev_lists++;
+  const bool wide = cov_fill_wide(s);
   const int pool = wide ? 2 * COV_R : s->cov_spec;
-  if (spec) e = launch_topk(s->bd2, s->p, pool, s->cov_extras, s->cand, nullptr, 0, s->st);
-  if (e == hipSuccess)
+  if (spec && !listed) e = launch_topk(s->bd2, s->p, pool, s->cov_extras, s->cand, nullptr, 0, s->st);
+  if (e == hipSuccess && !listed)
     e = launch_cov_fill_list(s->cov_fcols, s->cov_extras, s->bd2, smap, cv.meta, s->ctrl, 1, s->st, s->cov_spec,
                              spec ? (wide ? 2 : 1) : 0, s->cov_spec_min);
   if (e != hipSuccess) return fail(BESSX_ERR_HIP, std::string("cov_unpark: ") + hipGetErrorString(e));
   const int room = spec ? std::min(((nm + s->cov_spec_min + s->cov_spec - 1) / s->cov_spec) * s->cov_spec - nm, pool) : 0;
-  const int ngroups = (nm + room + COV_R - 1) / COV_R;
+  const int ngroups = listed ? hc->cov_nfill / COV_R : (nm + room + COV_R - 1) / COV_R;
   if (test_hook("panel_log")) std::fprintf(stderr, "[bessx] fill: level %d, %d missing, list of up to %d -> %d group(s)%s\n", T0, nm, nm + room, ngroups, s->kch_owner ? " (chunk chain)" : "");
   hipStream_t own_st = s->st;
   hipStream_t fill_st = staged ? s->kch_owner->kch_fill_st : nullptr;
@@ -402,7 +426,9 @@
     HIPX(hipStreamWaitEvent(fill_st, s->kch_ev, 0));
     s->st = fill_st;
   }
+  s->cov_known_nfill = listed ? hc->cov_nfill : -1;
   int frc = enqueue_cov_fill(s, rs, ngroups, 1, nullptr, 0, true, smap);
+  s->cov_known_nfill = -1;
   hipError_t fe = hipSuccess;
   if (frc == 0 && staged) fe = launch_cov_publish_slots(s->cov_fcols, cv.slot_w, cv.slot_of, s->ctrl, s->st);
   s->st = own_st;
@@ -1147,6 +1173,7 @@
   bool published = false, snapshotted = false;
   for (int b = 0, sl = 1; b < batch && sl <= s->max_iter; b++, sl++) {
     SlotFuse sf;
+    sf.ahead = true;
     const bool last = b + 1 == batch || sl == s->max_iter;
     if (last) {
       sf.pub = &pa;
diff --git a/bess_amd/csrc/bessx_host.h b/bess_amd/csrc/bessx_host.h
--- a/bess_amd/csrc/bessx_host.h
+++ b/bess_amd/csrc/bessx_host.h
@@ -316,6 +316,9 @@
   bool cov_cg = true;
   long long cov_cg_fallbacks = 0;
   long long cov_tie_rescues = 0;
+  bool fill_dev = true;
+  long long cov_dev_lists = 0;
+  int cov_known_nfill = -1;
   int cov_C = 0;
   int cov_rps = 0, cov_nslab = 0;
   bool cv_shared = false;
diff --git a/bess_amd/csrc/bessx_k_cov.hip b/bess_amd/csrc/bessx_k_cov.hip
--- a/bess_amd/csrc/bessx_k_cov.hip
+++ b/bess_amd/csrc/bessx_k_cov.hip
@@ -46,43 +46,11 @@
   KT(10);
   if (parked ? !ctrl->cov_stall : (ctrl->done || ctrl->l != 0)) return;
   const int nm = ctrl->cov_nmiss;
-  const int tid = threadIdx.x;
   if (nm == 0) {
-    if (tid == 0) ctrl->cov_nfill = 0;
+    if (threadIdx.x == 0) ctrl->cov_nfill = 0;
     return;
   }
-  const int count = meta[0];
-  const int pool = spec == 2 ? 2 * COV_R : spec_max;
-  const int room = spec ? min(((nm + spec_min + spec_max - 1) / spec_max) * spec_max - nm, pool) : 0;
-  __shared__ int s_ne;
-  if (tid < 64) {
-    const int col = (spec && tid < pool) ? extras[tid] : -1;
-    const double sc = col >= 0 ? bd2[col] : -1.0;
-    const bool valid = col >= 0 && sc >= 0.0 && slot_of[col] < 0;
-    const unsigned long long bal = __ballot(valid);
-    int rank = 0;
-    if (pool > spec_max) {
-      for (int u = 0; u < 64; u++) {
-        const double su = __shfl(sc, u);
-        const int cu = __shfl(col, u);
-        const bool vu = (bal >> u) & 1ull;
-        if (vu && (su > sc || (su == sc && cu < col))) rank++;
-      }
-    } else {
-      rank = __popcll(bal & ((1ull << tid) - 1ull));
-    }
-    if (valid && rank < room) fcols[nm + rank] = col;
-    if (tid == 0) s_ne = min((int)__popcll(bal), room);
-  }
-  __syncthreads();
-  const int tot = nm + s_ne, padded = (tot + COV_R - 1) / COV_R * COV_R;
-  for (int i = tot + tid; i < padded; i += 256) fcols[i] = -1;
-  for (int i = tid; i < tot; i += 256) slot_of[fcols[i]] = count + i;
-  if (tid == 0) {
-    meta[0] = count + tot;
-    ctrl->cov_nfill = padded;
-    ctrl->cov_groups += padded / COV_R;
-  }
+  cov_fill_list_body<256>(fcols, extras, bd2, slot_of, meta, ctrl, nm, spec_max, spec, spec_min, 0);
 }
 
 __global__ void __launch_bounds__(256) k_cov_publish_slots(const int *__restrict__ fcols, const int *__restrict__ slot_w,
@@ -361,7 +329,9 @@
                                                 int njg, int p, const int *__restrict__ fcols,
                                                 const int *__restrict__ slot_of, double *__restrict__ G,
                                                 const FitCtrl *__restrict__ ctrl, int big,
-                                                int ex_lo, int ex_hi) {
+                                                int ex_lo, int ex_hi, double *__restrict__ GS = nullptr, int CS = 0,
+                                                const double *__restrict__ xtx = nullptr,
+                                                int *__restrict__ meta = nullptr) {
   if (big ? !ctrl->cov_stall : (ctrl->done || ctrl->l != 0)) return;
   const int gl = blockIdx.y;
   if (gl >= ngroups || (g0 + gl) * COV_R >= ctrl->cov_nfill) return;
@@ -374,16 +344,29 @@
   const int j = jt * 16 + (lane >> 4) + 4 * reg;
   const int ci = (g0 + gl) * COV_R + ni * 16 + (lane & 15);
   const int col = fcols[ci];
-  if (j < p && col >= 0) G[(size_t)slot_of[col] * p + j] = s;
+  if (j < p && col >= 0) {
+    const int sc = slot_of[col];
+    G[(size_t)sc * p + j] = s;
+    const int t = GS != nullptr ? slot_of[j] : -1;
+    if (t >= 0 && sc >= 0) {
+      const double dj = xtx != nullptr ? xtx[j] : 0.0;
+      if (xtx != nullptr && j != col && s * s >= (1.0 - 2e-11) * dj * xtx[col] && dj > 0.0) meta[4] = 1;
+      if (sc < CS && t < CS) {
+        GS[(size_t)sc * CS + t] = s;
+        GS[(size_t)t * CS + sc] = s;
+      }
+    }
+  }
 }
 
 __global__ void __launch_bounds__(256) k_cov_reduce(const double *__restrict__ part, int g0, int ngroups, int nslab,
                                                     int njg, int p, const int *__restrict__ fcols,
                                                     const int *__restrict__ slot_of, double *__restrict__ G,
                                                     const FitCtrl *__restrict__ ctrl, int slot, int big,
-                                                    int ex_lo, int ex_hi) {
+                                                    int ex_lo, int ex_hi, double *__restrict__ GS, int CS,
+                                                    const double *__restrict__ xtx, int *__restrict__ meta) {
   KT(6);
-  cov_reduce_body(part, g0, ngroups, nslab, njg, p, fcols, slot_of, G, ctrl, big, ex_lo, ex_hi);
+  cov_reduce_body(part, g0, ngroups, nslab, njg, p, fcols, slot_of, G, ctrl, big, ex_lo, ex_hi, GS, CS, xtx, meta);
 }
 
 __global__ void __launch_bounds__(256) k_cov_reduce_sets(const double *__restrict__ part, int g0, int ngroups, int nslab,
@@ -645,10 +628,10 @@
 
 hipError_t launch_cov_reduce(const double *part, int p, const int *fcols, const int *slot_of, double *G, int g0,
                              int ngroups, int nslab, const FitCtrl *ctrl, int parked, hipStream_t st, int ex_lo,
-                             int ex_hi) {
+                             int ex_hi, double *GS, int CS, const double *xtx, int *meta) {
   const int pt = (p + 15) / 16, njg = (pt + COV_NJ - 1) / COV_NJ;
   hipLaunchKernelGGL(k_cov_reduce, dim3(njg * COV_NJ * 2, ngroups), dim3(256), 0, st, part, g0, ngroups, nslab, njg, p,
-                     fcols, slot_of, G, ctrl, 0, parked, ex_lo, ex_hi);
+                     fcols, slot_of, G, ctrl, 0, parked, ex_lo, ex_hi, GS, CS, xtx, meta);
   LAUNCH_CHECK();
   return hipSuccess;
 }
diff --git a/bess_amd/csrc/bessx_k_solve.hip b/bess_amd/csrc/bessx_k_solve.hip
--- a/bess_amd/csrc/bessx_k_solve.hip
+++ b/bess_amd/csrc/bessx_k_solve.hip
@@ -65,7 +65,7 @@
 }
 
 template <int EB, int NT>
-__device__ __forceinline__ void topk_body(const double *__restrict__ score, const int *__restrict__ idx_in,
+__device__ __forceinline__ int topk_body(const double *__restrict__ score, const int *__restrict__ idx_in,
                                           int len_total, int chunk, int k, int *__restrict__ out,
                                           int *__restrict__ out_count, const FitCtrl *ctrl, int slot,
                                           const int *__restrict__ run_flag, const TopkNeed &nd) {
@@ -73,7 +73,7 @@
   if (nd.cont_on) {
     FitCtrl *c = nd.ctrl;
     const bool go = c->serial == nd.cont_parent && c->done && c->d_fresh && c->l >= 0 && !c->cov_stall && !c->info;
-    if (!go) return;
+    if (!go) return 0;
     for (int i = threadIdx.x; i < k; i += NT) nd.cm_hist[i] = 0;
     __syncthreads();
     if (threadIdx.x == 0) {
@@ -96,9 +96,9 @@
     }
     __syncthreads();
   } else if (ctrl != nullptr && (ctrl->done || ctrl->l != slot - 1)) {
-    return;
-  }
-  if (run_flag != nullptr && *run_flag == 0) return;
+    return 0;
+  }
+  if (run_flag != nullptr && *run_flag == 0) return 0;
   __shared__ int wcnt[2][NWV];
   if (nd.slot_of != nullptr && nd.inc1 && nd.ctrl->l == 0 && nd.ctrl->k_cur + 1 == k &&
       (gridDim.x == 1 || nd.pub.on)) {
@@ -196,14 +196,14 @@
         __syncthreads();
         PH(3);
         PH_COUNT();
-        return;
+        return 0;
       }
       __syncthreads();
-      cov_need_body<NT>(out, k, nd.bd, nd.bd2, nd.p, nd.slot_of, nd.meta, nd.C, nd.fcols, nd.ctrl, slot, nd.A_cur, true,
-                      nd.no_restart != 0);
+      const int pk = cov_need_body<NT>(out, k, nd.bd, nd.bd2, nd.p, nd.slot_of, nd.meta, nd.C, nd.fcols, nd.ctrl, slot,
+                                       nd.A_cur, true, nd.no_restart != 0);
       PH(3);
       PH_COUNT();
-      return;
+      return pk;
     }
     for (int base = 0; base < k - 1; base += NT) {
       const int i = base + threadIdx.x;
@@ -221,15 +221,15 @@
     }
     __syncthreads();
     PH(2);
-    cov_need_body<NT>(out, k, nd.bd, nd.bd2, nd.p, nd.slot_of, nd.meta, nd.C, nd.fcols, nd.ctrl, slot, nd.A_cur, true,
-                      nd.no_restart != 0);
+    const int pk = cov_need_body<NT>(out, k, nd.bd, nd.bd2, nd.p, nd.slot_of, nd.meta, nd.C, nd.fcols, nd.ctrl, slot,
+                                     nd.A_cur, true, nd.no_restart != 0);
     PH(3);
     PH_COUNT();
-    return;
+    return pk;
   }
 full_search:
   if (nd.slot_of != nullptr && nd.ctrl->fast_same) {
-    if (repeated_set_body<NT>(nd, k, out, slot)) return;
+    if (repeated_set_body<NT>(nd, k, out, slot)) return 0;
   }
   __shared__ int wsum[NWV];
   __shared__ int wsum2[NWV];
@@ -300,7 +300,7 @@
       nd.ctrl->l = -1 - nd.ctrl->l;
       nd.ctrl->fast_same = 0;
     }
-    return;
+    return 0;
   }
   int take_eq = min(max(need_eq - eq_before, 0), neq);
   int nsel = ngt + take_eq, tot_sel;
@@ -323,10 +323,22 @@
   if (tid == 0 && out_count != nullptr && tot_eq > need_eq && kk < len) out_count[0] = 1;
   if (nd.slot_of != nullptr) {
     __syncthreads();
-    cov_need_body<NT>(out, k, nd.bd, nd.bd2, nd.p, nd.slot_of, nd.meta, nd.C, nd.fcols, nd.ctrl, slot, nd.A_cur, false,
-                      nd.no_restart != 0);
-  }
-}
+    return cov_need_body<NT>(out, k, nd.bd, nd.bd2, nd.p, nd.slot_of, nd.meta, nd.C, nd.fcols, nd.ctrl, slot, nd.A_cur,
+                             false, nd.no_restart != 0);
+  }
+  return 0;
+}
+
+template <int EB, int NT>
+__device__ __forceinline__ void cov_park_list(const TopkNeed *nd, int nm) {
+  __syncthreads();
+  const TopkNeed none = {};
+  (void)topk_body<EB, NT>(nd->bd2, nullptr, nd->p, nd->p, nd->list_pool, nd->extras, nullptr, nullptr, 0, nullptr, none);
+  __syncthreads();
+  cov_fill_list_body<NT>(nd->fcols, nd->extras, nd->bd2, nd->slot_of, nd->meta, nd->ctrl, nm, nd->list_spec_max,
+                         nd->list_spec, nd->list_spec_min, COV_STALL_LISTED);
+}
+
 
 template <int EB>
 __global__ void __launch_bounds__(1024) k_topk(const double *__restrict__ score, const int *__restrict__ idx_in,
@@ -338,7 +350,8 @@
     publish_body(nd.pub);
     return;
   }
-  topk_body<EB, 1024>(score, idx_in, len_total, chunk, k, out, out_count, ctrl, slot, run_flag, nd);
+  const int pk = topk_body<EB, 1024>(score, idx_in, len_total, chunk, k, out, out_count, ctrl, slot, run_flag, nd);
+  if (nd.list_on && pk > 0) cov_park_list<EB, 1024>(&nd, pk);
 }
 
 __global__ void __launch_bounds__(1024) k_topk_ties(const double *__restrict__ score, int len, int k,
@@ -1530,7 +1543,8 @@
       }
     }
   }
-  topk_body<EB, 512>(score, nullptr, len, len, k, out, nullptr, ctrl, slot, nullptr, nd);
+  const int pk = topk_body<EB, 512>(score, nullptr, len, len, k, out, nullptr, ctrl, slot, nullptr, nd);
+  if (nd.list_on && pk > 0) cov_park_list<EB, 512>(&nd, pk);
   __syncthreads();
 #ifdef BESSX_KTRACE
   const unsigned long long kt1_ = wall_clock64();
@@ -1568,7 +1582,7 @@
 template <int EB>
 __device__ __noinline__ void mc_topk_call(const double *score, int p, int k, int *out, const FitCtrl *ctrl, int slot,
                                           const TopkNeed *nd) {
-  topk_body<EB, 512>(score, nullptr, p, p, k, out, nullptr, ctrl, slot, nullptr, *nd);
+  (void)topk_body<EB, 512>(score, nullptr, p, p, k, out, nullptr, ctrl, slot, nullptr, *nd);
 }
 template <int RPT, int NCW>
 __device__ __noinline__ void mc_cgr_call(int m, int nc, double ridge, const double *rhs, const int *A_new, double *sol,
diff --git a/bess_amd/csrc/bessx_kchunks.cpp b/bess_amd/csrc/bessx_kchunks.cpp
--- a/bess_amd/csrc/bessx_kchunks.cpp
+++ b/bess_amd/csrc/bessx_kchunks.cpp
@@ -809,6 +809,7 @@
   std::vector<int> bounds;
   CoarsePlan coarse;
   bool staged = false;
+  bool map_in_step = false;
   std::vector<StartModel> start;
   std::vector<ChunkRun> run;
   bool early_on = false;
@@ -879,6 +880,10 @@
         if (coarse.start_of[(size_t)r] == (int)m + 1) start[(size_t)r] = at;
     }
     if (int rc = settle_device_chain(s)) return rc;
+    if (staged && s->fill_dev) {
+      HIPX(hipMemcpyAsync(s->kch_slot_w, s->cov[0].slot_of, (size_t)s->p * sizeof(int), hipMemcpyDeviceToDevice, s->st));
+      map_in_step = true;
+    }
     HIPX(hipStreamSynchronize(s->st));
     t_coarse = Clock::now();
     return 0;
@@ -886,6 +891,10 @@
 
   int writer_map_in_step() {
     if (!staged) return 0;
+    if (map_in_step) {
+      map_in_step = false;
+      return 0;
+    }
     HIPX(hipMemcpyAsync(s->kch_slot_w, s->cov[0].slot_of, (size_t)s->p * sizeof(int), hipMemcpyDeviceToDevice, s->st));
     HIPX(hipStreamSynchronize(s->st));
     return 0;
diff --git a/bess_amd/csrc/bessx_kdev.hpp b/bess_amd/csrc/bessx_kdev.hpp
--- a/bess_amd/csrc/bessx_kdev.hpp
+++ b/bess_amd/csrc/bessx_kdev.hpp
@@ -480,7 +480,7 @@
 }
 
 template <int NT>
-__device__ void cov_need_body(const int *__restrict__ list, int len, const double *__restrict__ bd,
+__device__ int cov_need_body(const int *__restrict__ list, int len, const double *__restrict__ bd,
                               double *__restrict__ bd2, int p, int *__restrict__ slot_of, int *__restrict__ meta, int C,
                               int *__restrict__ fcols, FitCtrl *__restrict__ ctrl, int slot,
                               const int *__restrict__ A_cur, bool known_diff = false, bool no_restart = false) {
@@ -496,7 +496,7 @@
     }
     diff = __syncthreads_or(diff);
     if (tid == 0) ctrl->same_prev = diff ? 0 : 1;
-    if (!diff) return;
+    if (!diff) return 0;
   }
   int count = meta[0];
   bool restart = count + len + COV_R > C;
@@ -515,7 +515,7 @@
       ctrl->cov_stall = 4;
       ctrl->l = -1 - ctrl->l;
     }
-    return;
+    return 0;
   }
   if (restart) {
     for (int j = tid; j < p; j += NT) slot_of[j] = -1;
@@ -528,7 +528,7 @@
     const int miss = (col >= 0 && slot_of[col] < 0) ? 1 : 0;
     if (!__syncthreads_or(miss)) {
       if (tid == 0) ctrl->cov_nmiss = 0;
-      return;
+      return 0;
     }
   }
   for (int base = 0; base < len; base += NT) {
@@ -571,6 +571,48 @@
     __syncthreads();
     for (int i = tid; i < nm; i += NT) bd2[fcols[i]] = -1.0;
   }
+  return (spec && slot > 0 && !restart) ? nm : 0;
+}
+
+template <int NT>
+__device__ __forceinline__ void cov_fill_list_body(int *__restrict__ fcols, const int *__restrict__ extras,
+                                                   const double *__restrict__ bd2, int *__restrict__ slot_of,
+                                                   int *__restrict__ meta, FitCtrl *__restrict__ ctrl, int nm,
+                                                   int spec_max, int spec, int spec_min, int stall_mark) {
+  const int tid = threadIdx.x;
+  const int count = meta[0];
+  const int pool = spec == 2 ? 2 * COV_R : spec_max;
+  const int room = spec ? min(((nm + spec_min + spec_max - 1) / spec_max) * spec_max - nm, pool) : 0;
+  __shared__ int s_ne;
+  if (tid < 64) {
+    const int col = (spec && tid < pool) ? extras[tid] : -1;
+    const double sc = col >= 0 ? bd2[col] : -1.0;
+    const bool valid = col >= 0 && sc >= 0.0 && slot_of[col] < 0;
+    const unsigned long long bal = __ballot(valid);
+    int rank = 0;
+    if (pool > spec_max) {
+      for (int u = 0; u < 64; u++) {
+        const double su = __shfl(sc, u);
+        const int cu = __shfl(col, u);
+        const bool vu = (bal >> u) & 1ull;
+        if (vu && (su > sc || (su == sc && cu < col))) rank++;
+      }
+    } else {
+      rank = __popcll(bal & ((1ull << tid) - 1ull));
+    }
+    if (valid && rank < room) fcols[nm + rank] = col;
+    if (tid == 0) s_ne = min((int)__popcll(bal), room);
+  }
+  __syncthreads();
+  const int tot = nm + s_ne, padded = (tot + COV_R - 1) / COV_R * COV_R;
+  for (int i = tot + tid; i < padded; i += NT) fcols[i] = -1;
+  for (int i = tid; i < tot; i += NT) slot_of[fcols[i]] = count + i;
+  if (tid == 0) {
+    meta[0] = count + tot;
+    ctrl->cov_nfill = padded;
+    ctrl->cov_groups += padded / COV_R;
+    if (stall_mark) ctrl->cov_stall = stall_mark;
+  }
 }
 
 #define LAUNCH_CHECK()                         \
diff --git a/bess_amd/csrc/bessx_session.cpp b/bess_amd/csrc/bessx_session.cpp
--- a/bess_amd/csrc/bessx_session.cpp
+++ b/bess_amd/csrc/bessx_session.cpp
@@ -94,7 +94,7 @@
 int cov_collect(bessx_session *s, int nfill) {
   if (!s->timing) return 0;
   for (auto &pr : s->cov_timed) {
-    const int real = std::min(2, std::max(0, nfill / 32 - pr.second));
+    const int real = pr.second < 0 ? -pr.second : std::min(2, std::max(0, nfill / 32 - pr.second));
     if (real == 0) continue;
     float ms = 0.f;
     HIPX(hipEventElapsedTime(&ms, s->ev_pool[pr.first], s->ev_pool[pr.first + 1]));
@@ -1100,6 +1100,7 @@
         if (!s->fuse) s->defer_pub = false;
         if (const char *ev = test_hook("cg_layout")) s->cg_by_rows = std::string(ev) != "tiles";
         if (const char *ev = test_hook("cov_cs")) s->cov_cs = std::min(COV_CS, std::max(1, std::atoi(ev)));
+        if (const char *ev = test_hook("fill_path")) s->fill_dev = std::string(ev) != "host";
       } else if (mode == 2) {
         return bail(fail(BESSX_ERR_ARG, "covariance score mode: p too large for the Gram column cache"));
       }
@@ -1695,6 +1696,7 @@
     case 38: return Ledger::device_bytes.load();
     case 39: return Ledger::pinned_bytes.load();
     case 40: return Ledger::requests.load();
+    case 41: return s->cov_dev_lists;
     case 10: {
       if (s->cov.empty()) return 0;
       int m[8] = {0, 0, 0, 0, 0, 0, 0, 0};
```

Measured after the change: 19420 candidates/s (median of 6 runs). 1.8% higher.
